# bgmanuel99/Super-Resolution-Images-for-3D-Printing-Defect-Detection

Hardware: AMD Instinct MI355X
Metric: 4x-SR MPix/s on 512x512 LR batch (higher is better)
Workload: dtype bf16

## Files before the change

__graft_entry__.py:

```python
import os
import subprocess
import sys

ROOT = os.path.dirname(os.path.abspath(__file__))
PKG = os.path.join(ROOT, "super-resolution-images-for-3d-printing-defect-detection_amd")
for p in (ROOT, PKG):
    if p not in sys.path:
        sys.path.insert(0, p)


def build():
    jobs = str(min(4, os.cpu_count() or 1))
    subprocess.run(["make", "-C", os.path.join(PKG, "csrc"), "-j", jobs], check=True)
    subprocess.run([sys.executable, os.path.join(ROOT, "tools", "check_prefetch_hazards.py")], check=True)
    subprocess.run([sys.executable, os.path.join(ROOT, "tools", "check_prefetch_hazards.py"), "--source", os.path.join(PKG, "csrc", "attention.hip"),
                    "--match", "attn_bf16_kernel", "--allow-scratch"], check=True)
    import sr355
    from sr355 import _lib
    _lib.load()
    import SRModels.loading_methods
    import oracle


def smoke():
    import numpy as np
    import torch
    assert torch.cuda.is_available(), "smoke() needs a GPU"
    from oracle import models as OM
    from oracle import ops as OO
    from sr355 import Context
    from sr355.synth import make_pairs
    from sr355.weights import bf16_rounded, init_weights
    from SRModels.deep_learning_models.ESRGAN_model import ESRGAN

    ctx = Context.get(0)
    lr, hr = make_pairs(1, 40, 36, 4, seed=7)
    for dtype, tol in (("f32", 1e-4), ("bf16", 2e-2)):
        m = ESRGAN(compute_dtype=dtype)
        m.setup_model(scale_factor=4, growth_channels=32, num_rrdb_blocks=2)
        w = init_weights(m.generator.layer_shapes(), seed=3000)
        if dtype == "bf16":
            w = bf16_rounded(w)
        m.set_weights(w)
        sr, metrics = m.super_resolve_image(lr[0], patch_size_lr=24, stride=12)
        ref = OM.esrgan_super_resolve(lr[0], w, 4, 24, 12, num_rrdb=2, dtype=np.float64)
        err = float(np.abs(sr - ref).max())
        assert sr.shape == (160, 144, 3) and err <= tol, (dtype, err)
        p_gpu = float(ctx.psnr(ctx.to_device(hr), ctx.to_device(sr[None]))[0])
        p_ref = float(OO.psnr(hr, ref[None].astype(np.float32))[0])
        assert abs(p_gpu - p_ref) <= 0.01, (p_gpu, p_ref)
        print(f"smoke[{dtype}]: max|gpu-oracle|={err:.2e}  PSNR(gpu,HR)={p_gpu:.4f} dB  PSNR(oracle,HR)={p_ref:.4f} dB  "
              f"time_sec={metrics['time_sec']:.4f}")
    print("smoke OK")


if __name__ == "__main__":
    build()
    if len(sys.argv) > 1 and sys.argv[1] == "smoke":
        smoke()
```

super-resolution-images-for-3d-printing-defect-detection_amd/csrc/api.hip:

```cpp
#include <math.h>
#include <stdio.h>
#include <stdlib.h>
#include <string.h>

#include <memory>

#include "common.h"

void* sr_ctx::dalloc(size_t bytes) {
    void* p = nullptr;
    if (bytes == 0) bytes = 16;
    if (alloc_cap > 0 && cur_bytes + (int64_t)bytes > alloc_cap) {
        err = "allocation of " + std::to_string(bytes) + " bytes exceeds the debug cap (sr_debug_set_alloc_cap)";
        return nullptr;
    }
    hipError_t e = hipMalloc(&p, bytes);
    if (e != hipSuccess) {
        err = std::string("hipMalloc(") + std::to_string(bytes) + "): " + hipGetErrorString(e);
        return nullptr;
    }
    allocs[p] = bytes;
    cur_bytes += (int64_t)bytes;
    if (cur_bytes > peak_bytes) peak_bytes = cur_bytes;
    return p;
}
void sr_ctx::dfree(void* p) {
    if (!p) return;
    auto it = allocs.find(p);
    if (it != allocs.end()) { cur_bytes -= (int64_t)it->second; allocs.erase(it); }
    (void)hipFree(p);
}
int sr_ctx::ensure_dyn_lds(const void* kernel, int bytes) {
    if (bytes > MAX_LDS_BYTES) return fail(SR_ERR_INVALID, "kernel needs " + std::to_string(bytes) + " bytes of LDS, a CU has " + std::to_string(MAX_LDS_BYTES));
    auto it = lds_attr_done.find(kernel);
    if (it != lds_attr_done.end() && it->second >= bytes) return SR_OK;
    hipError_t e = hipFuncSetAttribute(kernel, hipFuncAttributeMaxDynamicSharedMemorySize, bytes);
    if (e != hipSuccess) return fail(SR_ERR_HIP, std::string("hipFuncSetAttribute: ") + hipGetErrorString(e));
    lds_attr_done[kernel] = bytes;
    return SR_OK;
}
void* sr_ctx::scratch(size_t bytes) {
    if (bytes <= scratch_cap) return scratch_buf;
    if (scratch_buf) { (void)hipDeviceSynchronize(); dfree(scratch_buf); scratch_buf = nullptr; scratch_cap = 0; }
    size_t cap = bytes < (1u << 20) ? (1u << 20) : bytes;
    scratch_buf = dalloc(cap);
    if (scratch_buf) scratch_cap = cap;
    return scratch_buf;
}

int sr_ctx::cu_count() {
    if (num_cus <= 0) {
        hipDeviceProp_t prop;
        num_cus = (hipGetDeviceProperties(&prop, device) == hipSuccess && prop.multiProcessorCount > 0) ? prop.multiProcessorCount : 256;
    }
    return num_cus;
}

void* sr_ctx::arena(Arena& a, size_t bytes, hipStream_t st) {
    if (bytes <= a.cap) return a.p;
    if (a.p) { (void)hipStreamSynchronize(st); dfree(a.p); a.p = nullptr; a.cap = 0; }
    const size_t cap = bytes < (1u << 20) ? (1u << 20) : bytes + bytes / 4;
    a.p = dalloc(cap);
    if (a.p) a.cap = cap;
    return a.p;
}

int sr_ctx::prof_open(const std::string& name, double flops, double bytes, hipStream_t st) {
    if (!prof) return -1;
    int ni = -1;
    for (size_t i = 0; i < prof_names.size(); ++i) if (prof_names[i] == name) { ni = (int)i; break; }
    if (ni < 0) { prof_names.push_back(name); ni = (int)prof_names.size() - 1; }
    hipEvent_t e[2];
    for (int k = 0; k < 2; ++k) {
        if (!ev_pool.empty()) { e[k] = ev_pool.back(); ev_pool.pop_back(); }
        else if (hipEventCreate(&e[k]) != hipSuccess) return -1;
    }
    (void)hipEventRecord(e[0], st);
    prof_recs.push_back(ProfRec{ni, e[0], e[1], flops, bytes});
    return (int)prof_recs.size() - 1;
}
void sr_ctx::prof_close(int rec, hipStream_t st) {
    if (rec >= 0) (void)hipEventRecord(prof_recs[rec].e1, st);
}

namespace {

struct Param {
    std::string name; int which; std::vector<int64_t> shape; std::vector<float> host; bool set = false;
    int64_t count() const { int64_t n = 1; for (auto s : shape) n *= s; return n; }
};
struct Ref { int buf = -1; int coff = 0; };
enum OpKind { OP_CONVERT, OP_CONV, OP_ATTN, OP_POOL, OP_GAP, OP_DENSE, OP_TOBLK, OP_SUBSAMPLE, OP_PREPROC };
struct Op {
    OpKind kind = OP_CONV;
    Ref in, out, skip1, skip2;
    int conv = -1;
    int act = SR_ACT_LINEAR; float alpha = 1.f, beta1 = 0.f, beta2 = 0.f; int clip = 0, d2s = 1;
    int dw = -1, db = -1, In = 0, Out = 0;
    int chain = -1, chain_pos = 0;
    int rgbtail = -1;
    int pack_alt = -1;
    int pw2 = -1;
    int proj = -1;
    int block = -1, block_pos = 0;
};
struct BufSpec { int C = 0; int mul = 1; int shift = 0; bool vec = false; int Cbuf = 0; int blk = 0; int cshift = 0; int cells = 0; int cat = 0; };
struct ConvPart { std::string name; int cout; float scale = 1.f; };
struct ConvSpec { std::vector<ConvPart> parts; int KS = 3, Cin = 0, Cout = 0; ConvWeights w; int rows_head = 0; };
struct ChainSpec { int conv_a = -1, conv_b = -1; int tail = 0; ChainWeights w; };
struct RgbTailSpec { int conv_b = -1; RgbTailWeights w; };
struct BlockSpec { int conv[5] = {-1, -1, -1, -1, -1}; BlockWeights w; };
struct ProjSpec { int conv = -1; ProjWeights w; };
struct Pw2Spec { int conv = -1; int act = 0; Pw2Weights w; };

}

struct sr_model {
    sr_ctx* ctx = nullptr;
    int kind = 0;
    sr_model_cfg cfg{};
    int T = SR_DTYPE_BF16;
    std::vector<Param> params;
    std::vector<ConvSpec> convs;
    std::vector<ChainSpec> chains;
    std::vector<BlockSpec> blocks;
    std::vector<RgbTailSpec> rgbtails;
    std::vector<ProjSpec> projs;
    std::vector<Pw2Spec> pw2s;
    std::vector<BufSpec> bufs;
    std::vector<void*> bufp;
    std::vector<float*> dense_dev;
    std::vector<Op> ops;
    int in_C = 3, out_C = 3, out_mul = 1, out_shift = 0; bool out_vec = false;
    bool finalized = false;
    std::vector<size_t> bufcap;
    std::vector<CellGrid> grid_now;
    std::vector<int> routes;
    struct Tap { float* dst; int64_t cap; };
    std::unordered_map<int, Tap> taps;
    std::vector<std::string> op_names;
    int block_stream = 0;

    int find_param(const std::string& n, int which) const {
        for (size_t i = 0; i < params.size(); ++i) if (params[i].which == which && params[i].name == n) return (int)i;
        return -1;
    }
    void free_bufs() { for (auto& p : bufp) { if (p) ctx->dfree(p); p = nullptr; } bufcap.assign(bufcap.size(), 0); grid_now.assign(grid_now.size(), CellGrid{}); }
    TensorView view(const Ref& r) const { return r.buf >= 0 ? TensorView{bufp[r.buf], bufs[r.buf].Cbuf, r.coff, bufs[r.buf].blk} : TensorView{}; }
};

namespace {

struct Builder {
    sr_model* m;
    int esz() const { return dtype_size(m->T); }
    int E() const { return 16 / esz(); }
    int buf(int C, int mul = 1, int shift = 0) {
        BufSpec b; b.C = C; b.mul = mul; b.shift = shift; b.Cbuf = round_up(C, 32);
        m->bufs.push_back(b); return (int)m->bufs.size() - 1;
    }
    int vecbuf(int C) { BufSpec b; b.C = C; b.vec = true; b.Cbuf = C; m->bufs.push_back(b); return (int)m->bufs.size() - 1; }
    void add_layer_params(const std::string& name, std::vector<int64_t> kshape) {
        Param k; k.name = name; k.which = SR_WEIGHT_KERNEL; k.shape = kshape; m->params.push_back(k);
        Param b; b.name = name; b.which = SR_WEIGHT_BIAS; b.shape = {kshape.back()}; m->params.push_back(b);
    }
    int conv_spec(std::vector<ConvPart> parts, int KS, int Cin) {
        ConvSpec c; c.parts = parts; c.KS = KS; c.Cin = Cin; c.Cout = 0;
        for (auto& p : parts) { c.Cout += p.cout; add_layer_params(p.name, {KS, KS, Cin, p.cout}); }
        m->convs.push_back(c); return (int)m->convs.size() - 1;
    }
    Op& conv(const std::string& name, int KS, int Cin, int Cout, Ref in, Ref out, int act = SR_ACT_LINEAR) {
        Op o; o.kind = OP_CONV; o.conv = conv_spec({{name, Cout}}, KS, Cin); o.in = in; o.out = out; o.act = act;
        m->ops.push_back(o); return m->ops.back();
    }
    Op& conv_again(int spec, Ref in, Ref out, int act = SR_ACT_LINEAR) {
        Op o; o.kind = OP_CONV; o.conv = spec; o.in = in; o.out = out; o.act = act;
        m->ops.push_back(o); return m->ops.back();
    }
    void self_attention(const std::string& name, int x, int y, int qkv, int ao) {
        const float kscale = m->T == SR_DTYPE_BF16 ? 1.4426950408889634f : 1.f;
        Op p; p.kind = OP_CONV; p.conv = conv_spec({{name + "_f", 8, kscale}, {name + "_g", 8}, {name + "_h", 32}}, 1, 64);
        p.in = {x, 0}; p.out = {qkv, 0};
        if (m->T == SR_DTYPE_BF16 && !m->ops.empty() && m->ops.back().kind == OP_CONV && m->ops.back().out.buf == x && m->ops.back().out.coff == 0) {
            ProjSpec ps; ps.conv = p.conv;
            m->projs.push_back(ps);
            m->ops.back().proj = (int)m->projs.size() - 1;
        }
        m->ops.push_back(p);
        Op a; a.kind = OP_ATTN; a.in = {qkv, 0}; a.out = {ao, 0}; m->ops.push_back(a);
        Op& v = conv(name + "_v", 1, 32, 64, {ao, 0}, {y, 0});
        v.skip1 = {x, 0}; v.beta1 = 1.f;
    }
};

int build_srcnn(sr_model* m) {
    Builder b{m};
    const int C = m->cfg.channels;
    m->in_C = C; m->out_C = C; m->out_mul = 1;
    const int x0 = b.buf(b.E()), c1 = b.buf(96), c2 = b.buf(32);
    m->bufs[x0].Cbuf = b.E();
    Op cv; cv.kind = OP_CONVERT; cv.out = {x0, 0}; m->ops.push_back(cv);
    b.conv("conv2d", 9, C, 96, {x0, 0}, {c1, 0}, SR_ACT_RELU);
    b.conv("conv2d_1", 1, 96, 32, {c1, 0}, {c2, 0}, SR_ACT_RELU);
    if (m->T == SR_DTYPE_F32 && C == 3) {
        Pw2Spec ps; ps.conv = m->ops.back().conv; ps.act = SR_ACT_RELU;
        m->pw2s.push_back(ps);
        m->ops[m->ops.size() - 2].pw2 = (int)m->pw2s.size() - 1;
    }
    b.conv("conv2d_2", 5, 32, C, {c2, 0}, {-2, 0});
    return SR_OK;
}

int build_edsr(sr_model* m) {
    Builder b{m};
    const sr_model_cfg& c = m->cfg;
    const int C = c.channels, F = c.num_filters, s = c.scale_factor;
    if (s != 2 && s != 3 && s != 4) return m->ctx->fail(SR_ERR_INVALID, "Scale factor " + std::to_string(s) + " not supported. Use 2, 3, or 4.");
    m->in_C = C; m->out_C = C; m->out_mul = s;
    int li = 0;
    auto lname = [&]() { std::string n = li == 0 ? "conv2d" : "conv2d_" + std::to_string(li); ++li; return n; };
    const int x0 = b.buf(b.E());
    m->bufs[x0].Cbuf = b.E();
    const int head = b.buf(F), tmp = b.buf(F), ra = b.buf(F), rb = b.buf(F);
    Op cv; cv.kind = OP_CONVERT; cv.out = {x0, 0}; m->ops.push_back(cv);
    b.conv(lname(), 3, C, F, {x0, 0}, {head, 0});
    int cur = head;
    for (int i = 0; i < c.num_blocks; ++i) {
        const int nxt = (cur == ra) ? rb : ra;
        b.conv(lname(), 3, F, F, {cur, 0}, {tmp, 0}, SR_ACT_RELU);
        Op& o = b.conv(lname(), 3, F, F, {tmp, 0}, {nxt, 0});
        o.alpha = c.res_scaling; o.skip1 = {cur, 0}; o.beta1 = 1.f;
        cur = nxt;
    }
    const int body = (cur == ra) ? rb : ra;
    { Op& o = b.conv(lname(), 3, F, F, {cur, 0}, {body, 0}); o.skip1 = {head, 0}; o.beta1 = 1.f; }
    int up = body, mul = 1;
    const int nup = s == 4 ? 2 : 1, r = s == 4 ? 2 : s;
    for (int i = 0; i < nup; ++i) {
        mul *= r;
        const int ub = b.buf(F, mul);
        Op& o = b.conv(lname(), 3, F, F * r * r, {up, 0}, {ub, 0}); o.d2s = r;
        up = ub;
    }
    { Op& o = b.conv(lname(), 3, F, C, {up, 0}, {-2, 0}); o.clip = 1; }
    return SR_OK;
}

int build_esrgan(sr_model* m) {
    Builder b{m};
    const sr_model_cfg& c = m->cfg;
    const int C = c.channels, G = c.growth_channels, s = c.scale_factor;
    if (s < 1 || (s & (s - 1)) != 0) return m->ctx->fail(SR_ERR_INVALID, "ESRGAN scale_factor must be a power of two");
    if (G <= 0 || c.num_blocks < 0) return m->ctx->fail(SR_ERR_INVALID, "ESRGAN growth_channels/num_rrdb_blocks invalid");
    m->in_C = C; m->out_C = C; m->out_mul = s;
    const int CC = 64 + 4 * G;
    const int x0 = b.buf(b.E());
    const bool head_rows = m->T == SR_DTYPE_BF16;
    m->bufs[x0].Cbuf = head_rows ? 32 : b.E();
    const int trunk = b.buf(64);
    int cat[3] = {b.buf(CC), b.buf(CC), b.buf(CC)};
    if (m->T == SR_DTYPE_BF16 && G % 8 == 0)
        for (int i = 0; i < 3; ++i) m->bufs[cat[i]].blk = 1;
    for (int i = 0; i < 3; ++i) m->bufs[cat[i]].cat = 1;
    Op cv; cv.kind = OP_CONVERT; cv.out = {x0, 0}; m->ops.push_back(cv);
    b.conv("initial_conv", 3, C, 64, {x0, 0}, {trunk, 0});
    if (head_rows) m->convs.back().rows_head = 1;
    if (m->bufs[cat[0]].blk) {
        Op t; t.kind = OP_TOBLK; t.in = {trunk, 0}; t.out = {cat[0], 0}; m->ops.push_back(t);
    } else {
        b.conv_again((int)m->convs.size() - 1, {x0, 0}, {cat[0], 0});
    }
    int X = 0, Y = 1, Z = 2;
    for (int r = 0; r < c.num_blocks; ++r) {
        const int src[3] = {X, Y, Z}, dst[3] = {Y, Z, Y};
        for (int d = 0; d < 3; ++d) {
            const std::string dn = "rrdb_" + std::to_string(r) + "_dense" + std::to_string(d + 1);
            const int I = cat[src[d]], O = cat[dst[d]];
            const size_t first_op = m->ops.size();
            for (int k = 1; k <= 4; ++k)
                b.conv(dn + "_conv" + std::to_string(k), 3, 64 + (k - 1) * G, G, {I, 0}, {I, 64 + (k - 1) * G}, SR_ACT_RELU);
            Op& o = b.conv(dn + "_conv5", 3, CC, 64, {I, 0}, {O, 0});
            if (d < 2) { o.alpha = 0.2f; o.skip1 = {I, 0}; o.beta1 = 1.f; }
            else { o.alpha = 0.04f; o.skip1 = {cat[X], 0}; o.beta1 = 1.f; o.skip2 = {I, 0}; o.beta2 = 0.2f; }
            if (m->bufs[I].blk && G == 32) {
                auto link = [&](size_t opa, int tail) {
                    ChainSpec cs; cs.conv_a = m->ops[opa].conv; cs.conv_b = m->ops[opa + 1].conv; cs.tail = tail;
                    m->chains.push_back(cs);
                    m->ops[opa].chain = m->ops[opa + 1].chain = (int)m->chains.size() - 1;
                    m->ops[opa].chain_pos = 0; m->ops[opa + 1].chain_pos = 1;
                };
                link(first_op + 1, 0);
                link(first_op + 3, 1);
            }
            if (m->bufs[I].blk && G == 8) {
                BlockSpec bs;
                for (int k = 0; k < 5; ++k) {
                    bs.conv[k] = m->ops[first_op + k].conv;
                    m->ops[first_op + k].block = (int)m->blocks.size(); m->ops[first_op + k].block_pos = k;
                }
                m->blocks.push_back(bs);
            }
        }
        const int nX = Y, nY = Z, nZ = X; X = nX; Y = nY; Z = nZ;
    }
    const int t2 = b.buf(64);
    { Op& o = b.conv("trunk_conv", 3, 64, 64, {cat[X], 0}, {t2, 0}); o.skip1 = {trunk, 0}; o.beta1 = 1.f; o.pack_alt = cat[Y]; }
    int cur = t2;
    if (c.use_attention) {
        const int qkv = b.buf(64), ao = b.buf(32), t3 = b.buf(64);
        b.self_attention("self_attention_trunk", cur, t3, qkv, ao);
        cur = t3;
    }
    int mul = 1, nup = 0;
    for (int t = s; t > 1; t >>= 1) ++nup;
    for (int i = 0; i < nup; ++i) {
        mul *= 2;
        const int u = b.buf(64, mul);
        Op& o = b.conv("upsample_" + std::to_string(i) + "_conv", 3, 64, 256, {cur, 0}, {u, 0}, SR_ACT_LRELU);
        o.d2s = 2;
        cur = u;
        if (i == 0 && c.use_attention) {
            const int qkv = b.buf(64, mul), ao = b.buf(32, mul), ua = b.buf(64, mul);
            b.self_attention("self_attention_upsample_0", cur, ua, qkv, ao);
            cur = ua;
        }
    }
    const int f1 = b.buf(64, mul);
    b.conv("final_conv1", 3, 64, 64, {cur, 0}, {f1, 0}, SR_ACT_RELU);
    b.conv("final_conv2", 3, 64, C, {f1, 0}, {-2, 0}, SR_ACT_TANH);
    if (m->T == SR_DTYPE_BF16 && C <= 3) {
        RgbTailSpec rt; rt.conv_b = m->ops.back().conv;
        m->rgbtails.push_back(rt);
        m->ops[m->ops.size() - 2].rgbtail = (int)m->rgbtails.size() - 1;
    }
    return SR_OK;
}

int build_vgg16(sr_model* m) {
    Builder b{m};
    const int nc = m->cfg.num_classes;
    if (nc <= 0) return m->ctx->fail(SR_ERR_INVALID, "num_classes must be positive");
    m->in_C = 3; m->out_C = nc; m->out_vec = true;
    static const int cfg[5][2] = {{2, 64}, {2, 128}, {3, 256}, {3, 512}, {3, 512}};
    const int x0 = b.buf(b.E());
    const bool head_rows = m->T == SR_DTYPE_BF16;
    m->bufs[x0].Cbuf = head_rows ? 32 : b.E();
    Op cv; cv.kind = OP_CONVERT; cv.out = {x0, 0}; m->ops.push_back(cv);
    int cur = x0, cin = 3;
    for (int blk = 0; blk < 5; ++blk) {
        for (int k = 0; k < cfg[blk][0]; ++k) {
            const int o = b.buf(cfg[blk][1], 1, blk);
            b.conv("block" + std::to_string(blk + 1) + "_conv" + std::to_string(k + 1), 3, cin, cfg[blk][1], {cur, 0}, {o, 0}, SR_ACT_RELU);
            if (blk == 0 && k == 0 && head_rows) m->convs.back().rows_head = 1;
            if (blk == 4 && m->T == SR_DTYPE_BF16) m->bufs[o].cells = 1;
            cur = o; cin = cfg[blk][1];
        }
        const int pb = b.buf(cin, 1, blk + 1);
        if (blk == 3 && m->T == SR_DTYPE_BF16) m->bufs[pb].cells = 1;
        Op p; p.kind = OP_POOL; p.in = {cur, 0}; p.out = {pb, 0}; m->ops.push_back(p);
        cur = pb;
    }
    const int g = b.vecbuf(512), d1 = b.vecbuf(256);
    { Op o; o.kind = OP_GAP; o.in = {cur, 0}; o.out = {g, 0}; m->ops.push_back(o); }
    b.add_layer_params("dense", {512, 256});
    { Op o; o.kind = OP_DENSE; o.in = {g, 0}; o.out = {d1, 0}; o.In = 512; o.Out = 256; o.act = SR_ACT_RELU;
      o.dw = m->find_param("dense", SR_WEIGHT_KERNEL); o.db = m->find_param("dense", SR_WEIGHT_BIAS); m->ops.push_back(o); }
    b.add_layer_params("predictions", {256, nc});
    { Op o; o.kind = OP_DENSE; o.in = {d1, 0}; o.out = {-2, 0}; o.In = 256; o.Out = nc; o.act = 100;
      o.dw = m->find_param("predictions", SR_WEIGHT_KERNEL); o.db = m->find_param("predictions", SR_WEIGHT_BIAS); m->ops.push_back(o); }
    return SR_OK;
}

int build_discriminator(sr_model* m) {
    Builder b{m};
    m->in_C = 3; m->out_C = 1; m->out_vec = true;
    const int x0 = b.buf(b.E());
    m->bufs[x0].Cbuf = b.E();
    Op cv; cv.kind = OP_CONVERT; cv.out = {x0, 0}; m->ops.push_back(cv);
    static const int filt[6] = {64, 64, 64, 128, 128, 256}, strd[6] = {1, 2, 1, 2, 1, 2};
    int cur = x0, cin = 3, halv = 0;
    for (int i = 0; i < 6; ++i) {
        const int o = b.buf(filt[i]);
        m->bufs[o].cshift = halv;
        b.conv("disc_conv" + std::to_string(i + 1), 3, cin, filt[i], {cur, 0}, {o, 0}, SR_ACT_LRELU);
        cur = o; cin = filt[i];
        if (strd[i] == 2) {
            ++halv;
            const int s2 = b.buf(filt[i]);
            m->bufs[s2].cshift = halv;
            Op sp; sp.kind = OP_SUBSAMPLE; sp.in = {cur, 0}; sp.out = {s2, 0}; m->ops.push_back(sp);
            cur = s2;
        }
    }
    const int g = b.vecbuf(256), d1 = b.vecbuf(256);
    { Op o; o.kind = OP_GAP; o.in = {cur, 0}; o.out = {g, 0}; m->ops.push_back(o); }
    b.add_layer_params("disc_dense1", {256, 256});
    { Op o; o.kind = OP_DENSE; o.in = {g, 0}; o.out = {d1, 0}; o.In = 256; o.Out = 256; o.act = SR_ACT_LRELU;
      o.dw = m->find_param("disc_dense1", SR_WEIGHT_KERNEL); o.db = m->find_param("disc_dense1", SR_WEIGHT_BIAS); m->ops.push_back(o); }
    b.add_layer_params("disc_output", {256, 1});
    { Op o; o.kind = OP_DENSE; o.in = {d1, 0}; o.out = {-2, 0}; o.In = 256; o.Out = 1; o.act = 101;
      o.dw = m->find_param("disc_output", SR_WEIGHT_KERNEL); o.db = m->find_param("disc_output", SR_WEIGHT_BIAS); m->ops.push_back(o); }
    return SR_OK;
}

int build_vgg19_features(sr_model* m) {
    Builder b{m};
    m->in_C = 3; m->out_C = 512; m->out_mul = 1; m->out_shift = 4;
    static const int cfg[5][2] = {{2, 64}, {2, 128}, {4, 256}, {4, 512}, {4, 512}};
    const int x0 = b.buf(b.E());
    m->bufs[x0].Cbuf = b.E();
    Op pp; pp.kind = OP_PREPROC; pp.out = {x0, 0}; m->ops.push_back(pp);
    int cur = x0, cin = 3;
    for (int blk = 0; blk < 5; ++blk) {
        for (int k = 0; k < cfg[blk][0]; ++k) {
            const bool last = blk == 4 && k == cfg[blk][0] - 1;
            const int o = last ? -2 : b.buf(cfg[blk][1], 1, blk);
            b.conv("block" + std::to_string(blk + 1) + "_conv" + std::to_string(k + 1), 3, cin, cfg[blk][1], {cur, 0}, {o, 0}, SR_ACT_RELU);
            cur = o; cin = cfg[blk][1];
        }
        if (blk == 4) break;
        const int pb = b.buf(cin, 1, blk + 1);
        Op p; p.kind = OP_POOL; p.in = {cur, 0}; p.out = {pb, 0}; m->ops.push_back(p);
        cur = pb;
    }
    return SR_OK;
}

inline void buf_hw(const BufSpec& b, int H, int W, int* h, int* w) {
    *h = (H * b.mul) >> b.shift; *w = (W * b.mul) >> b.shift;
    for (int i = 0; i < b.cshift; ++i) { *h = (*h + 1) / 2; *w = (*w + 1) / 2; }
}

CellGrid cell_grid_for(int B, int h, int w, int Cbuf) {
    CellGrid g;
    if (h < 1 || w < 1 || w + 1 > 16) return g;
    const int gx = 16 / (w + 1);
    const double plain = (double)h * w / ((double)((h + 11) / 12 * 12) * ((w + 15) / 16 * 16));
    const double packed = (double)h / (h + 1) * gx * w / 16.0;
    if (packed < 1.3 * plain) return g;
    const int64_t Hv = (int64_t)((B + gx - 1) / gx) * (h + 1), Wv = (int64_t)gx * (w + 1);
    if (Hv * Wv * Cbuf >= ((int64_t)1 << 31)) return g;
    g.gx = gx; g.ch = h + 1; g.cw = w + 1; g.Hv = (int)Hv; g.Wv = (int)Wv;
    return g;
}

CellGrid cat_grid_for(int B, int H, int W, int Cmax) {
    CellGrid g;
    if (B < 4 || H < 2 || W < 2) return g;
    const double plain = (double)H * W / ((double)((H + 15) / 16 * 16) * ((W + 15) / 16 * 16));
    const int gx = B < 16 ? B : 16;
    const int64_t Hv = (int64_t)((B + gx - 1) / gx) * (H + 1), Wv = (int64_t)gx * (W + 1);
    const double packed = (double)B * H * W / ((double)((Hv + 15) / 16 * 16) * ((Wv + 15) / 16 * 16));
    if (packed >= 1.15 * plain && Hv * Wv * Cmax < ((int64_t)1 << 31)) { g.gx = gx; g.ch = H + 1; g.cw = W + 1; g.Hv = (int)Hv; g.Wv = (int)Wv; }
    return g;
}

struct Layout {
    bool pack2 = false;
    CellGrid cat;
    bool use_cells = false;
    int B_ws = 0;
};

enum BlockKernel { BLOCK_NONE, BLOCK_RESIDENT, BLOCK_STREAM };
BlockKernel block_kernel(const sr_model* m, int H, int W) {
    if (!(m->kind == SR_MODEL_ESRGAN_G && m->T == SR_DTYPE_BF16 && !m->blocks.empty() && (m->ctx->chain_mask & SR_FUSE_TWO_UP) == SR_FUSE_TWO_UP)) return BLOCK_NONE;
    const bool ring = m->block_stream && H >= 1 && sr_dense_block_stream_lds_bytes(m->cfg.growth_channels, W) > 0;
    if (m->block_stream == 2 && ring) return BLOCK_STREAM;
    if (sr_dense_block_lds_bytes(m->cfg.growth_channels, H, W) > 0) return BLOCK_RESIDENT;
    return ring ? BLOCK_STREAM : BLOCK_NONE;
}
bool block_here(const sr_model* m, int H, int W) { return block_kernel(m, H, W) != BLOCK_NONE; }

Layout choose_layout(const sr_model* m, int B, int H, int W) {
    const int mask = m->ctx->chain_mask;
    Layout L;
    L.use_cells = m->taps.empty() && (mask & SR_FUSE_CELLS) != 0;
    L.pack2 = m->kind == SR_MODEL_ESRGAN_G && m->T == SR_DTYPE_BF16 && W == 24 && (mask & SR_FUSE_TWO_UP) == SR_FUSE_TWO_UP && !m->chains.empty() && B >= 2;
    for (const auto& tp : m->taps) {
        const Op& to = m->ops[tp.first];
        if (to.kind == OP_CONV && to.chain >= 0 && m->chains[to.chain].tail && to.chain_pos == 0) L.pack2 = false;
    }
    bool cat_blk = false; int Cmax = 0;
    for (const BufSpec& bs : m->bufs) if (bs.cat) { cat_blk = cat_blk || bs.blk; Cmax = std::max(Cmax, bs.Cbuf); }
    const bool fused_here = !m->chains.empty() && W == 48 && (mask & (SR_FUSE_DENSE_TAIL | SR_FUSE_DENSE_MID));
    if (m->kind == SR_MODEL_ESRGAN_G && m->T == SR_DTYPE_BF16 && cat_blk && !L.pack2 && !fused_here && !block_here(m, H, W) && m->taps.empty()) L.cat = cat_grid_for(B, H, W, Cmax);
    L.B_ws = L.pack2 ? (B + 1) & ~1 : L.cat.gx ? (int)std::max<int64_t>(B, ((int64_t)L.cat.Hv * L.cat.Wv + (int64_t)H * W - 1) / ((int64_t)H * W)) : B;
    return L;
}

int ensure_workspace(sr_model* m, const Layout& L, int H, int W, hipStream_t st) {
    const int B = L.B_ws;
    if (m->bufp.size() != m->bufs.size()) { m->bufp.assign(m->bufs.size(), nullptr); m->bufcap.assign(m->bufs.size(), 0); m->grid_now.assign(m->bufs.size(), CellGrid{}); }
    for (size_t i = 0; i < m->bufs.size(); ++i) {
        const BufSpec& b = m->bufs[i];
        size_t bytes;
        CellGrid want;
        if (b.vec) bytes = (size_t)B * b.C * sizeof(float);
        else {
            int h, w; buf_hw(b, H, W, &h, &w);
            bytes = (size_t)B * h * w * b.Cbuf * dtype_size(m->T) + 4096;
            if (b.cat) want = L.cat;
            else if (b.cells && L.use_cells) want = cell_grid_for(B, h, w, b.Cbuf);
            if (want.gx) bytes = std::max(bytes, (size_t)want.Hv * want.Wv * b.Cbuf * dtype_size(m->T) + 4096);
        }
        if (bytes <= m->bufcap[i]) {
            const CellGrid& have = m->grid_now[i];
            if (want.gx && !(have.gx == want.gx && have.ch == want.ch && have.cw == want.cw && have.Wv == want.Wv)) SR_HIP(m->ctx, hipMemsetAsync(m->bufp[i], 0, m->bufcap[i], st));
            m->grid_now[i] = want;
            continue;
        }
        m->grid_now[i] = want;
        if (m->bufp[i]) { SR_HIP(m->ctx, hipDeviceSynchronize()); m->ctx->dfree(m->bufp[i]); m->bufp[i] = nullptr; m->bufcap[i] = 0; }
        m->bufp[i] = m->ctx->dalloc(bytes);
        if (!m->bufp[i]) {
            const std::string why = m->ctx->err;
            (void)hipDeviceSynchronize();
            m->free_bufs();
            return m->ctx->fail(SR_ERR_OOM, "workspace for [" + std::to_string(B) + "," + std::to_string(H) + "," + std::to_string(W) + "]: " + why +
                                                " (all workspaces of this model were released)");
        }
        SR_HIP(m->ctx, hipMemsetAsync(m->bufp[i], 0, bytes, st));
        m->bufcap[i] = bytes;
    }
    return SR_OK;
}

enum Route { RT_CHAIN = OP_PREPROC + 1, RT_CHAIN_SECOND, RT_BLOCK, RT_BLOCK_REST, RT_CONV1_STREAM, RT_RGB_TAIL, RT_PW2, RT_IN_EPILOGUE, RT_BLOCK_STREAM };

bool tapped(const sr_model* m, size_t oi) { return !m->taps.empty() && m->taps.count((int)oi) != 0; }
bool bare_epilogue(const Op& op) { return op.skip1.buf < 0 && op.skip2.buf < 0 && op.d2s == 1 && !op.clip; }

bool chain_fits(const sr_model* m, size_t oi, int w, bool pack2) {
    const Op& op = m->ops[oi];
    if (op.chain < 0 || op.chain_pos != 0) return false;
    const ChainSpec& ch = m->chains[op.chain];
    return !(ch.tail && tapped(m, oi)) && (m->ctx->chain_mask & (ch.tail ? SR_FUSE_DENSE_TAIL : SR_FUSE_DENSE_MID)) && chain_supported(ch.w, m->view(op.in), pack2 ? 48 : w);
}
bool conv1_stream_fits(const sr_model* m, const Op& op, int w, bool pack2) {
    return (m->ctx->chain_mask & SR_FUSE_CONV1_STREAM) && op.chain < 0 && op.act == SR_ACT_RELU && op.alpha == 1.f && bare_epilogue(op) && op.out.buf == op.in.buf &&
           op.in.coff == 0 && op.out.coff == 64 && conv1_stream_supported(m->convs[op.conv].w, m->view(op.in), pack2 ? 48 : w);
}
bool rgb_tail_fits(const sr_model* m, const Op& op, size_t oi, int B, int h, int w) {
    const ConvWeights& cw = m->convs[op.conv].w;
    return op.rgbtail >= 0 && (m->ctx->chain_mask & SR_FUSE_RGB_TAIL) && !tapped(m, oi) && cw.rows && cw.NT == 4 && cw.Cout == 64 && bare_epilogue(op) &&
           op.act != SR_ACT_TANH && op.out.buf >= 0 && (int64_t)m->bufcap[op.out.buf] >= rgbtail_partial_bytes(B, h, w);
}
bool pw2_fits(const sr_model* m, const Op& op, size_t oi) {
    const ConvWeights& cw = m->convs[op.conv].w;
    return op.pw2 >= 0 && (m->ctx->chain_mask & SR_FUSE_SRCNN_1X1) && !tapped(m, oi) && cw.thin && !cw.few && cw.dtype == SR_DTYPE_F32 && bare_epilogue(op);
}
bool pool_fits(const sr_model* m, const Op& op, size_t oi, int h, int w) {
    if (oi + 1 >= m->ops.size() || op.out.buf < 0) return false;
    const Op& pl = m->ops[oi + 1];
    const ConvWeights& cw = m->convs[op.conv].w;
    return (m->ctx->chain_mask & SR_FUSE_POOL) && m->T == SR_DTYPE_BF16 && pl.kind == OP_POOL && pl.in.buf == op.out.buf && pl.out.buf >= 0 && cw.rows && cw.NT == 4 &&
           cw.CoutP == cw.Cout && bare_epilogue(op) && op.act != SR_ACT_TANH && !tapped(m, oi) && !m->grid_now[op.in.buf].gx && !m->grid_now[op.out.buf].gx &&
           h >= 2 && w >= 2 && m->bufs[pl.out.buf].Cbuf % 8 == 0 && m->bufs[pl.out.buf].Cbuf >= cw.Cout;
}
bool proj_fits(const sr_model* m, const Op& op) {
    const ConvWeights& cw = m->convs[op.conv].w;
    return op.proj >= 0 && (m->ctx->chain_mask & SR_FUSE_ATTN_PROJ) && cw.rows && cw.NT == 4 && cw.Cout / (op.d2s * op.d2s) == 64 && cw.CoutP == cw.Cout &&
           op.out.buf >= 0 && !m->bufs[op.out.buf].blk && op.skip2.buf < 0 && !op.clip && op.act != SR_ACT_TANH && m->bufs[op.out.buf].Cbuf % 4 == 0;
}

void plan_routes(sr_model* m, const Layout& L, int B, int H, int W) {
    std::vector<int>& rt = m->routes;
    rt.resize(m->ops.size());
    for (size_t oi = 0; oi < m->ops.size(); ++oi) rt[oi] = m->ops[oi].kind;
    for (size_t oi = 0; oi < m->ops.size(); ++oi) {
        const Op& op = m->ops[oi];
        if (rt[oi] != OP_CONV) continue;
        int h, w;
        buf_hw(m->bufs[op.in.buf], H, W, &h, &w);
        if (op.block >= 0 && op.block_pos == 0 && block_here(m, h, w)) {
            rt[oi] = block_kernel(m, h, w) == BLOCK_STREAM ? RT_BLOCK_STREAM : RT_BLOCK;
            for (int k = 1; k < 5; ++k) rt[oi + k] = RT_BLOCK_REST;
        }
        else if (chain_fits(m, oi, w, L.pack2)) { rt[oi] = RT_CHAIN; rt[oi + 1] = RT_CHAIN_SECOND; }
        else if (conv1_stream_fits(m, op, w, L.pack2)) rt[oi] = RT_CONV1_STREAM;
        else if (rgb_tail_fits(m, op, oi, B, h, w)) { rt[oi] = RT_RGB_TAIL; rt[oi + 1] = RT_IN_EPILOGUE; }
        else if (pw2_fits(m, op, oi)) { rt[oi] = RT_PW2; rt[oi + 1] = RT_IN_EPILOGUE; }
        else if (pool_fits(m, op, oi, h, w) || proj_fits(m, op)) rt[oi + 1] = RT_IN_EPILOGUE;
    }
}

}

extern "C" {

int sr_init(int device_id, sr_ctx** out) {
    if (!out) return SR_ERR_INVALID;
    *out = nullptr;
    int n = 0;
    if (hipGetDeviceCount(&n) != hipSuccess || device_id < 0 || device_id >= n) return SR_ERR_HIP;
    if (hipSetDevice(device_id) != hipSuccess) return SR_ERR_HIP;
    sr_ctx* c = new sr_ctx();
    c->device = device_id;
    if (hipEventCreate(&c->ev0) != hipSuccess || hipEventCreate(&c->ev1) != hipSuccess) { delete c; return SR_ERR_HIP; }
    c->zero_page = c->dalloc(sr_ctx::ZERO_PAGE_BYTES);
    if (!c->zero_page) { sr_destroy(c); return SR_ERR_OOM; }
    if (hipMemset(c->zero_page, 0, sr_ctx::ZERO_PAGE_BYTES) != hipSuccess) { sr_destroy(c); return SR_ERR_HIP; }
    *out = c;
    return SR_OK;
}

void sr_destroy(sr_ctx* ctx) {
    DeviceGuard dg_(ctx);
    if (!ctx) return;
    (void)hipDeviceSynchronize();
    lpips_release(ctx);
    std::vector<void*> ps;
    for (auto& kv : ctx->allocs) ps.push_back(kv.first);
    for (void* p : ps) ctx->dfree(p);
    if (ctx->ev0) (void)hipEventDestroy(ctx->ev0);
    if (ctx->ev1) (void)hipEventDestroy(ctx->ev1);
    for (auto& r : ctx->prof_recs) { (void)hipEventDestroy(r.e0); (void)hipEventDestroy(r.e1); }
    for (auto& e : ctx->ev_pool) (void)hipEventDestroy(e);
    delete ctx;
}

const char* sr_last_error(sr_ctx* ctx) { return ctx ? ctx->err.c_str() : "null ctx"; }

int sr_mem_info(sr_ctx* ctx, int64_t* current_bytes, int64_t* peak_bytes) {
    if (!ctx) return SR_ERR_INVALID;
    if (current_bytes) *current_bytes = ctx->cur_bytes;
    if (peak_bytes) *peak_bytes = ctx->peak_bytes;
    return SR_OK;
}

int sr_last_forward_ms(sr_ctx* ctx, float* ms) {
    DeviceGuard dg_(ctx);
    if (!ctx || !ms) return SR_ERR_INVALID;
    if (!ctx->timed) return ctx->fail(SR_ERR_STATE, "no forward has run on this ctx");
    SR_HIP(ctx, hipEventSynchronize(ctx->ev1));
    SR_HIP(ctx, hipEventElapsedTime(ms, ctx->ev0, ctx->ev1));
    return SR_OK;
}

int64_t sr_debug_stamp_bytes_needed(int which, int64_t workgroups) {
    if (which == 0) return workgroups < 0 ? -1 : workgroups * 16 * (int64_t)sizeof(unsigned long long);
    if (which == 1) return (int64_t)64 * 4 * 64 * 4 * (int64_t)sizeof(unsigned long long);
    return -1;
}

int sr_debug_set_stamp_buffer(sr_ctx* ctx, void* device_u64_buffer, int64_t capacity_bytes) {
    if (!ctx) return SR_ERR_INVALID;
    if (device_u64_buffer && capacity_bytes < sr_debug_stamp_bytes_needed(0, 1))
        return ctx->fail(SR_ERR_INVALID, "sr_debug_set_stamp_buffer: the buffer does not hold one workgroup's stamps");
    ctx->stamp_buf = static_cast<unsigned long long*>(device_u64_buffer);
    ctx->stamp_cap = device_u64_buffer ? capacity_bytes : 0;
    return SR_OK;
}

int sr_measure_clock(sr_ctx* ctx, float* mhz, void* stream) {
    if (!ctx || !mhz) return SR_ERR_INVALID;
    DeviceGuard dg_(ctx);
    return clock_probe_launch(ctx, mhz, static_cast<hipStream_t>(stream));
}

int sr_debug_set_chain_stamp_buffer(sr_ctx* ctx, void* device_u64_buffer, int64_t capacity_bytes) {
    if (!ctx) return SR_ERR_INVALID;
    if (device_u64_buffer && capacity_bytes < sr_debug_stamp_bytes_needed(1, 0))
        return ctx->fail(SR_ERR_INVALID, "sr_debug_set_chain_stamp_buffer: the buffer is smaller than the stamped kernels write (sr_debug_stamp_bytes_needed(1, 0))");
    ctx->chain_stamp_buf = static_cast<unsigned long long*>(device_u64_buffer);
    const char* skip = getenv("SR355_CHAIN_STAMP_SKIP");
    ctx->chain_stamp_skip = skip ? atoi(skip) : -1;
    return SR_OK;
}

int sr_debug_set_fused(sr_ctx* ctx, int mask, int max_workgroups) {
    if (!ctx) return SR_ERR_INVALID;
    ctx->chain_mask = mask;
    ctx->chain_max_wgs = max_workgroups > 0 ? max_workgroups : 0;
    return SR_OK;
}

int sr_debug_set_block_stream_bands(sr_ctx* ctx, int n) {
    if (!ctx) return SR_ERR_INVALID;
    ctx->block_stream_bands = n > 0 ? n : 0;
    return SR_OK;
}

int sr_model_set_dense_block_stream(sr_model* m, int mode) {
    if (!m) return SR_ERR_INVALID;
    if (mode < 0 || mode > 2) return m->ctx->fail(SR_ERR_INVALID, "sr_model_set_dense_block_stream: mode is 0, 1 or 2");
    if (!(m->kind == SR_MODEL_ESRGAN_G && m->T == SR_DTYPE_BF16 && m->cfg.growth_channels == 8 && !m->blocks.empty()))
        return m->ctx->fail(SR_ERR_INVALID, "sr_model_set_dense_block_stream: the streamed dense-block kernel serves bf16 ESRGAN generators of 8 growth channels only");
    m->block_stream = mode;
    return SR_OK;
}

int sr_debug_set_alloc_cap(sr_ctx* ctx, int64_t bytes) {
    if (!ctx) return SR_ERR_INVALID;
    ctx->alloc_cap = bytes > 0 ? bytes : 0;
    return SR_OK;
}

int sr_debug_conv_routes(sr_ctx* ctx, int enable, char* text, int64_t cap) {
    if (!ctx) return SR_ERR_INVALID;
    if (text && cap <= (int64_t)ctx->route_text.size()) return ctx->fail(SR_ERR_CAPACITY, "sr_debug_conv_routes: the text buffer is too small");
    if (text) memcpy(text, ctx->route_text.c_str(), ctx->route_text.size() + 1);
    ctx->route_text.clear();
    ctx->route_log = enable != 0;
    return SR_OK;
}

int sr_profile_begin(sr_ctx* ctx) {
    if (!ctx) return SR_ERR_INVALID;
    for (auto& r : ctx->prof_recs) { ctx->ev_pool.push_back(r.e0); ctx->ev_pool.push_back(r.e1); }
    ctx->prof_recs.clear();
    ctx->prof = true;
    return SR_OK;
}

int sr_profile_end(sr_ctx* ctx, char* json, int64_t cap) {
    DeviceGuard dg_(ctx);
    if (!ctx || !json || cap <= 0) return SR_ERR_INVALID;
    ctx->prof = false;
    SR_HIP(ctx, hipDeviceSynchronize());
    struct Agg { int64_t n = 0; double ms = 0, flops = 0, bytes = 0; };
    std::vector<Agg> agg(ctx->prof_names.size());
    for (auto& r : ctx->prof_recs) {
        float ms = 0.f;
        if (hipEventElapsedTime(&ms, r.e0, r.e1) != hipSuccess) continue;
        Agg& a = agg[r.name];
        a.n += 1; a.ms += ms; a.flops += r.flops; a.bytes += r.bytes;
    }
    std::string s = "[";
    bool first = true;
    for (size_t i = 0; i < agg.size(); ++i) {
        if (!agg[i].n) continue;
        char buf[512];
        snprintf(buf, sizeof buf, "%s{\"kernel\": \"%s\", \"launches\": %lld, \"total_ms\": %.6f, \"flops\": %.6e, \"bytes\": %.6e}",
                 first ? "" : ", ", ctx->prof_names[i].c_str(), (long long)agg[i].n, agg[i].ms, agg[i].flops, agg[i].bytes);
        s += buf;
        first = false;
    }
    s += "]";
    for (auto& r : ctx->prof_recs) { ctx->ev_pool.push_back(r.e0); ctx->ev_pool.push_back(r.e1); }
    ctx->prof_recs.clear();
    if ((int64_t)s.size() + 1 > cap) return ctx->fail(SR_ERR_CAPACITY, "profile buffer too small");
    memcpy(json, s.c_str(), s.size() + 1);
    return SR_OK;
}

int sr_model_create(sr_ctx* ctx, int kind, const sr_model_cfg* cfg, sr_model** out) {
    if (!ctx || !cfg || !out) return SR_ERR_INVALID;
    *out = nullptr;
    if (cfg->compute_dtype != SR_DTYPE_F32 && cfg->compute_dtype != SR_DTYPE_BF16)
        return ctx->fail(SR_ERR_INVALID, "compute_dtype must be SR_DTYPE_F32 or SR_DTYPE_BF16");
    std::unique_ptr<sr_model> m(new sr_model());
    m->ctx = ctx; m->kind = kind; m->cfg = *cfg; m->T = cfg->compute_dtype;
    if (m->cfg.channels <= 0) m->cfg.channels = 3;
    if (m->cfg.channels > 16 / dtype_size(m->T))
        return ctx->fail(SR_ERR_INVALID, "channels must fit one 16-byte slice (<= 4 for f32, <= 8 for bf16)");
    int rc;
    switch (kind) {
        case SR_MODEL_SRCNN: rc = build_srcnn(m.get()); break;
        case SR_MODEL_EDSR: rc = build_edsr(m.get()); break;
        case SR_MODEL_ESRGAN_G: rc = build_esrgan(m.get()); break;
        case SR_MODEL_VGG16: rc = build_vgg16(m.get()); break;
        case SR_MODEL_ESRGAN_D: rc = build_discriminator(m.get()); break;
        case SR_MODEL_VGG19_FEATURES: rc = build_vgg19_features(m.get()); break;
        default: return ctx->fail(SR_ERR_INVALID, "unknown model kind");
    }
    if (rc) return rc;
    m->dense_dev.assign(m->params.size(), nullptr);
    *out = m.release();
    return SR_OK;
}

void sr_model_destroy(sr_model* m) {
    DeviceGuard dg_(m ? m->ctx : nullptr);
    if (!m) return;
    (void)hipDeviceSynchronize();
    m->free_bufs();
    for (auto& c : m->convs) conv_free_weights(m->ctx, &c.w);
    for (auto& ch : m->chains) chain_free_weights(m->ctx, &ch.w);
    for (auto& bs : m->blocks) block_free_weights(m->ctx, &bs.w);
    for (auto& rt : m->rgbtails) rgbtail_free_weights(m->ctx, &rt.w);
    for (auto& pj : m->projs) proj_free_weights(m->ctx, &pj.w);
    for (auto& pw : m->pw2s) pw2_free_weights(m->ctx, &pw.w);
    for (auto& p : m->dense_dev) if (p) m->ctx->dfree(p);
    delete m;
}

int sr_model_release_workspace(sr_model* m) {
    if (!m) return SR_ERR_INVALID;
    DeviceGuard dg_(m->ctx);
    SR_HIP(m->ctx, hipDeviceSynchronize());
    m->free_bufs();
    return SR_OK;
}

static void op_out_view(const sr_model* m, const Op& op, int* C, int* mul, int* shift, int* cshift = nullptr) {
    *C = 0; *mul = 1; *shift = 0;
    if (cshift) *cshift = 0;
    if (op.out.buf < 0) return;
    const BufSpec& b = m->bufs[op.out.buf];
    if (b.vec) return;
    *mul = b.mul; *shift = b.shift;
    if (cshift) *cshift = b.cshift;
    if (op.kind == OP_CONV) { const ConvSpec& cs = m->convs[op.conv]; *C = cs.Cout / (op.d2s * op.d2s); }
    else if (op.kind == OP_ATTN) *C = 32;
    else if (op.kind == OP_TOBLK) *C = 64;
    else *C = b.C;
}

int sr_model_num_ops(sr_model* m) { return m ? (int)m->ops.size() : SR_ERR_INVALID; }

int sr_model_op_info(sr_model* m, int index, const char** name, int* channels, int* mul, int* shift, int* ceil_halvings) {
    if (!m || index < 0 || index >= (int)m->ops.size()) return SR_ERR_INVALID;
    if (m->op_names.size() != m->ops.size()) {
        m->op_names.clear();
        static const char* kinds[] = {"convert", "conv", "attention", "maxpool", "gap", "dense", "to_blocked", "stride2_pick", "vgg_preprocess"};
        for (const Op& op : m->ops)
            m->op_names.push_back(op.kind == OP_CONV ? m->convs[op.conv].parts[0].name : std::string(kinds[op.kind]));
    }
    int C, mu, sh, cs;
    op_out_view(m, m->ops[index], &C, &mu, &sh, &cs);
    if (name) *name = m->op_names[index].c_str();
    if (channels) *channels = C;
    if (mul) *mul = mu;
    if (shift) *shift = sh;
    if (ceil_halvings) *ceil_halvings = cs;
    return SR_OK;
}

int sr_model_set_tap(sr_model* m, int op_index, float* device_dst, int64_t capacity) {
    if (!m || op_index < 0 || op_index >= (int)m->ops.size()) return SR_ERR_INVALID;
    if (!device_dst) { m->taps.erase(op_index); return SR_OK; }
    int C, mu, sh;
    op_out_view(m, m->ops[op_index], &C, &mu, &sh);
    if (C <= 0) return m->ctx->fail(SR_ERR_INVALID, "this op has no activation-buffer output to tap");
    m->taps[op_index] = sr_model::Tap{device_dst, capacity};
    return SR_OK;
}

int sr_model_num_params(sr_model* m) { return m ? (int)m->params.size() : SR_ERR_INVALID; }

int sr_model_param_info(sr_model* m, int index, const char** name, int* which, int64_t shape[4], int* ndim) {
    if (!m || index < 0 || index >= (int)m->params.size()) return SR_ERR_INVALID;
    const Param& p = m->params[index];
    if (name) *name = p.name.c_str();
    if (which) *which = p.which;
    if (ndim) *ndim = (int)p.shape.size();
    if (shape) for (size_t i = 0; i < 4; ++i) shape[i] = i < p.shape.size() ? p.shape[i] : 1;
    return SR_OK;
}

int sr_model_set_weight(sr_model* m, const char* name, int which, const float* host, const int64_t* shape, int ndim) {
    if (!m || !name || !host || !shape) return SR_ERR_INVALID;
    const int i = m->find_param(name, which);
    if (i < 0) return m->ctx->fail(SR_ERR_NAME, std::string("no parameter '") + name + "' (which=" + std::to_string(which) + ")");
    Param& p = m->params[i];
    bool ok = ndim == (int)p.shape.size();
    for (int d = 0; ok && d < ndim; ++d) ok = shape[d] == p.shape[d];
    if (!ok) return m->ctx->fail(SR_ERR_INVALID, std::string("shape mismatch for '") + name + "'");
    p.host.assign(host, host + p.count());
    p.set = true;
    m->finalized = false;
    return SR_OK;
}

int sr_model_finalize(sr_model* m) {
    DeviceGuard dg_(m ? m->ctx : nullptr);
    if (!m) return SR_ERR_INVALID;
    sr_ctx* ctx = m->ctx;
    for (auto& p : m->params)
        if (!p.set) return ctx->fail(SR_ERR_STATE, "parameter '" + p.name + (p.which ? "' bias" : "' kernel") + " was never set");
    auto gather = [&](const ConvSpec& c, std::vector<float>& k, std::vector<float>& bias) {
        const int taps = c.KS * c.KS;
        k.assign((size_t)taps * c.Cin * c.Cout, 0.f); bias.assign(c.Cout, 0.f);
        int co0 = 0;
        for (auto& part : c.parts) {
            const Param& pk = m->params[m->find_param(part.name, SR_WEIGHT_KERNEL)];
            const Param& pb = m->params[m->find_param(part.name, SR_WEIGHT_BIAS)];
            for (int t = 0; t < taps; ++t)
                for (int ci = 0; ci < c.Cin; ++ci)
                    for (int co = 0; co < part.cout; ++co)
                        k[((size_t)t * c.Cin + ci) * c.Cout + co0 + co] = part.scale * pk.host[((size_t)t * c.Cin + ci) * part.cout + co];
            for (int co = 0; co < part.cout; ++co) bias[co0 + co] = part.scale * pb.host[co];
            co0 += part.cout;
        }
    };
    for (auto& c : m->convs) {
        conv_free_weights(ctx, &c.w);
        std::vector<float> k, bias;
        gather(c, k, bias);
        int rc = conv_pack_weights(ctx, k.data(), bias.data(), c.KS, c.Cin, c.Cout, m->T, &c.w, c.rows_head);
        if (rc) return rc;
    }
    for (auto& ch : m->chains) {
        chain_free_weights(ctx, &ch.w);
        const ConvSpec& a = m->convs[ch.conv_a], &bq = m->convs[ch.conv_b];
        std::vector<float> ka, ba, kb, bb;
        gather(a, ka, ba);
        gather(bq, kb, bb);
        int rc = chain_pack_weights(ctx, ka.data(), ba.data(), kb.data(), bb.data(), a.Cin / 32, a.Cout / 16, bq.Cout / 16, &ch.w);
        if (rc) return rc;
    }
    for (auto& bs : m->blocks) {
        block_free_weights(ctx, &bs.w);
        std::vector<float> k[5], bias[5];
        const float* kp[5]; const float* bp[5];
        for (int i = 0; i < 5; ++i) { gather(m->convs[bs.conv[i]], k[i], bias[i]); kp[i] = k[i].data(); bp[i] = bias[i].data(); }
        int rc = block_pack_weights(ctx, kp, bp, &bs.w);
        if (rc) return rc;
    }
    for (auto& rt : m->rgbtails) {
        rgbtail_free_weights(ctx, &rt.w);
        const ConvSpec& c2 = m->convs[rt.conv_b];
        std::vector<float> k, bias;
        gather(c2, k, bias);
        int rc = rgbtail_pack_weights(ctx, k.data(), bias.data(), c2.Cout, &rt.w);
        if (rc) return rc;
    }
    for (auto& pj : m->projs) {
        proj_free_weights(ctx, &pj.w);
        const ConvSpec& c1 = m->convs[pj.conv];
        std::vector<float> k, bias;
        gather(c1, k, bias);
        int rc = proj_pack_weights(ctx, k.data(), bias.data(), c1.Cout, &pj.w);
        if (rc) return rc;
    }
    for (auto& pw : m->pw2s) {
        pw2_free_weights(ctx, &pw.w);
        const ConvSpec& c1 = m->convs[pw.conv];
        std::vector<float> k, bias;
        gather(c1, k, bias);
        int rc = pw2_pack_weights(ctx, k.data(), bias.data(), c1.Cin, c1.Cout, pw.act, &pw.w);
        if (rc) return rc;
    }
    for (auto& op : m->ops) {
        if (op.kind != OP_DENSE) continue;
        for (int pi : {op.dw, op.db}) {
            if (m->dense_dev[pi]) ctx->dfree(m->dense_dev[pi]);
            const Param& p = m->params[pi];
            m->dense_dev[pi] = static_cast<float*>(ctx->dalloc(sizeof(float) * p.count()));
            if (!m->dense_dev[pi]) return SR_ERR_OOM;
            SR_HIP(ctx, hipMemcpy(m->dense_dev[pi], p.host.data(), sizeof(float) * p.count(), hipMemcpyHostToDevice));
        }
    }
    m->finalized = true;
    return SR_OK;
}

int sr_model_output_shape(sr_model* m, int B, int H, int W, int C, int64_t out_shape[4]) {
    if (!m || !out_shape) return SR_ERR_INVALID;
    (void)C;
    if (m->out_vec) { out_shape[0] = B; out_shape[1] = m->out_C; out_shape[2] = 1; out_shape[3] = 1; }
    else { out_shape[0] = B; out_shape[1] = ((int64_t)H * m->out_mul) >> m->out_shift; out_shape[2] = ((int64_t)W * m->out_mul) >> m->out_shift; out_shape[3] = m->out_C; }
    return SR_OK;
}

int sr_forward(sr_model* m, const void* x, int io_dtype, int B, int H, int W, int C, void* y, int64_t y_capacity, void* stream) {
    DeviceGuard dg_(m ? m->ctx : nullptr);
    if (!m) return SR_ERR_INVALID;
    sr_ctx* ctx = m->ctx;
    hipStream_t st = static_cast<hipStream_t>(stream);
    if (!m->finalized) return ctx->fail(SR_ERR_STATE, "sr_model_finalize has not been called");
    if (!x || !y) return ctx->fail(SR_ERR_INVALID, "null tensor");
    if (io_dtype != SR_DTYPE_F32 && io_dtype != SR_DTYPE_BF16) return ctx->fail(SR_ERR_INVALID, "io dtype must be f32 or bf16");
    if (io_dtype == SR_DTYPE_BF16 && m->T == SR_DTYPE_F32) return ctx->fail(SR_ERR_INVALID, "an fp32 model takes fp32 tensors");
    if (C != m->in_C) return ctx->fail(SR_ERR_INVALID, "channel count does not match the model");
    if (B == 0) return SR_OK;
    if (B < 0 || H <= 0 || W <= 0) return ctx->fail(SR_ERR_INVALID, "bad tensor shape");
    int64_t os[4];
    sr_model_output_shape(m, B, H, W, C, os);
    if (y_capacity < os[0] * os[1] * os[2] * os[3]) return ctx->fail(SR_ERR_CAPACITY, "output buffer too small");
    if (m->kind == SR_MODEL_VGG16 && (H < 32 || W < 32)) return ctx->fail(SR_ERR_INVALID, "VGG16 needs H,W >= 32");
    if (m->kind == SR_MODEL_VGG19_FEATURES && (H < 16 || W < 16)) return ctx->fail(SR_ERR_INVALID, "VGG19 features need H,W >= 16");
    const Layout L = choose_layout(m, B, H, W);
    int rc = ensure_workspace(m, L, H, W, st);
    if (rc) return rc;
    plan_routes(m, L, B, H, W);
    SR_HIP(ctx, hipEventRecord(ctx->ev0, st));
    const int T = m->T;
    for (size_t oi = 0; oi < m->ops.size(); ++oi) {
        const Op& op = m->ops[oi];
        const int route = m->routes[oi];
        const Op* nx = oi + 1 < m->ops.size() && m->routes[oi + 1] == RT_IN_EPILOGUE ? &m->ops[oi + 1] : nullptr;
        int h = H, w = W;
        if (op.in.buf >= 0) buf_hw(m->bufs[op.in.buf], H, W, &h, &w);
        const TensorView vi = m->view(op.in), vo = m->view(op.out);
        void* const po = op.out.buf >= 0 ? m->bufp[op.out.buf] : nullptr;
        switch (route) {
            case RT_CHAIN_SECOND: case RT_BLOCK_REST: case RT_IN_EPILOGUE:
                break;
            case RT_BLOCK: case RT_BLOCK_STREAM: {
                const Op& o5 = m->ops[oi + 4];
                const bool x1 = o5.skip1.buf == op.in.buf && o5.skip1.coff == 0;
                const Ref& other = x1 ? o5.skip2 : o5.skip1;
                bool grow = false;
                for (int k = 0; k < 4; ++k) grow = grow || tapped(m, oi + k);
                rc = (route == RT_BLOCK ? block_launch : block_stream_launch)(ctx, m->blocks[op.block].w, vi, B, h, w, m->view(o5.out), other.buf >= 0 ? m->view(other) : TensorView{},
                                                                              o5.alpha, o5.beta1, o5.beta2, x1 ? 1 : 2, grow ? 1 : 0, st);
                break;
            }
            case RT_CHAIN: {
                const ChainSpec& ch = m->chains[op.chain];
                const Op& ob = m->ops[oi + 1];
                TensorView outv{}, so{};
                float bx = 0.f, bo = 0.f;
                if (ch.tail) {
                    outv = m->view(ob.out);
                    for (int k2 = 0; k2 < 2; ++k2) {
                        const Ref& r = k2 ? ob.skip2 : ob.skip1;
                        const float be = k2 ? ob.beta2 : ob.beta1;
                        if (r.buf < 0) continue;
                        if (r.buf == op.in.buf && r.coff == 0) bx = be; else { so = m->view(r); bo = be; }
                    }
                }
                rc = chain_launch(ctx, ch.w, vi, L.pack2 ? (B + 1) / 2 : B, h, L.pack2 ? 48 : w, outv, so, ob.alpha, bx, bo, st, L.pack2);
                break;
            }
            case RT_CONV1_STREAM:
                rc = conv1_stream_launch(ctx, m->convs[op.conv].w, vi, L.pack2 ? (B + 1) / 2 : B, h, L.pack2 ? 48 : w, st, L.pack2);
                break;
            case RT_RGB_TAIL: case RT_PW2: case OP_CONV: {
                const ConvSpec& cs = m->convs[op.conv];
                int in = op.in.buf;
                TensorView xin = vi;
                if (op.pack_alt >= 0 && (L.pack2 || m->grid_now[in].gx)) {
                    void* d = m->bufp[op.pack_alt];
                    const int64_t dC = m->bufs[op.pack_alt].Cbuf;
                    const CellGrid& g = m->grid_now[in];
                    rc = g.gx ? cell_unpack_launch(ctx, vi.p, vi.cs, vi.coff, B, h, w, 64, d, dC, 0, g, st) : unpack_pairs_launch(ctx, vi.p, vi.cs, vi.coff, B, h, w, 64, d, dC, 0, st);
                    if (rc) return rc;
                    in = op.pack_alt;
                    m->grid_now[in] = CellGrid{};
                    xin = m->view({in, 0});
                } else if (L.pack2 && vi.blk) {
                    return ctx->fail(SR_ERR_STATE, "two-up packed dense blocks: a conv outside the fused kernels would read a packed buffer");
                }
                const CellGrid g = m->grid_now[in];
                bool same = g.gx == 0 || op.d2s == 1;
                for (const Ref& r : {op.out, op.skip1, op.skip2})
                    if (r.buf != -1 && !((r.buf >= 0 ? m->grid_now[r.buf] : CellGrid{}) == g)) same = false;
                if (!same) return ctx->fail(SR_ERR_STATE, "packed small-image layout: producer and consumer disagree");
                const int cB = g.gx ? 1 : B;
                if (g.gx) { h = g.Hv; w = g.Wv; }
                ConvEpilogue ep;
                ep.act = op.act; ep.alpha = op.alpha; ep.clip01 = op.clip; ep.d2s_r = op.d2s; ep.cell_h = g.ch; ep.cell_w = g.cw;
                if (op.skip1.buf >= 0) { ep.skip1 = m->view(op.skip1); ep.beta1 = op.beta1; }
                if (op.skip2.buf >= 0) { ep.skip2 = m->view(op.skip2); ep.beta2 = op.beta2; }
                if (route == RT_RGB_TAIL) {
                    const RgbTailWeights& rt = m->rgbtails[op.rgbtail].w;
                    ep.f2 = &rt; ep.f2_part = static_cast<float*>(po);
                    rc = conv_launch(ctx, cs.w, xin, cB, h, w, TensorView{}, ep, st);
                    if (!rc) rc = rgbtail_finish_launch(ctx, rt, ep.f2_part, cB, h, w, nx->act, nx->alpha, nx->clip, y, m->out_C, 0, io_dtype == SR_DTYPE_F32, st);
                    break;
                }
                if (route == RT_PW2) ep.pw2 = &m->pw2s[op.pw2].w;
                else if (nx && nx->kind == OP_POOL) { ep.pool_out = m->view(nx->out); ep.pool_grid = m->grid_now[nx->out.buf]; }
                else if (nx) { ep.pj = &m->projs[op.proj].w; ep.pj_out = m->view(nx->out); }
                if (op.out.buf == -2) {
                    ep.out_f32 = io_dtype == SR_DTYPE_F32;
                    rc = conv_launch(ctx, cs.w, xin, B, h, w, y, m->out_C, 0, ep, st);
                } else {
                    rc = conv_launch(ctx, cs.w, xin, cB, h, w, route == RT_PW2 ? m->view(nx->out) : vo, ep, st);
                }
                break;
            }
            case OP_CONVERT:
                rc = convert_pad_launch(ctx, x, io_dtype, (int64_t)B * H * W, C, po, T, vo.cs, 1.f, 0.f, st);
                break;
            case OP_PREPROC:
                rc = vgg_preproc_launch(ctx, x, io_dtype, (int64_t)B * H * W, po, T, vo.cs, st);
                break;
            case OP_ATTN:
                rc = attention_launch(ctx, T, vi.p, vi.cs,  8,  0,  16, B, h * w, po, vo.cs, 0, st);
                break;
            case OP_SUBSAMPLE:
                rc = subsample2_launch(ctx, T, vi.p, B, h, w, m->bufs[op.in.buf].C, vi.cs, po, vo.cs, st);
                break;
            case OP_TOBLK: {
                const CellGrid& g = m->grid_now[op.out.buf];
                rc = g.gx ? cell_pack_launch(ctx, vi.p, vi.cs, vi.coff, B, h, w, 64, po, vo.cs, vo.coff, g, st)
                   : L.pack2 ? pack_pairs_launch(ctx, vi.p, vi.cs, vi.coff, B, h, w, 64, po, vo.cs, vo.coff, st)
                             : nhwc_to_blocked_launch(ctx, vi.p, vi.cs, vi.coff, B, h, w, 64, po, vo.cs, vo.coff, st);
                break;
            }
            case OP_POOL:
                rc = maxpool2_launch(ctx, T, vi.p, B, h, w, m->bufs[op.in.buf].C, vi.cs, po, vo.cs, st, m->grid_now[op.in.buf], m->grid_now[op.out.buf]);
                break;
            case OP_GAP:
                rc = gap_launch(ctx, T, vi.p, B, h * w, m->bufs[op.in.buf].C, vi.cs, static_cast<float*>(po), st);
                break;
            case OP_DENSE: {
                const bool f32 = op.out.buf != -2 || io_dtype == SR_DTYPE_F32;
                float* yf = static_cast<float*>(op.out.buf == -2 ? y : po);
                rc = dense_launch(ctx, static_cast<const float*>(vi.p), m->dense_dev[op.dw], m->dense_dev[op.db], B, op.In, op.Out, op.act, f32 ? yf : nullptr,
                                  f32 ? 0 : io_dtype, f32 ? nullptr : y, st);
                break;
            }
        }
        if (rc) return rc;
        if (tapped(m, oi)) {
            int C_, mu, sh, th, tw;
            op_out_view(m, op, &C_, &mu, &sh);
            buf_hw(m->bufs[op.out.buf], H, W, &th, &tw);
            const sr_model::Tap& tp = m->taps.at((int)oi);
            if (tp.cap < (int64_t)B * th * tw * C_) return ctx->fail(SR_ERR_CAPACITY, "tap buffer too small");
            rc = tap_copy_launch(ctx, vo.p, T, vo.blk, vo.cs, vo.coff, B, th, tw, C_, tp.dst, st, L.pack2 && vo.blk);
            if (rc) return rc;
        }
    }
    SR_HIP(ctx, hipEventRecord(ctx->ev1, st));
    ctx->timed = true;
    return SR_OK;
}

static ConvEpilogue single_op_epilogue(int act, float alpha, int clip01, int d2s_r, TensorView skip1, float beta1, TensorView skip2, float beta2) {
    ConvEpilogue ep;
    ep.act = act; ep.alpha = alpha; ep.clip01 = clip01; ep.d2s_r = d2s_r < 1 ? 1 : d2s_r;
    ep.allow_splitk = 1;
    if (skip1.p) { ep.skip1 = skip1; ep.beta1 = beta1; }
    if (skip2.p) { ep.skip2 = skip2; ep.beta2 = beta2; }
    return ep;
}

static int padded_cin(const ConvWeights& cw) { return cw.thin ? cw.CinP : round_up(cw.CinP, 32); }

int sr_conv2d(sr_ctx* ctx, const void* x, int dtype, int B, int H, int W, int Cin, const float* w_hwio, const float* bias, int KH, int KW,
              int Cout, int act, float alpha, const void* skip1, float beta1, const void* skip2, float beta2, int clip01, int d2s_r,
              void* y, void* stream) {
    DeviceGuard dg_(ctx);
    if (!ctx) return SR_ERR_INVALID;
    hipStream_t st = static_cast<hipStream_t>(stream);
    if (!x || !w_hwio || !y) return ctx->fail(SR_ERR_INVALID, "null tensor");
    if (KH != KW) return ctx->fail(SR_ERR_INVALID, "square kernels only");
    if (dtype != SR_DTYPE_F32 && dtype != SR_DTYPE_BF16) return ctx->fail(SR_ERR_INVALID, "dtype must be f32 or bf16");
    if (B <= 0 || H <= 0 || W <= 0 || Cin <= 0 || Cout <= 0) return ctx->fail(SR_ERR_INVALID, "bad tensor shape");
    ConvWeights cw;
    int rc = conv_pack_weights(ctx, w_hwio, bias, KH, Cin, Cout, dtype, &cw);
    if (rc) return rc;
    const int esz = dtype_size(dtype);
    const int Cp = padded_cin(cw);
    void* xp = ctx->dalloc((size_t)B * H * W * Cp * esz + 4096);
    if (!xp) { conv_free_weights(ctx, &cw); return SR_ERR_OOM; }
    rc = convert_pad_launch(ctx, x, dtype, (int64_t)B * H * W, Cin, xp, dtype, Cp, 1.f, 0.f, st);
    if (!rc) {
        auto skip_view = [&](const void* s) { return (s == x && Cout == Cin) ? TensorView{xp, Cp, 0} : TensorView{s, Cout, 0}; };
        const ConvEpilogue ep = single_op_epilogue(act, alpha, clip01, d2s_r, skip_view(skip1), beta1, skip_view(skip2), beta2);
        const int r = ep.d2s_r;
        rc = conv_launch(ctx, cw, TensorView{xp, Cp, 0}, B, H, W, y, Cout / (r * r), 0, ep, st);
    }
    hipError_t e = hipStreamSynchronize(st);
    ctx->dfree(xp);
    conv_free_weights(ctx, &cw);
    if (!rc && e != hipSuccess) return ctx->fail(SR_ERR_HIP, std::string("conv2d: ") + hipGetErrorString(e));
    return rc;
}

int sr_conv2d_dev(sr_ctx* ctx, const void* x, int B, int H, int W, int Cin, const float* d_w, const float* d_bias, int K, int Cout, int rot,
                  int act, float alpha, const void* skip1, float beta1, const void* skip2, float beta2, int clip01, int d2s_r, void* y,
                  void* stream) {
    DeviceGuard dg_(ctx);
    if (!ctx) return SR_ERR_INVALID;
    hipStream_t st = static_cast<hipStream_t>(stream);
    if (!x || !d_w || !y) return ctx->fail(SR_ERR_INVALID, "null tensor");
    if (B <= 0 || H <= 0 || W <= 0 || Cin <= 0 || Cout <= 0) return ctx->fail(SR_ERR_INVALID, "bad tensor shape");
    ConvWeights cw;
    int rc = conv_pack_weights_dev(ctx, d_w, d_bias, K, Cin, Cout, rot, &cw, st);
    if (rc) return rc;
    const int Cp = padded_cin(cw);
    const void* xp = x;
    if (Cp != Cin || ((uintptr_t)x % 16) != 0) {
        void* xa = ctx->arena(ctx->dev_x, (size_t)B * H * W * Cp * 4 + 4096, st);
        if (!xa) return SR_ERR_OOM;
        rc = convert_pad_launch(ctx, x, SR_DTYPE_F32, (int64_t)B * H * W, Cin, xa, SR_DTYPE_F32, Cp, 1.f, 0.f, st);
        if (rc) return rc;
        xp = xa;
    }
    const ConvEpilogue ep = single_op_epilogue(act, alpha, clip01, d2s_r, TensorView{skip1, Cout, 0}, beta1, TensorView{skip2, Cout, 0}, beta2);
    const int r = ep.d2s_r;
    return conv_launch(ctx, cw, TensorView{xp, Cp, 0}, B, H, W, y, Cout / (r * r), 0, ep, st);
}

int sr_conv2d_dev_views(sr_ctx* ctx, const sr_view* x, int B, int H, int W, int Cin, const float* d_w, const float* d_bias, int K, int Cout, int rot, int act, float alpha,
                        const sr_view* skip1, float beta1, const sr_view* y, void* stream) {
    DeviceGuard dg_(ctx);
    if (!ctx) return SR_ERR_INVALID;
    hipStream_t st = static_cast<hipStream_t>(stream);
    if (!x || !x->p || !d_w || !y || !y->p) return ctx->fail(SR_ERR_INVALID, "null tensor");
    if (B <= 0 || H <= 0 || W <= 0 || Cin <= 0 || Cout <= 0) return ctx->fail(SR_ERR_INVALID, "bad tensor shape");
    for (const sr_view* v : {x, y, skip1})
        if (v && v->p && (v->coff < 0 || v->cs <= 0 || v->coff >= v->cs)) return ctx->fail(SR_ERR_INVALID, "bad view");
    if (x->cs - x->coff < Cin || y->cs - y->coff < Cout || (skip1 && skip1->p && skip1->cs - skip1->coff < Cout)) return ctx->fail(SR_ERR_INVALID, "a view is narrower than its channel count");
    ConvWeights cw;
    int rc = conv_pack_weights_dev(ctx, d_w, d_bias, K, Cin, Cout, rot, &cw, st);
    if (rc) return rc;
    if (cw.thin || cw.CinP != Cin) return ctx->fail(SR_ERR_INVALID, "conv views: the input channel count must be a whole number of the kernel's channel chunks (16 fp32 channels)");
    const ConvEpilogue ep = single_op_epilogue(act, alpha, 0, 1, skip1 ? TensorView{skip1->p, skip1->cs, skip1->coff} : TensorView{}, beta1, TensorView{}, 0.f);
    return conv_launch(ctx, cw, TensorView{x->p, x->cs, x->coff}, B, H, W, TensorView{y->p, y->cs, y->coff}, ep, st);
}

int sr_conv_prepack(sr_ctx* ctx, const sr_pack_desc* uses, int n, void* stream) {
    DeviceGuard dg_(ctx);
    if (!ctx) return SR_ERR_INVALID;
    if (n < 0 || (n > 0 && !uses)) { ctx->pack32.cache.clear(); return ctx->fail(SR_ERR_INVALID, "conv prepack: bad list"); }
    return conv_prepack_dev(ctx, uses, n, static_cast<hipStream_t>(stream));
}

int sr_conv2d_dev_bf16(sr_ctx* ctx, const void* x, int B, int H, int W, int Cin, const float* d_w, const float* d_bias, int K, int Cout, int rot,
                       int act, float alpha, const void* skip1, float beta1, const void* skip2, float beta2, int clip01, int d2s_r, void* y,
                       void* stream) {
    DeviceGuard dg_(ctx);
    if (!ctx) return SR_ERR_INVALID;
    hipStream_t st = static_cast<hipStream_t>(stream);
    if (!x || !d_w || !y) return ctx->fail(SR_ERR_INVALID, "null tensor");
    if (B <= 0 || H <= 0 || W <= 0 || Cin <= 0 || Cout <= 0) return ctx->fail(SR_ERR_INVALID, "bad tensor shape");
    ConvWeights cw;
    int rc = conv_pack_weights_dev_bf16(ctx, d_w, d_bias, K, Cin, Cout, rot, &cw, st);
    if (rc) return rc;
    const int Cp = padded_cin(cw);
    const void* xp = x;
    if (Cp != Cin || ((uintptr_t)x % 16) != 0) {
        void* xa = ctx->arena(ctx->dev_x, (size_t)B * H * W * Cp * 2 + 4096, st);
        if (!xa) return SR_ERR_OOM;
        rc = convert_pad_launch(ctx, x, SR_DTYPE_BF16, (int64_t)B * H * W, Cin, xa, SR_DTYPE_BF16, Cp, 1.f, 0.f, st);
        if (rc) return rc;
        xp = xa;
    }
    auto skip_view = [&](const void* s) { return (s == x && Cout == Cin) ? TensorView{xp, Cp, 0} : TensorView{s, Cout, 0}; };
    const ConvEpilogue ep = single_op_epilogue(act, alpha, clip01, d2s_r, skip_view(skip1), beta1, skip_view(skip2), beta2);
    const int r = ep.d2s_r;
    return conv_launch(ctx, cw, TensorView{xp, Cp, 0}, B, H, W, y, Cout / (r * r), 0, ep, st);
}

int sr_conv_prepack_bf16(sr_ctx* ctx, const sr_pack_desc* uses, int n, void* stream) {
    DeviceGuard dg_(ctx);
    if (!ctx) return SR_ERR_INVALID;
    if (n < 0 || (n > 0 && !uses)) { ctx->pack16.cache.clear(); return ctx->fail(SR_ERR_INVALID, "conv prepack: bad list"); }
    return conv_prepack_dev_bf16(ctx, uses, n, static_cast<hipStream_t>(stream));
}

int sr_conv2d_wgrad_bf16(sr_ctx* ctx, const void* x, int64_t x_cs, const void* dy, int64_t dy_cs, int B, int H, int W, int Cin, int Cout, int K, float scale, float* dw_hwio,
                         float* db, void* stream) {
    DeviceGuard dg_(ctx);
    if (!ctx) return SR_ERR_INVALID;
    if (!x || !dy || !dw_hwio) return ctx->fail(SR_ERR_INVALID, "null tensor");
    if (K != 3) return ctx->fail(SR_ERR_INVALID, "wgrad_bf16: 3x3 layers only");
    return wgrad_bf16_launch(ctx, static_cast<const bf16_t*>(x), x_cs, static_cast<const bf16_t*>(dy), dy_cs, B, H, W, Cin, Cout, scale, dw_hwio, db, static_cast<hipStream_t>(stream));
}

int sr_conv2d_dev_views_bf16(sr_ctx* ctx, const sr_view* x, int B, int H, int W, int Cin, const float* d_w, const float* d_bias, int K, int Cout, int rot, int act, float alpha,
                             const sr_view* skip1, float beta1, const sr_view* skip2, float beta2, const sr_view* y, void* stream) {
    DeviceGuard dg_(ctx);
    if (!ctx) return SR_ERR_INVALID;
    hipStream_t st = static_cast<hipStream_t>(stream);
    if (!x || !x->p || !d_w || !y || !y->p) return ctx->fail(SR_ERR_INVALID, "null tensor");
    if (B <= 0 || H <= 0 || W <= 0 || Cin <= 0 || Cout <= 0) return ctx->fail(SR_ERR_INVALID, "bad tensor shape");
    for (const sr_view* v : {x, y, skip1, skip2})
        if (v && v->p && (v->coff < 0 || v->cs <= 0 || v->coff >= v->cs || v->cs % 8 != 0 || v->coff % 8 != 0 || ((uintptr_t)v->p % 16) != 0))
            return ctx->fail(SR_ERR_INVALID, "conv views bf16: a view's channel stride and first channel must be multiples of 8 (16 bytes), its buffer 16-byte aligned");
    if (x->cs - x->coff < Cin || y->cs - y->coff < Cout || (skip1 && skip1->p && skip1->cs - skip1->coff < Cout) || (skip2 && skip2->p && skip2->cs - skip2->coff < Cout))
        return ctx->fail(SR_ERR_INVALID, "a view is narrower than its channel count");
    if (Cin % 32 != 0) return ctx->fail(SR_ERR_INVALID, "conv views bf16: the input channel count must be a whole number of the kernel's 32-channel chunks");
    ConvWeights cw;
    int rc = conv_pack_weights_dev_bf16(ctx, d_w, d_bias, K, Cin, Cout, rot, &cw, st);
    if (rc) return rc;
    if (cw.thin || cw.CinP != Cin) return ctx->fail(SR_ERR_INVALID, "conv views bf16: the input channel count must be a whole number of the kernel's 32-channel chunks");
    auto tv = [](const sr_view* v) { return (v && v->p) ? TensorView{v->p, v->cs, v->coff} : TensorView{}; };
    const ConvEpilogue ep = single_op_epilogue(act, alpha, 0, 1, tv(skip1), beta1, tv(skip2), beta2);
    return conv_launch(ctx, cw, tv(x), B, H, W, tv(y), ep, st);
}

int sr_conv2d_wgrad_group_bf16(sr_ctx* ctx, const sr_wgrad_job* jobs, int n, int B, int H, int W, void* stream) {
    DeviceGuard dg_(ctx);
    if (!ctx) return SR_ERR_INVALID;
    return wgrad_group_bf16_launch(ctx, jobs, n, B, H, W, static_cast<hipStream_t>(stream));
}

int sr_eltwise_views_bf16(sr_ctx* ctx, int op, const sr_view* a, const sr_view* b, float alpha, float beta, const sr_view* out, int64_t npix, int C, void* stream) {
    DeviceGuard dg_(ctx);
    if (!ctx) return SR_ERR_INVALID;
    if (!a || !a->p || !out || !out->p) return ctx->fail(SR_ERR_INVALID, "null tensor");
    for (const sr_view* v : {a, b, out})
        if (v && v->p && (v->coff < 0 || v->cs - v->coff < C)) return ctx->fail(SR_ERR_INVALID, "a view is narrower than its channel count");
    const bf16_t* bp = (b && b->p) ? static_cast<const bf16_t*>(b->p) + b->coff : nullptr;
    return eltwise_views_bf16_launch(ctx, op, static_cast<const bf16_t*>(a->p) + a->coff, a->cs, bp, bp ? b->cs : 0, alpha, beta,
                                     static_cast<bf16_t*>(const_cast<void*>(out->p)) + out->coff, out->cs, npix, C, static_cast<hipStream_t>(stream));
}

int sr_relu_bwd_bf16(sr_ctx* ctx, const void* dy, const void* y, void* out, int64_t n, void* stream) {
    DeviceGuard dg_(ctx);
    if (!ctx) return SR_ERR_INVALID;
    if (!dy || !y || !out) return ctx->fail(SR_ERR_INVALID, "null tensor");
    return relu_bwd_bf16_launch(ctx, static_cast<const bf16_t*>(dy), static_cast<const bf16_t*>(y), static_cast<bf16_t*>(out), n, static_cast<hipStream_t>(stream));
}

int sr_space_to_depth_bf16(sr_ctx* ctx, const void* x, int B, int H, int W, int C, int r, void* y, void* stream) {
    DeviceGuard dg_(ctx);
    if (!ctx) return SR_ERR_INVALID;
    if (!x || !y) return ctx->fail(SR_ERR_INVALID, "null tensor");
    return space_to_depth_bf16_launch(ctx, static_cast<const bf16_t*>(x), B, H, W, C, r, static_cast<bf16_t*>(y), static_cast<hipStream_t>(stream));
}

int sr_mse_clip_grad_bf16(sr_ctx* ctx, const void* pre, const float* t, int64_t n, float* loss1, void* dpre, float* y, void* stream) {
    DeviceGuard dg_(ctx);
    if (!ctx) return SR_ERR_INVALID;
    if (!pre || !t || !loss1 || !dpre) return ctx->fail(SR_ERR_INVALID, "null tensor");
    return mse_clip_grad_bf16_launch(ctx, static_cast<const bf16_t*>(pre), t, n, loss1, static_cast<bf16_t*>(dpre), y, static_cast<hipStream_t>(stream));
}

int sr_conv2d_wgrad_views(sr_ctx* ctx, const sr_view* x, const sr_view* dy, int B, int H, int W, int Cin, int Cout, int K, float* dw_hwio, float* db, void* stream) {
    DeviceGuard dg_(ctx);
    if (!ctx) return SR_ERR_INVALID;
    if (!x || !x->p || !dy || !dy->p || !dw_hwio) return ctx->fail(SR_ERR_INVALID, "null tensor");
    if (x->coff < 0 || dy->coff < 0 || x->cs - x->coff < Cin || dy->cs - dy->coff < Cout) return ctx->fail(SR_ERR_INVALID, "a view is narrower than its channel count");
    return wgrad_launch_views(ctx, static_cast<const float*>(x->p) + x->coff, x->cs, static_cast<const float*>(dy->p) + dy->coff, dy->cs, B, H, W, Cin, Cout, K, dw_hwio, db,
                              static_cast<hipStream_t>(stream));
}

int sr_eltwise_views(sr_ctx* ctx, int op, const sr_view* a, const sr_view* b, float alpha, float beta, const sr_view* out, int64_t npix, int C, void* stream) {
    DeviceGuard dg_(ctx);
    if (!ctx) return SR_ERR_INVALID;
    if (!a || !a->p || !out || !out->p) return ctx->fail(SR_ERR_INVALID, "null tensor");
    for (const sr_view* v : {a, b, out})
        if (v && v->p && (v->coff < 0 || v->cs - v->coff < C)) return ctx->fail(SR_ERR_INVALID, "a view is narrower than its channel count");
    const float* bp = (b && b->p) ? static_cast<const float*>(b->p) + b->coff : nullptr;
    return eltwise_views_launch(ctx, op, static_cast<const float*>(a->p) + a->coff, a->cs, bp, bp ? b->cs : 0, alpha, beta,
                                static_cast<float*>(const_cast<void*>(out->p)) + out->coff, out->cs, npix, C, static_cast<hipStream_t>(stream));
}

int sr_self_attention(sr_ctx* ctx, const void* x, int dtype, int B, int H, int W, int C, const float* wf, const float* bf, const float* wg,
                      const float* bg, const float* wh, const float* bh, const float* wv, const float* bv, void* y, void* stream) {
    DeviceGuard dg_(ctx);
    if (!ctx) return SR_ERR_INVALID;
    hipStream_t st = static_cast<hipStream_t>(stream);
    if (C != 64) return ctx->fail(SR_ERR_INVALID, "SelfAttention kernel is built for channels=64 (d_qk=8, d_v=32)");
    if (dtype != SR_DTYPE_F32 && dtype != SR_DTYPE_BF16) return ctx->fail(SR_ERR_INVALID, "dtype must be f32 or bf16");
    if (B <= 0 || H <= 0 || W <= 0) return ctx->fail(SR_ERR_INVALID, "bad tensor shape");
    const float kscale = dtype == SR_DTYPE_BF16 ? 1.4426950408889634f : 1.f;
    std::vector<float> wp((size_t)64 * 48), bp(48);
    for (int ci = 0; ci < 64; ++ci) {
        for (int co = 0; co < 8; ++co) { wp[(size_t)ci * 48 + co] = kscale * wf[ci * 8 + co]; wp[(size_t)ci * 48 + 8 + co] = wg[ci * 8 + co]; }
        for (int co = 0; co < 32; ++co) wp[(size_t)ci * 48 + 16 + co] = wh[ci * 32 + co];
    }
    for (int co = 0; co < 8; ++co) { bp[co] = bf ? kscale * bf[co] : 0.f; bp[8 + co] = bg ? bg[co] : 0.f; }
    for (int co = 0; co < 32; ++co) bp[16 + co] = bh ? bh[co] : 0.f;
    ConvWeights cp, cv;
    int rc = conv_pack_weights(ctx, wp.data(), bp.data(), 1, 64, 48, dtype, &cp);
    if (rc) return rc;
    rc = conv_pack_weights(ctx, wv, bv, 1, 32, 64, dtype, &cv);
    if (rc) { conv_free_weights(ctx, &cp); return rc; }
    const int esz = dtype_size(dtype);
    const int64_t npix = (int64_t)B * H * W;
    void* qkv = ctx->dalloc((size_t)npix * 64 * esz + 4096);
    void* ao = ctx->dalloc((size_t)npix * 32 * esz + 4096);
    if (!qkv || !ao) rc = SR_ERR_OOM;
    if (!rc) rc = (hipMemsetAsync(qkv, 0, (size_t)npix * 64 * esz, st) == hipSuccess) ? SR_OK : ctx->fail(SR_ERR_HIP, "memset");
    ConvEpilogue e0;
    if (!rc) rc = conv_launch(ctx, cp, TensorView{x, 64, 0}, B, H, W, qkv, 64, 0, e0, st);
    if (!rc) rc = attention_launch(ctx, dtype, qkv, 64, 8, 0, 16, B, H * W, ao, 32, 0, st);
    ConvEpilogue e1;
    e1.skip1 = {x, 64, 0}; e1.beta1 = 1.f;
    if (!rc) rc = conv_launch(ctx, cv, TensorView{ao, 32, 0}, B, H, W, y, 64, 0, e1, st);
    hipError_t e = hipStreamSynchronize(st);
    ctx->dfree(qkv); ctx->dfree(ao);
    conv_free_weights(ctx, &cp); conv_free_weights(ctx, &cv);
    if (!rc && e != hipSuccess) return ctx->fail(SR_ERR_HIP, std::string("self_attention: ") + hipGetErrorString(e));
    return rc;
}

int sr_bicubic(sr_ctx* ctx, const void* x, int dtype, int B, int H, int W, int C, int outH, int outW, void* y, void* stream) {
    DeviceGuard dg_(ctx);
    if (!ctx) return SR_ERR_INVALID;
    if (!x || !y) return ctx->fail(SR_ERR_INVALID, "null tensor");
    return bicubic_launch(ctx, x, dtype, B, H, W, C, outH, outW, y, dtype, C, static_cast<hipStream_t>(stream));
}

int sr_resize(sr_ctx* ctx, const void* x, int dtype, int B, int H, int W, int C, int outH, int outW, int interpolation, void* y, void* stream) {
    DeviceGuard dg_(ctx);
    if (!ctx) return SR_ERR_INVALID;
    if (!x || !y) return ctx->fail(SR_ERR_INVALID, "null tensor");
    return resize_launch(ctx, x, dtype, B, H, W, C, outH, outW, interpolation, y, static_cast<hipStream_t>(stream));
}

int sr_psnr(sr_ctx* ctx, const void* a, const void* b, int B, int H, int W, int C, float max_val, float* out_B, void* stream) {
    DeviceGuard dg_(ctx);
    if (!ctx) return SR_ERR_INVALID;
    if (!a || !b || !out_B) return ctx->fail(SR_ERR_INVALID, "null tensor");
    return psnr_launch(ctx, static_cast<const float*>(a), static_cast<const float*>(b), B, (int64_t)H * W * C, max_val, out_B,
                       static_cast<hipStream_t>(stream));
}

int sr_ssim(sr_ctx* ctx, const void* a, const void* b, int B, int H, int W, int C, float max_val, float* out_B, void* stream) {
    DeviceGuard dg_(ctx);
    if (!ctx) return SR_ERR_INVALID;
    if (!a || !b || !out_B) return ctx->fail(SR_ERR_INVALID, "null tensor");
    return ssim_launch(ctx, static_cast<const float*>(a), static_cast<const float*>(b), B, H, W, C, max_val, out_B,
                       static_cast<hipStream_t>(stream));
}

int sr_mse(sr_ctx* ctx, const void* a, const void* b, int64_t n, float* out1, void* stream) {
    DeviceGuard dg_(ctx);
    if (!ctx) return SR_ERR_INVALID;
    if (!a || !b || !out1) return ctx->fail(SR_ERR_INVALID, "null tensor");
    return mse_launch(ctx, static_cast<const float*>(a), static_cast<const float*>(b), n, out1, static_cast<hipStream_t>(stream));
}

int sr_conv2d_wgrad(sr_ctx* ctx, const void* x, const void* dy, int B, int H, int W, int Cin, int Cout, int K, float* dw_hwio, float* db, void* stream) {
    DeviceGuard dg_(ctx);
    if (!ctx) return SR_ERR_INVALID;
    if (!x || !dy || !dw_hwio) return ctx->fail(SR_ERR_INVALID, "null tensor");
    return wgrad_launch(ctx, static_cast<const float*>(x), static_cast<const float*>(dy), B, H, W, Cin, Cout, K, dw_hwio, db, static_cast<hipStream_t>(stream));
}

int sr_conv2d_wgrad_maps(sr_ctx* ctx, const void* x, const void* dy, int B, int H, int W, int Cin, int Cout, float* dw_hwio, float* db, void* stream) {
    DeviceGuard dg_(ctx);
    if (!ctx) return SR_ERR_INVALID;
    if (!x || !dy || !dw_hwio) return ctx->fail(SR_ERR_INVALID, "null tensor");
    return wgrad_maps_launch(ctx, static_cast<const float*>(x), static_cast<const float*>(dy), B, H, W, Cin, Cout, dw_hwio, db, static_cast<hipStream_t>(stream));
}

int sr_eltwise(sr_ctx* ctx, int op, const void* a, const void* b, float alpha, float beta, void* out, int64_t n, void* stream) {
    DeviceGuard dg_(ctx);
    if (!ctx) return SR_ERR_INVALID;
    if (!a || !out) return ctx->fail(SR_ERR_INVALID, "null tensor");
    return eltwise_launch(ctx, op, static_cast<const float*>(a), static_cast<const float*>(b), alpha, beta, static_cast<float*>(out), n, static_cast<hipStream_t>(stream));
}

int sr_adam(sr_ctx* ctx, void* w, const void* g, void* m, void* v, int64_t n, float lr_t, float beta1, float one_minus_beta1, float beta2,
            float one_minus_beta2, float epsilon, float grad_scale, void* stream) {
    DeviceGuard dg_(ctx);
    if (!ctx) return SR_ERR_INVALID;
    if (!w || !g || !m || !v) return ctx->fail(SR_ERR_INVALID, "null tensor");
    return adam_launch(ctx, static_cast<float*>(w), static_cast<const float*>(g), static_cast<float*>(m), static_cast<float*>(v), n, lr_t, beta1,
                       one_minus_beta1, beta2, one_minus_beta2, epsilon, grad_scale, static_cast<hipStream_t>(stream));
}

int sr_space_to_depth(sr_ctx* ctx, const void* x, int B, int H, int W, int C, int r, void* y, void* stream) {
    DeviceGuard dg_(ctx);
    if (!ctx) return SR_ERR_INVALID;
    if (!x || !y) return ctx->fail(SR_ERR_INVALID, "null tensor");
    return space_to_depth_launch(ctx, static_cast<const float*>(x), B, H, W, C, r, static_cast<float*>(y), static_cast<hipStream_t>(stream));
}

int sr_spatial_op(sr_ctx* ctx, int op, const void* x, int B, int H, int W, int C, void* y, void* stream) {
    DeviceGuard dg_(ctx);
    if (!ctx) return SR_ERR_INVALID;
    if (!x || !y) return ctx->fail(SR_ERR_INVALID, "null tensor");
    if (B <= 0 || H <= 0 || W <= 0 || C <= 0) return ctx->fail(SR_ERR_INVALID, "bad tensor shape");
    hipStream_t st = static_cast<hipStream_t>(stream);
    switch (op) {
        case SR_SP_MAXPOOL2: return maxpool2_launch(ctx, SR_DTYPE_F32, x, B, H, W, C, C, y, C, st);
        case SR_SP_GAP: return gap_launch(ctx, SR_DTYPE_F32, x, B, H * W, C, C, static_cast<float*>(y), st);
        case SR_SP_PICK2: return subsample2_launch(ctx, SR_DTYPE_F32, x, B, H, W, C, C, y, C, st);
        case SR_SP_VGG_PREPROCESS:
            if (C != 3) return ctx->fail(SR_ERR_INVALID, "VGG preprocessing takes RGB");
            return vgg_preproc_launch(ctx, x, SR_DTYPE_F32, (int64_t)B * H * W, y, SR_DTYPE_F32, 3, st);
    }
    return ctx->fail(SR_ERR_INVALID, "unknown spatial op");
}

#define SR_F(p) static_cast<const float*>(p)
#define SR_FM(p) static_cast<float*>(p)
int sr_matmul(sr_ctx* ctx, const void* A, const void* B, void* C, int batch, int M, int N, int K, int transA, int transB, float alpha, void* stream) {
    DeviceGuard dg_(ctx);
    if (!ctx) return SR_ERR_INVALID;
    if (!A || !B || !C) return ctx->fail(SR_ERR_INVALID, "null tensor");
    return matmul_launch(ctx, SR_F(A), SR_F(B), SR_FM(C), batch, M, N, K, transA, transB, alpha, static_cast<hipStream_t>(stream));
}
int sr_softmax_rows(sr_ctx* ctx, void* s, int64_t rows, int cols, void* stream) {
    DeviceGuard dg_(ctx);
    if (!ctx) return SR_ERR_INVALID;
    if (!s) return ctx->fail(SR_ERR_INVALID, "null tensor");
    return softmax_rows_launch(ctx, SR_FM(s), rows, cols, static_cast<hipStream_t>(stream));
}
int sr_softmax_bwd(sr_ctx* ctx, const void* p, const void* dp, void* ds, int64_t rows, int cols, void* stream) {
    DeviceGuard dg_(ctx);
    if (!ctx) return SR_ERR_INVALID;
    if (!p || !dp || !ds) return ctx->fail(SR_ERR_INVALID, "null tensor");
    return softmax_bwd_launch(ctx, SR_F(p), SR_F(dp), SR_FM(ds), rows, cols, static_cast<hipStream_t>(stream));
}
int sr_attention_fwd_lse(sr_ctx* ctx, const void* q, const void* k, const void* v, int64_t q_rs, int64_t k_rs, int64_t v_rs, int B, int N, void* o,
                         void* lse, void* stream) {
    DeviceGuard dg_(ctx);
    if (!ctx) return SR_ERR_INVALID;
    if (!q || !k || !v || !o || !lse) return ctx->fail(SR_ERR_INVALID, "null tensor");
    return attention_fwd_lse_launch(ctx, SR_F(q), SR_F(k), SR_F(v), q_rs, k_rs, v_rs, B, N, SR_FM(o), SR_FM(lse), static_cast<hipStream_t>(stream));
}
int sr_attention_bwd(sr_ctx* ctx, const void* q, const void* k, const void* v, const void* o, const void* dO, const void* lse, int64_t q_rs,
                     int64_t k_rs, int64_t v_rs, int B, int N, void* dq, void* dk, void* dv, void* stream) {
    DeviceGuard dg_(ctx);
    if (!ctx) return SR_ERR_INVALID;
    if (!q || !k || !v || !o || !dO || !lse || !dq || !dk || !dv) return ctx->fail(SR_ERR_INVALID, "null tensor");
    return attention_bwd_launch(ctx, SR_F(q), SR_F(k), SR_F(v), SR_F(o), SR_F(dO), SR_F(lse), q_rs, k_rs, v_rs, B, N, SR_FM(dq), SR_FM(dk), SR_FM(dv),
                                static_cast<hipStream_t>(stream));
}
int sr_maxpool2_bwd(sr_ctx* ctx, const void* x, const void* dy, int B, int H, int W, int C, void* dx, void* stream) {
    DeviceGuard dg_(ctx);
    if (!ctx) return SR_ERR_INVALID;
    if (!x || !dy || !dx) return ctx->fail(SR_ERR_INVALID, "null tensor");
    return maxpool2_bwd_launch(ctx, SR_F(x), SR_F(dy), B, H, W, C, SR_FM(dx), static_cast<hipStream_t>(stream));
}
int sr_zero_insert2(sr_ctx* ctx, const void* dy, int B, int H, int W, int C, void* out, void* stream) {
    DeviceGuard dg_(ctx);
    if (!ctx) return SR_ERR_INVALID;
    if (!dy || !out) return ctx->fail(SR_ERR_INVALID, "null tensor");
    return zero_insert2_launch(ctx, SR_F(dy), B, H, W, C, SR_FM(out), static_cast<hipStream_t>(stream));
}
int sr_spectral_l1_bwd(sr_ctx* ctx, const void* a, const void* b, int B, int H, int W, int C, float scale, void* da, void* stream) {
    DeviceGuard dg_(ctx);
    if (!ctx) return SR_ERR_INVALID;
    if (!a || !b || !da) return ctx->fail(SR_ERR_INVALID, "null tensor");
    return spectral_l1_bwd_launch(ctx, SR_F(a), SR_F(b), B, H, W, C, scale, SR_FM(da), static_cast<hipStream_t>(stream));
}

int sr_l1(sr_ctx* ctx, const void* a, const void* b, int64_t n, float* out1, void* stream) {
    DeviceGuard dg_(ctx);
    if (!ctx) return SR_ERR_INVALID;
    if (!a || !b || !out1) return ctx->fail(SR_ERR_INVALID, "null tensor");
    return l1_launch(ctx, static_cast<const float*>(a), static_cast<const float*>(b), n, out1, static_cast<hipStream_t>(stream));
}

int sr_spectral_l1(sr_ctx* ctx, const void* a, const void* b, int B, int H, int W, int C, float* out1, void* stream) {
    DeviceGuard dg_(ctx);
    if (!ctx) return SR_ERR_INVALID;
    if (!a || !b || !out1) return ctx->fail(SR_ERR_INVALID, "null tensor");
    return spectral_l1_launch(ctx, static_cast<const float*>(a), static_cast<const float*>(b), B, H, W, C, out1, static_cast<hipStream_t>(stream));
}

int sr_extract_patches(sr_ctx* ctx, const float* img, int H, int W, int C, int patch, int stride, float mul, float add, int out_dtype,
                       void* out, int64_t out_capacity, int* n_patches, void* stream) {
    DeviceGuard dg_(ctx);
    if (!ctx) return SR_ERR_INVALID;
    if (H <= 0 || W <= 0 || C <= 0 || patch <= 0 || stride <= 0) return ctx->fail(SR_ERR_INVALID, "bad shape/patch/stride");
    const int ph = pad_amount(H, patch, stride), pw = pad_amount(W, patch, stride);
    if (ph >= H || pw >= W) return ctx->fail(SR_ERR_INVALID, "reflect padding needs pad < image size");
    const int Hp = H + ph, Wp = W + pw;
    const int ny = Hp >= patch ? (Hp - patch) / stride + 1 : 0, nx = Wp >= patch ? (Wp - patch) / stride + 1 : 0;
    if (n_patches) *n_patches = ny * nx;
    if (!out) return SR_OK;
    if (!img) return ctx->fail(SR_ERR_INVALID, "null image");
    if (out_dtype != SR_DTYPE_F32 && out_dtype != SR_DTYPE_BF16) return ctx->fail(SR_ERR_INVALID, "out dtype must be f32 or bf16");
    if (out_capacity < (int64_t)ny * nx * patch * patch * C) return ctx->fail(SR_ERR_CAPACITY, "patch buffer too small");
    return extract_patches_launch(ctx, img, H, W, C, patch, stride, mul, add, out_dtype, out, ny, nx, static_cast<hipStream_t>(stream));
}

int sr_overlap_add(sr_ctx* ctx, const void* patches, int in_dtype, int H, int W, int C, int patch, int stride, int scale, float mul,
                   float add, float* out, void* stream) {
    DeviceGuard dg_(ctx);
    if (!ctx) return SR_ERR_INVALID;
    if (!patches || !out) return ctx->fail(SR_ERR_INVALID, "null tensor");
    if (H <= 0 || W <= 0 || C <= 0 || patch <= 0 || stride <= 0 || scale <= 0) return ctx->fail(SR_ERR_INVALID, "bad shape/patch/stride");
    if (in_dtype != SR_DTYPE_F32 && in_dtype != SR_DTYPE_BF16) return ctx->fail(SR_ERR_INVALID, "patch dtype must be f32 or bf16");
    const int Hp = H + pad_amount(H, patch, stride), Wp = W + pad_amount(W, patch, stride);
    const int ny = (Hp - patch) / stride + 1, nx = (Wp - patch) / stride + 1;
    return overlap_add_launch(ctx, patches, in_dtype, H, W, C, patch, stride, scale, mul, add, ny, nx, out, static_cast<hipStream_t>(stream));
}

}
```

super-resolution-images-for-3d-printing-defect-detection_amd/csrc/attention.hip:

```cpp
#include "attn_f32.h"
#include "common.h"

#include <cstdlib>

namespace {

struct AttnParams {
    const char* qkv; int64_t cs; int qoff, koff, voff;
    char* o; int64_t o_cs; int o_coff;
    int N;
    const float* knorm;
};

__global__ void __launch_bounds__(256, 2) attn_f32_kernel(AttnParams p) {
    __shared__ __attribute__((aligned(16))) char vt[32 * ATTN_VT_PITCH];
    const int b = blockIdx.y;
    const float* base = reinterpret_cast<const float*>(p.qkv) + (int64_t)b * p.N * p.cs;
    const AttnF32Args a{base + p.qoff, base + p.koff, base + p.voff, p.cs, p.cs, p.cs,
                        reinterpret_cast<float*>(p.o) + (int64_t)b * p.N * p.o_cs + p.o_coff, p.o_cs, nullptr, p.N};
    attn_f32_body<false>(a, blockIdx.x * 128, vt);
}

constexpr int KT2 = 128;
constexpr int PITCH2 = KT2 * 2 + 8;

__global__ void __launch_bounds__(64) attn_knorm_kernel(const bf16_t* qkv, int64_t cs, int koff, int N, int ngroups, float* out) {
    const int g = blockIdx.x % ngroups, b = blockIdx.x / ngroups, lane = threadIdx.x;
    const bf16_t* base = qkv + (int64_t)b * N * cs + koff;
    float m = 0.f;
#pragma unroll
    for (int t = 0; t < 2; ++t) {
        const int key = g * 128 + t * 64 + lane;
        if (key < N) {
            const bf16x8 k = *reinterpret_cast<const bf16x8*>(base + (int64_t)key * cs);
            float n2 = 0.f;
#pragma unroll
            for (int e = 0; e < 8; ++e) n2 += (float)k[e] * (float)k[e];
            m = fmaxf(m, n2);
        }
    }
#pragma unroll
    for (int o = 32; o > 0; o >>= 1) m = fmaxf(m, __shfl_xor(m, o));
    if (lane == 0) out[(int64_t)b * ngroups + g] = sqrtf(m);
}

template <int QB>
__global__ void __launch_bounds__(256, 3) attn_bf16_kernel(AttnParams p) {
    __shared__ __attribute__((aligned(16))) char vt[32 * PITCH2];
    const int tid = threadIdx.x, lane = tid & 63, wave = tid >> 6, r = lane & 31, h = lane >> 5;
    const int N = p.N;
    constexpr int QW = 64 * QB * 2;
    const int nqt = (N + QW - 1) / QW;
    const int b = blockIdx.x / nqt, qt = blockIdx.x - b * nqt;
    const bf16_t* base = reinterpret_cast<const bf16_t*>(p.qkv) + (int64_t)b * N * p.cs;
    const int cs = (int)p.cs;
    int qi[QB];
    bf16x8 qb[QB];
#pragma unroll
    for (int j = 0; j < QB; ++j) {
        qi[j] = qt * QW + wave * (32 * QB) + j * 32 + r;
        const int qc = qi[j] < N ? qi[j] : N - 1;
        bf16x8 z = {};
        qb[j] = z;
        if (h == 0) qb[j] = *reinterpret_cast<const bf16x8*>(base + (int64_t)qc * cs + p.qoff);
    }
    float qn2 = 0.f;
#pragma unroll
    for (int j = 0; j < QB; ++j) {
        float n2 = 0.f;
#pragma unroll
        for (int e = 0; e < 8; ++e) n2 += (float)qb[j][e] * (float)qb[j][e];
        qn2 = fmaxf(qn2, n2);
    }
#pragma unroll
    for (int o = 32; o > 0; o >>= 1) qn2 = fmaxf(qn2, __shfl_xor(qn2, o));
    const float qmaxv = sqrtf(qn2) * 1.0009765625f;
    const int* knorm_bits = reinterpret_cast<const int*>(p.knorm) + (int64_t)b * ((N + KT2 - 1) / KT2);
    f32x16 oacc[QB];
    bf16x8 sel = {};
    {
        const int m = lane & 15, kg = lane >> 4;
        const bf16_t one = (bf16_t)1.f;
        if ((m == 0 && (kg & 1) == 0) || (m == 1 && (kg & 1) == 1)) sel = bf16x8{one, one, one, one, one, one, one, one};
    }
    f32x4 lacc[QB];
    float m_run[QB];
#pragma unroll
    for (int j = 0; j < QB; ++j) {
        m_run[j] = 0.f; lacc[j] = f32x4{0.f, 0.f, 0.f, 0.f};
#pragma unroll
        for (int e = 0; e < 16; ++e) oacc[j][e] = 0.f;
    }

    const int kp = tid >> 2, oct = tid & 3;
    bf16x8 kneg = {};
    kneg[0] = (bf16_t)-1.f; kneg[1] = (bf16_t)-1.f; kneg[2] = (bf16_t)-1.f;
    auto load_k = [&](int kb) {
        int l;
        asm volatile("v_mbcnt_lo_u32_b32 %0, -1, 0\n\tv_mbcnt_hi_u32_b32 %0, -1, %0" : "=v"(l));
        bf16x8 kf = kneg;
        const int key = kb + (l & 31);
        if (l < 32) kf = *reinterpret_cast<const bf16x8*>(base + (int64_t)(key < N ? key : N - 1) * cs + p.koff);
        return kf;
    };
    bf16x8 knext = load_k(0);
    f32x16 zero16;
#pragma unroll
    for (int e = 0; e < 16; ++e) zero16[e] = 0.f;
    struct { } false_c; struct { int x; } true_c{0};
    auto hmax = [](float v) {
        const unsigned u = __builtin_bit_cast(unsigned, v);
        const auto sw = __builtin_amdgcn_permlane32_swap(u, u, false, false);
        return fmaxf(__builtin_bit_cast(float, (unsigned)sw[0]), __builtin_bit_cast(float, (unsigned)sw[1]));
    };
    auto tile = [&](const bf16x8 kf, const int sub, const int kb, auto ragged_tag, const bool first) {
        constexpr bool RAGGED = sizeof(ragged_tag) > 1;
        f32x16 s[QB];
        float mx[QB];
#pragma unroll
        for (int j = 0; j < QB; ++j) {
            s[j] = __builtin_amdgcn_mfma_f32_32x32x16_bf16(kf, qb[j], zero16, 0, 0, 0);
            if constexpr (RAGGED) {
#pragma unroll
                for (int i = 0; i < 16; ++i)
                    if (kb + (i & 3) + 8 * (i >> 2) + 4 * h >= N) s[j][i] = -INFINITY;
            }
            float m = fmaxf(fmaxf(s[j][0], s[j][1]), s[j][2]);
#pragma unroll
            for (int i = 3; i + 1 < 16; i += 2) m = fmaxf(fmaxf(m, s[j][i]), s[j][i + 1]);
            m = fmaxf(m, s[j][15]);
            mx[j] = hmax(m);
        }
        bool grew = first;
#pragma unroll
        for (int j = 0; j < QB; ++j) grew = grew || mx[j] > 0.f;
        if (__any(grew)) {
#pragma unroll
            for (int j = 0; j < QB; ++j) {
                const float delta = first ? mx[j] : fmaxf(mx[j], 0.f);
                const float alpha = first ? 1.f : __builtin_amdgcn_exp2f(-delta);
                lacc[j][0] *= alpha;
                lacc[j][1] *= __shfl(alpha, (lane + 16) & 63);
#pragma unroll
                for (int e = 0; e < 16; ++e) oacc[j][e] *= alpha;
#pragma unroll
                for (int i = 0; i < 16; ++i) s[j][i] -= delta;
                m_run[j] += delta;
                if (h == 1) {
                    const bf16_t m1 = (bf16_t)m_run[j];
                    const float r1 = m_run[j] - (float)m1;
                    const bf16_t m2 = (bf16_t)r1;
                    qb[j][0] = m1; qb[j][1] = m2; qb[j][2] = (bf16_t)(r1 - (float)m2);
                }
            }
        }
#pragma unroll
        for (int j = 0; j < QB; ++j) {
#pragma unroll
            for (int i = 0; i < 16; ++i) s[j][i] = __builtin_amdgcn_exp2f(s[j][i]);
        }
#pragma unroll
        for (int ks = 0; ks < 2; ++ks) {
            const char* vrow = vt + r * PITCH2 + (sub * 32 + 16 * ks + 4 * h) * 2;
            const bf16x4 va = *reinterpret_cast<const bf16x4*>(vrow);
            const bf16x4 vb = *reinterpret_cast<const bf16x4*>(vrow + 16);
            const bf16x8 vf = {va[0], va[1], va[2], va[3], vb[0], vb[1], vb[2], vb[3]};
#pragma unroll
            for (int j = 0; j < QB; ++j) {
                bf16x8 pf;
#pragma unroll
                for (int e = 0; e < 8; ++e) pf[e] = (bf16_t)s[j][8 * ks + e];
                oacc[j] = __builtin_amdgcn_mfma_f32_32x32x16_bf16(vf, pf, oacc[j], 0, 0, 0);
                lacc[j] = __builtin_amdgcn_mfma_f32_16x16x32_bf16(sel, pf, lacc[j], 0, 0, 0);
            }
        }
    };

    constexpr float GROW_OK = 40.f;
    auto tile_fast = [&](const bf16x8 kf, const int sub, const bool guard) -> bool {
        f32x16 s[QB];
#pragma unroll
        for (int j = 0; j < QB; ++j) s[j] = __builtin_amdgcn_mfma_f32_32x32x16_bf16(kf, qb[j], zero16, 0, 0, 0);
        if (guard) {
            bool risky = false;
#pragma unroll
            for (int j = 0; j < QB; ++j) {
                float m = fmaxf(fmaxf(s[j][0], s[j][1]), s[j][2]);
#pragma unroll
                for (int i = 3; i + 1 < 16; i += 2) m = fmaxf(fmaxf(m, s[j][i]), s[j][i + 1]);
                m = fmaxf(m, s[j][15]);
                risky = risky || m > GROW_OK;
            }
            if (__any(risky)) return false;
        }
#pragma unroll
        for (int j = 0; j < QB; ++j) {
#pragma unroll
            for (int i = 0; i < 16; ++i) s[j][i] = __builtin_amdgcn_exp2f(s[j][i]);
        }
#pragma unroll
        for (int ks = 0; ks < 2; ++ks) {
            const char* vrow = vt + r * PITCH2 + (sub * 32 + 16 * ks + 4 * h) * 2;
            const bf16x4 va = *reinterpret_cast<const bf16x4*>(vrow);
            const bf16x4 vb = *reinterpret_cast<const bf16x4*>(vrow + 16);
            const bf16x8 vf = {va[0], va[1], va[2], va[3], vb[0], vb[1], vb[2], vb[3]};
#pragma unroll
            for (int j = 0; j < QB; ++j) {
                bf16x8 pf;
#pragma unroll
                for (int e = 0; e < 8; ++e) pf[e] = (bf16_t)s[j][8 * ks + e];
                oacc[j] = __builtin_amdgcn_mfma_f32_32x32x16_bf16(vf, pf, oacc[j], 0, 0, 0);
                lacc[j] = __builtin_amdgcn_mfma_f32_16x16x32_bf16(sel, pf, lacc[j], 0, 0, 0);
            }
        }
        return true;
    };
    auto thresh_of_wave = [&]() -> int {
        float m = m_run[0];
#pragma unroll
        for (int j = 1; j < QB; ++j) m = fminf(m, m_run[j]);
#pragma unroll
        for (int o = 32; o > 0; o >>= 1) m = fminf(m, __shfl_xor(m, o));
        const float lim = GROW_OK + m;
        const float th = !(lim >= 0.f) ? -1.f : (qmaxv > 0.f ? lim / qmaxv * 0.9990234375f : INFINITY);
        return __builtin_amdgcn_readfirstlane(__builtin_bit_cast(int, th));
    };
    int thresh_bits = __builtin_amdgcn_readfirstlane(__builtin_bit_cast(int, -1.f));
    auto stage_v = [&](const int k0, auto whole_tag) {
        constexpr bool WHOLE = sizeof(whole_tag) > 1;
        __syncthreads();
#pragma unroll
        for (int part = 0; part < KT2 / 128; ++part) {
            const int ka = k0 + part * 128 + 2 * kp, kbb = ka + 1;
            if (!WHOLE && ka - 2 * kp >= N) break;
            const bf16x8 va = *reinterpret_cast<const bf16x8*>(base + (int64_t)(WHOLE || ka < N ? ka : N - 1) * cs + p.voff + oct * 8);
            const bf16x8 vb = *reinterpret_cast<const bf16x8*>(base + (int64_t)(WHOLE || kbb < N ? kbb : N - 1) * cs + p.voff + oct * 8);
#pragma unroll
            for (int e = 0; e < 8; ++e) {
                typedef bf16_t bf16x2 __attribute__((ext_vector_type(2)));
                bf16x2 pr = {va[e], vb[e]};
                *reinterpret_cast<bf16x2*>(vt + (oct * 8 + e) * PITCH2 + (part * 64 + kp) * 4) = pr;
            }
        }
        __syncthreads();
    };
    auto slow_tiles = [&](const int k0, const int sub0, bf16x8 kf) {
        for (int sub = sub0; sub < KT2 / 32; ++sub) {
            const int kb = k0 + sub * 32;
            if (kb >= N) break;
            if (sub != sub0) { kf = knext; knext = load_k(kb + 32); }
            if (kb + 32 <= N) tile(kf, sub, kb, false_c, kb == 0);
            else tile(kf, sub, kb, true_c, kb == 0);
        }
    };

    const unsigned kvoff = (unsigned)r * (unsigned)cs * 2u;
    auto fetch_k = [&](bf16x8& use, bf16x8& next, const char* tile_base) {
        asm volatile("s_waitcnt vmcnt(0)\n\ts_mov_b32 exec_hi, 0\n\tglobal_load_dwordx4 %1, %2, %3\n\ts_mov_b32 exec_hi, -1"
                     : "+v"(use), "+v"(next) : "v"(kvoff), "s"(tile_base) : "memory");
    };
    const int nfast = N % KT2 == 0 ? N / KT2 : (N - 32) / KT2;
    auto fast_run = [&](const int g) -> int {
        if (g >= nfast) return 0;
        int l;
        asm volatile("v_mbcnt_lo_u32_b32 %0, -1, 0\n\tv_mbcnt_hi_u32_b32 %0, -1, %0" : "=v"(l));
        const int gi = g + l;
        const bool ok = gi < nfast && knorm_bits[gi < nfast ? gi : nfast - 1] <= thresh_bits;
        const unsigned long long fails = ~__ballot(ok);
        return fails ? __builtin_ctzll(fails) : 64;
    };
    const char* const kimg = reinterpret_cast<const char*>(base + p.koff);
    const int64_t tile_bytes = (int64_t)32 * cs * 2;

    for (int k0 = 0; k0 < N;) {
        {
            stage_v(k0, false_c);
            int sub = 0;
            bf16x8 kf = knext;
            const bool full = k0 != 0 && k0 + KT2 <= N;
            if (full) {
                const bool guard = !(knorm_bits[k0 / KT2] <= thresh_bits);
#pragma unroll
                for (; sub < KT2 / 32; ++sub) {
                    kf = knext;
                    knext = load_k(k0 + sub * 32 + 32);
                    if (!tile_fast(kf, sub, guard)) break;
                }
            } else {
                knext = load_k(k0 + 32);
            }
            if (sub < KT2 / 32) {
                slow_tiles(k0, sub, kf);
                thresh_bits = thresh_of_wave();
            }
            k0 += KT2;
        }
        int run = fast_run(k0 / KT2);
        if (run > 0) {
            bf16x8 ka = knext, kb = kneg;
            const char* kt = kimg + (int64_t)(k0 + 32) * cs * 2;
            do {
                stage_v(k0, true_c);
                fetch_k(ka, kb, kt); kt += tile_bytes;
                tile_fast(ka, 0, false);
                fetch_k(kb, ka, kt); kt += tile_bytes;
                tile_fast(kb, 1, false);
                fetch_k(ka, kb, kt); kt += tile_bytes;
                tile_fast(ka, 2, false);
                fetch_k(kb, ka, k0 + KT2 + 32 <= N ? kt : kt - tile_bytes); kt += tile_bytes;
                tile_fast(kb, 3, false);
                k0 += KT2;
            } while (--run);
            asm volatile("s_waitcnt vmcnt(0)" : "+v"(ka));
            knext = ka;
        }
    }
#pragma unroll
    for (int j = 0; j < QB; ++j) {
        const float l0 = __shfl(lacc[j][0], r & 15), l1 = __shfl(lacc[j][1], r & 15);
        const float inv = 1.f / ((r >> 4) ? l1 : l0);
        if (qi[j] < N) {
            bf16_t* op = reinterpret_cast<bf16_t*>(p.o) + ((int64_t)b * N + qi[j]) * p.o_cs + p.o_coff;
#pragma unroll
            for (int g = 0; g < 4; ++g) {
                bf16x4 t = {(bf16_t)(oacc[j][4 * g] * inv), (bf16_t)(oacc[j][4 * g + 1] * inv), (bf16_t)(oacc[j][4 * g + 2] * inv),
                            (bf16_t)(oacc[j][4 * g + 3] * inv)};
                *reinterpret_cast<bf16x4*>(op + 8 * g + 4 * h) = t;
            }
        }
    }
}

}

int attention_launch(sr_ctx* ctx, int dtype, const void* qkv, int64_t cs, int qoff, int koff, int voff, int B, int N,
                     void* o, int64_t o_cs, int o_coff, hipStream_t st) {
    if (B <= 0 || N <= 0) return ctx->fail(SR_ERR_INVALID, "attention: empty tensor");
    const int esz = dtype_size(dtype);
    if ((cs * esz) % 16 || (qoff * esz) % 16 || (koff * esz) % 16 || (voff * esz) % 16 || (o_cs * esz) % 16 || (o_coff * esz) % 16)
        return ctx->fail(SR_ERR_INVALID, "attention: views must be 16-byte aligned");
    AttnParams p{static_cast<const char*>(qkv), cs, qoff, koff, voff, static_cast<char*>(o), o_cs, o_coff, N, nullptr};
    dim3 grid((unsigned)((N + 127) / 128), (unsigned)B);
    if (dtype != SR_DTYPE_BF16 && dtype != SR_DTYPE_F32) return ctx->fail(SR_ERR_INVALID, "attention: dtype must be f32 or bf16");
    const int rec = ctx->prof_open(dtype == SR_DTYPE_BF16 ? "attn<bf16>" : "attn<f32>", 2.0 * B * (double)N * N * 40.0,
                                   (double)B * N * 80.0 * esz, st);
    if (dtype == SR_DTYPE_BF16) {
        constexpr int QBr = 2;
        const int64_t nwg = (int64_t)B * ((N + 128 * QBr - 1) / (128 * QBr));
        const int ngroups = (N + KT2 - 1) / KT2;
        if (nwg >= (1ll << 31) || (int64_t)B * ngroups >= (1ll << 31)) { ctx->prof_close(rec, st); return ctx->fail(SR_ERR_INVALID, "attention: too many workgroups for one launch"); }
        float* kn = static_cast<float*>(ctx->arena(ctx->attn_kn, sizeof(float) * (size_t)B * ngroups, st));
        if (!kn) { ctx->prof_close(rec, st); return SR_ERR_OOM; }
        p.knorm = kn;
        hipLaunchKernelGGL(attn_knorm_kernel, dim3((unsigned)((int64_t)B * ngroups)), dim3(64), 0, st, reinterpret_cast<const bf16_t*>(qkv) + 0, cs, koff, N, ngroups, kn);
        hipLaunchKernelGGL(attn_bf16_kernel<QBr>, dim3((unsigned)nwg), dim3(256), 0, st, p);
    }
    else hipLaunchKernelGGL(attn_f32_kernel, grid, dim3(256), 0, st, p);
    ctx->prof_close(rec, st);
    SR_HIP(ctx, hipGetLastError());
    return SR_OK;
}
```

super-resolution-images-for-3d-printing-defect-detection_amd/csrc/common.h:

```cpp
#pragma once
#include <hip/hip_runtime.h>
#include <stdint.h>
#include <string.h>
#include <algorithm>
#include <string>
#include <unordered_map>
#include <unordered_set>
#include <vector>

#include "../../include/sr355.h"

typedef __bf16 bf16_t;
typedef __bf16 bf16x8 __attribute__((ext_vector_type(8)));
typedef __bf16 bf16x4 __attribute__((ext_vector_type(4)));
typedef float f32x4 __attribute__((ext_vector_type(4)));
typedef float f32x16 __attribute__((ext_vector_type(16)));

struct sr_ctx {
    int device = 0;
    std::string err;
    int64_t cur_bytes = 0, peak_bytes = 0;
    std::unordered_map<void*, size_t> allocs;
    hipEvent_t ev0 = nullptr, ev1 = nullptr;
    bool timed = false;

    void* scratch_buf = nullptr;
    size_t scratch_cap = 0;
    unsigned long long* stamp_buf = nullptr;
    int64_t stamp_cap = 0;
    int chain_stamp_skip = -1;
    unsigned long long* chain_stamp_buf = nullptr;

    struct ProfRec { int name; hipEvent_t e0, e1; double flops, bytes; };
    bool prof = false;
    std::vector<std::string> prof_names;
    std::vector<ProfRec> prof_recs;
    std::vector<hipEvent_t> ev_pool;
    int prof_open(const std::string& name, double flops, double bytes, hipStream_t st);
    void prof_close(int rec, hipStream_t st);

    static constexpr int MAX_LDS_BYTES = 160 * 1024;
    std::unordered_map<const void*, int> lds_attr_done;
    int ensure_dyn_lds(const void* kernel, int bytes);
    void* tab_buf = nullptr; size_t tab_cap = 0;
    struct Arena { void* p = nullptr; size_t cap = 0; };
    Arena attn_kn;
    Arena attn_d;
    Arena small_w;
    Arena dev_w, dev_b, dev_x;
    Arena cls_tab, cls_work, cls_fft;
    std::unordered_map<int64_t, double*> dft_ops;
    Arena met_work, met_fft;
    Arena eda_work, eda_dct;
    Arena deg_work;
    Arena crop_work;
    Arena sn_work, sn_tab, dhead_work;
    std::vector<char> sn_tab_host;
    void* sn_tab_dev = nullptr;
    struct LpipsState* lpips = nullptr;
    Arena lpips_work;
    int* deg_status = nullptr;
    void* arena(Arena& a, size_t bytes, hipStream_t st);
    struct PackKey {
        const void* w; const void* b; int K, Cin, Cout, rot;
        bool operator==(const PackKey& o) const { return w == o.w && b == o.b && K == o.K && Cin == o.Cin && Cout == o.Cout && rot == o.rot; }
    };
    struct PackKeyHash {
        size_t operator()(const PackKey& k) const {
            return std::hash<const void*>()(k.w) ^ (std::hash<const void*>()(k.b) * 31u) ^ ((size_t)k.rot << 1) ^ ((size_t)k.Cin << 20) ^ ((size_t)k.Cout << 36) ^ ((size_t)k.K << 52);
        }
    };
    struct PackSet {
        std::unordered_map<PackKey, std::pair<void*, float*>, PackKeyHash> cache;
        Arena w, b, tab;
        std::vector<char> tab_host;
        void* tab_dev = nullptr;
    };
    PackSet pack32, pack16;
    static constexpr int ZERO_PAGE_BYTES = 32768;
    void* zero_page = nullptr;
    int num_cus = 0;
    int cu_count();
    int chain_mask = 511;
    int chain_max_wgs = 0;
    int block_stream_bands = 0;
    int64_t alloc_cap = 0;
    bool route_log = false;
    std::string route_text;

    void* dalloc(size_t bytes);
    void dfree(void* p);
    void* scratch(size_t bytes);
    int fail(int code, const std::string& msg) { err = msg; return code; }
};
static_assert(511 == SR_FUSE_ALL && SR_FUSE_ALL == (SR_FUSE_DENSE_TAIL | SR_FUSE_DENSE_MID | SR_FUSE_RGB_TAIL | SR_FUSE_ATTN_PROJ | SR_FUSE_CELLS | SR_FUSE_CONV1_STREAM |
                                             SR_FUSE_POOL | SR_FUSE_CONV_STREAM | SR_FUSE_SRCNN_1X1), "sr_ctx::chain_mask's default is every SR_FUSE_* bit");

struct DeviceGuard {
    int prev = -1; bool switched = false;
    explicit DeviceGuard(const sr_ctx* c) {
        if (c && hipGetDevice(&prev) == hipSuccess && prev != c->device) switched = hipSetDevice(c->device) == hipSuccess;
    }
    ~DeviceGuard() { if (switched) (void)hipSetDevice(prev); }
    DeviceGuard(const DeviceGuard&) = delete;
    DeviceGuard& operator=(const DeviceGuard&) = delete;
};

#define SR_HIP(ctx, call)                                                                        \
    do {                                                                                         \
        hipError_t e_ = (call);                                                                  \
        if (e_ != hipSuccess)                                                                    \
            return (ctx)->fail(SR_ERR_HIP, std::string(#call) + ": " + hipGetErrorString(e_));   \
    } while (0)

void lpips_release(sr_ctx* ctx);

__device__ inline int gray_bgr(int b, int g, int r) { return (1868 * b + 9617 * g + 4899 * r + 8192) >> 14; }

static inline int dtype_size(int dt) { return dt == SR_DTYPE_F32 ? 4 : (dt == SR_DTYPE_BF16 ? 2 : 1); }
static inline int round_up(int a, int b) { return (a + b - 1) / b * b; }
static inline uint16_t f32_to_bf16_host(float f) {
    uint32_t u;
    memcpy(&u, &f, 4);
    if ((u & 0x7fffffffu) > 0x7f800000u) return (uint16_t)((u >> 16) | 0x40);
    u += 0x7fffu + ((u >> 16) & 1u);
    return (uint16_t)(u >> 16);
}

int weights_upload(sr_ctx* ctx, const void* packed, size_t bytes, const float* bias, int n, int npad, void** d_w, float** d_bias);
template <typename P> static inline void weights_free(sr_ctx* ctx, P*& w, float*& bias) {
    if (w) ctx->dfree(w);
    if (bias) ctx->dfree(bias);
    w = nullptr; bias = nullptr;
}

struct ConvWeights {
    void* w = nullptr;
    float* bias = nullptr;
    int dtype = SR_DTYPE_BF16;
    int KS = 3, Cin = 0, Cout = 0;
    int CinP = 0, CoutP = 0;
    int thin = 0;
    int KGPT = 2;
    int NT = 1;
    int rows = 0;
    int few = 0;
    int pw = 0;
    int nchunks = 1;
    size_t bytes = 0;
};

struct TensorView {
    const void* p = nullptr;
    int64_t cs = 0;
    int coff = 0;
    int blk = 0;
};

struct RgbTailWeights {
    void* a = nullptr;
    float* bias = nullptr;
    int c2 = 0;
};

struct ProjWeights {
    void* a = nullptr;
    float* bias = nullptr;
    int nblk = 0;
};

struct Pw2Weights {
    float* a = nullptr;
    float* bias = nullptr;
    int cin = 0, cout = 0, act = 0;
};

struct CellGrid {
    int gx = 0, ch = 0, cw = 0, Hv = 0, Wv = 0;
    bool operator==(const CellGrid& o) const { return gx == o.gx && ch == o.ch && cw == o.cw && Hv == o.Hv && Wv == o.Wv; }
};

struct ConvEpilogue {
    TensorView pool_out;
    CellGrid pool_grid;
    int cell_h = 0, cell_w = 0;
    const ProjWeights* pj = nullptr;
    TensorView pj_out;
    const Pw2Weights* pw2 = nullptr;
    const RgbTailWeights* f2 = nullptr;
    float* f2_part = nullptr;
    int act = SR_ACT_LINEAR;
    float alpha = 1.f;
    TensorView skip1, skip2;
    float beta1 = 0.f, beta2 = 0.f;
    int clip01 = 0;
    int d2s_r = 1;
    int out_f32 = 0;
    int allow_splitk = 0;
};

int conv_pack_weights_dev(sr_ctx* ctx, const float* d_hwio, const float* d_bias, int KS, int Cin, int Cout, int rot, ConvWeights* out, hipStream_t st);
int conv_prepack_dev(sr_ctx* ctx, const sr_pack_desc* descs, int n, hipStream_t st);
int conv_pack_weights_dev_bf16(sr_ctx* ctx, const float* d_hwio, const float* d_bias, int KS, int Cin, int Cout, int rot, ConvWeights* out, hipStream_t st);
int conv_prepack_dev_bf16(sr_ctx* ctx, const sr_pack_desc* descs, int n, hipStream_t st);
int conv_pack_weights(sr_ctx* ctx, const float* hwio, const float* bias, int KS, int Cin, int Cout,
                      int dtype, ConvWeights* out, int rows_head = 0);
static inline void conv_free_weights(sr_ctx* ctx, ConvWeights* w) { weights_free(ctx, w->w, w->bias); }
int conv_launch(sr_ctx* ctx, const ConvWeights& w, TensorView x, int B, int H, int W,
                void* y, int64_t y_cs, int y_coff, const ConvEpilogue& ep, hipStream_t st);
int conv_launch(sr_ctx* ctx, const ConvWeights& w, TensorView x, int B, int H, int W, TensorView y, const ConvEpilogue& ep, hipStream_t st);

int proj_pack_weights(sr_ctx* ctx, const float* w_hwio, const float* bias, int cout, ProjWeights* out);
int pw2_pack_weights(sr_ctx* ctx, const float* w_hwio, const float* bias, int cin, int cout, int act, Pw2Weights* out);
static inline void pw2_free_weights(sr_ctx* ctx, Pw2Weights* w) { weights_free(ctx, w->a, w->bias); *w = Pw2Weights{}; }
static inline void proj_free_weights(sr_ctx* ctx, ProjWeights* w) { weights_free(ctx, w->a, w->bias); }
int rgbtail_pack_weights(sr_ctx* ctx, const float* w2_hwio, const float* bias2, int c2, RgbTailWeights* out);
static inline void rgbtail_free_weights(sr_ctx* ctx, RgbTailWeights* w) { weights_free(ctx, w->a, w->bias); }
int64_t rgbtail_partial_bytes(int B, int H, int W);
int rgbtail_finish_launch(sr_ctx* ctx, const RgbTailWeights& w, const float* part, int B, int H, int W, int act, float alpha, int clip01, void* y,
                          int64_t y_cs, int y_coff, int out_f32, hipStream_t st);

struct ChainWeights {
    void* w = nullptr; float* bias = nullptr;
    int ext = 0, nb0 = 0, nb1 = 0;
    size_t bytes = 0;
};
int chain_pack_weights(sr_ctx* ctx, const float* wa_hwio, const float* ba, const float* wb_hwio, const float* bb, int ext, int nb0, int nb1, ChainWeights* out);
static inline void chain_free_weights(sr_ctx* ctx, ChainWeights* w) { weights_free(ctx, w->w, w->bias); }
bool chain_supported(const ChainWeights& w, const TensorView& in, int W);
bool conv1_stream_supported(const ConvWeights& w, const TensorView& in, int W);
int conv1_stream_launch(sr_ctx* ctx, const ConvWeights& w, TensorView in, int B, int H, int W, hipStream_t st, bool seam = false);
int pack_pairs_launch(sr_ctx* ctx, const void* src, int64_t src_cs, int src_coff, int B, int H, int W, int C, void* dst, int64_t dst_C, int dst_coff, hipStream_t st);
int unpack_pairs_launch(sr_ctx* ctx, const void* src, int64_t src_C, int src_coff, int B, int H, int W, int C, void* dst, int64_t dst_C, int dst_coff, hipStream_t st);
int cell_pack_launch(sr_ctx* ctx, const void* src, int64_t src_cs, int src_coff, int B, int H, int W, int C, void* dst, int64_t dst_C, int dst_coff, const CellGrid& g, hipStream_t st);
int cell_unpack_launch(sr_ctx* ctx, const void* src, int64_t src_C, int src_coff, int B, int H, int W, int C, void* dst, int64_t dst_C, int dst_coff, const CellGrid& g, hipStream_t st);
int chain_launch(sr_ctx* ctx, const ChainWeights& w, TensorView in, int B, int H, int W, TensorView out, TensorView skip_o, float alpha, float beta_x,
                 float beta_o, hipStream_t st, bool seam = false);

struct BlockWeights { void* w = nullptr; float* bias = nullptr; size_t bytes = 0; };
int block_pack_weights(sr_ctx* ctx, const float* const k[5], const float* const b[5], BlockWeights* out);
static inline void block_free_weights(sr_ctx* ctx, BlockWeights* w) { weights_free(ctx, w->w, w->bias); }
int block_launch(sr_ctx* ctx, const BlockWeights& w, TensorView in, int B, int H, int W, TensorView out, TensorView skip_o, float alpha, float beta1,
                 float beta2, int x_skip, int store_growth, hipStream_t st);
int block_stream_launch(sr_ctx* ctx, const BlockWeights& w, TensorView in, int B, int H, int W, TensorView out, TensorView skip_o, float alpha, float beta1,
                        float beta2, int x_skip, int store_growth, hipStream_t st);

int attention_launch(sr_ctx* ctx, int dtype, const void* qkv, int64_t cs, int qoff, int koff, int voff,
                     int B, int N, void* o, int64_t o_cs, int o_coff, hipStream_t st);
int attention_fwd_lse_launch(sr_ctx* ctx, const float* q, const float* k, const float* v, int64_t q_rs, int64_t k_rs, int64_t v_rs, int B, int N,
                             float* o, float* lse, hipStream_t st);
int attention_bwd_launch(sr_ctx* ctx, const float* q, const float* k, const float* v, const float* o, const float* dout, const float* lse,
                         int64_t q_rs, int64_t k_rs, int64_t v_rs, int B, int N, float* dq, float* dk, float* dv, hipStream_t st);

int nhwc_to_blocked_launch(sr_ctx* ctx, const void* src, int64_t src_cs, int src_coff, int B, int H, int W, int C, void* dst, int64_t dst_C,
                           int dst_coff, hipStream_t st);
int clock_probe_launch(sr_ctx* ctx, float* mhz_out, hipStream_t st);
int tap_copy_launch(sr_ctx* ctx, const void* src, int dtype, int blk, int64_t cs, int coff, int B, int H, int W, int C, float* dst, hipStream_t st, bool pairs = false);
int convert_pad_launch(sr_ctx* ctx, const void* x, int in_dtype, int64_t npix, int C, void* y, int out_dtype,
                       int Cp, float mul, float add, hipStream_t st);
int maxpool2_launch(sr_ctx* ctx, int dtype, const void* x, int B, int H, int W, int C, int64_t x_cs, void* y,
                    int64_t y_cs, hipStream_t st, CellGrid in_grid = CellGrid{}, CellGrid out_grid = CellGrid{});
int gap_launch(sr_ctx* ctx, int dtype, const void* x, int B, int HW, int C, int64_t x_cs, float* y, hipStream_t st);
int dense_launch(sr_ctx* ctx, const float* x, const float* w, const float* bias, int B, int In, int Out, int act,
                 float* y, int y_dtype, void* y_typed, hipStream_t st);
int bicubic_launch(sr_ctx* ctx, const void* x, int dtype, int B, int H, int W, int C, int outH, int outW,
                   void* y, int out_dtype, int64_t y_cs, hipStream_t st);
int subsample2_launch(sr_ctx* ctx, int dtype, const void* x, int B, int H, int W, int C, int64_t x_cs, void* y, int64_t y_cs, hipStream_t st);
int vgg_preproc_launch(sr_ctx* ctx, const void* x, int in_dtype, int64_t npix, void* y, int out_dtype, int Cp, hipStream_t st);
int l1_launch(sr_ctx* ctx, const float* a, const float* b, int64_t n, float* out, hipStream_t st);
int spectral_l1_launch(sr_ctx* ctx, const float* a, const float* b, int B, int H, int W, int C, float* out, hipStream_t st);
int wgrad_launch(sr_ctx* ctx, const float* x, const float* dy, int B, int H, int W, int Cin, int Cout, int KS, float* dw, float* db, hipStream_t st);
int wgrad_maps_launch(sr_ctx* ctx, const float* x, const float* dy, int B, int H, int W, int Cin, int Cout, float* dw, float* db, hipStream_t st);
int wgrad_launch_views(sr_ctx* ctx, const float* x, int64_t x_cs, const float* dy, int64_t dy_cs, int B, int H, int W, int Cin, int Cout, int KS, float* dw, float* db,
                       hipStream_t st);
int eltwise_views_launch(sr_ctx* ctx, int op, const float* a, int64_t a_cs, const float* b, int64_t b_cs, float alpha, float beta, float* out, int64_t o_cs, int64_t npix, int C,
                         hipStream_t st);
int adam_launch(sr_ctx* ctx, float* w, const float* g, float* m, float* v, int64_t n, float lr_t, float b1, float omb1, float b2, float omb2, float eps,
                float gscale, hipStream_t st);
int eltwise_launch(sr_ctx* ctx, int op, const float* a, const float* b, float alpha, float beta, float* out, int64_t n, hipStream_t st);
int space_to_depth_launch(sr_ctx* ctx, const float* x, int B, int H, int W, int C, int r, float* y, hipStream_t st);
int wgrad_bf16_launch(sr_ctx* ctx, const bf16_t* x, int64_t x_cs, const bf16_t* dy, int64_t dy_cs, int B, int H, int W, int Cin, int Cout, float scale, float* dw, float* db,
                      hipStream_t st);
int wgrad_group_bf16_launch(sr_ctx* ctx, const sr_wgrad_job* jobs, int n, int B, int H, int W, hipStream_t st);
int eltwise_views_bf16_launch(sr_ctx* ctx, int op, const bf16_t* a, int64_t a_cs, const bf16_t* b, int64_t b_cs, float alpha, float beta, bf16_t* out, int64_t o_cs, int64_t npix,
                              int C, hipStream_t st);
int relu_bwd_bf16_launch(sr_ctx* ctx, const bf16_t* dy, const bf16_t* y, bf16_t* out, int64_t n, hipStream_t st);
int space_to_depth_bf16_launch(sr_ctx* ctx, const bf16_t* x, int B, int H, int W, int C, int r, bf16_t* y, hipStream_t st);
int mse_clip_grad_bf16_launch(sr_ctx* ctx, const bf16_t* pre, const float* t, int64_t n, float* loss, bf16_t* dpre, float* y, hipStream_t st);
int matmul_launch(sr_ctx* ctx, const float* A, const float* B, float* C, int batch, int M, int N, int K, int tA, int tB, float alpha, hipStream_t st);
int softmax_rows_launch(sr_ctx* ctx, float* s, int64_t rows, int cols, hipStream_t st);
int softmax_bwd_launch(sr_ctx* ctx, const float* p, const float* dp, float* ds, int64_t rows, int cols, hipStream_t st);
int maxpool2_bwd_launch(sr_ctx* ctx, const float* x, const float* dy, int B, int H, int W, int C, float* dx, hipStream_t st);
int zero_insert2_launch(sr_ctx* ctx, const float* dy, int B, int H, int W, int C, float* out, hipStream_t st);
int spectral_l1_bwd_launch(sr_ctx* ctx, const float* a, const float* b, int B, int H, int W, int C, float scale, float* da, hipStream_t st);
int resize_launch(sr_ctx* ctx, const void* x, int dtype, int B, int H, int W, int C, int outH, int outW, int interp, void* y, hipStream_t st);
int psnr_launch(sr_ctx* ctx, const float* a, const float* b, int B, int64_t n_per_image, float max_val, float* out,
                hipStream_t st);
int ssim_launch(sr_ctx* ctx, const float* a, const float* b, int B, int H, int W, int C, float max_val, float* out,
                hipStream_t st);
int mse_launch(sr_ctx* ctx, const float* a, const float* b, int64_t n, float* out, hipStream_t st);
int extract_patches_launch(sr_ctx* ctx, const float* img, int H, int W, int C, int patch, int stride, float mul,
                           float add, int out_dtype, void* out, int ny, int nx, hipStream_t st);
int overlap_add_launch(sr_ctx* ctx, const void* patches, int in_dtype, int H, int W, int C, int patch, int stride,
                       int scale, float mul, float add, int ny, int nx, float* out, hipStream_t st);

static inline int pad_amount(int n, int patch, int stride) {
    int pad = (n % stride != 0) ? (patch - (n % stride)) % stride : 0;
    int extra = patch - stride;
    return pad > extra ? pad : extra;
}
```

super-resolution-images-for-3d-printing-defect-detection_amd/csrc/conv_stream.hip:

```cpp
#include <stdlib.h>

#include <algorithm>
#include <type_traits>

#include "conv_rows_epi.h"

namespace {

using namespace convk;

__device__ __forceinline__ f32x4 mma16s(bf16x8 a, bf16x8 b, f32x4 c) { return __builtin_amdgcn_mfma_f32_16x16x32_bf16(a, b, c, 0, 0, 0); }

constexpr int S_NCOMP = 8, S_NLOAD = 4, S_R = 3;
constexpr int S_TH = S_NCOMP * S_R, S_TW = 16, S_PH = S_TH + 2, S_PW = S_TW + 2, S_NPIX = S_PH * S_PW;
constexpr int S_BUF = S_NPIX * 64;
constexpr int S_NBUF = 3;
constexpr int S_WB = 2 * 9 * 4 * 1024;
constexpr int S_LDS = S_WB + S_NBUF * S_BUF + 64 * 4;
constexpr int S_PIECES = (S_NPIX + 15) / 16;
static_assert(S_LDS <= 160 * 1024, "LDS budget");

template <int N> __device__ __forceinline__ void wait_vm() {
    static_assert(N >= 0 && N < 64, "vmcnt is a 6-bit counter");
    asm volatile("s_waitcnt vmcnt(%0)" ::"n"(N) : "memory");
}

struct StreamParams {
    ConvParams c;
    const char* zero;
    int nct, tilesX, tilesY;
    int tiles_per_wg;
    int ntiles;
};

__global__ void __launch_bounds__((S_NCOMP + S_NLOAD) * 64, (S_NCOMP + S_NLOAD + 3) / 4) conv64_stream_kernel(StreamParams sp) {
    extern __shared__ __attribute__((aligned(16))) char smem[];
    char* const lw = smem;
    char* const stg = smem + S_WB;
    float* const lbias = reinterpret_cast<float*>(stg + S_NBUF * S_BUF);
    constexpr int NTHR = (S_NCOMP + S_NLOAD) * 64;
    const ConvParams& p = sp.c;
    const int tid = threadIdx.x, lane = tid & 63, px = lane & 15, q = lane >> 4;
    const int wave = __builtin_amdgcn_readfirstlane(tid >> 6);
    const int ct = blockIdx.x % sp.nct, wgs = blockIdx.x / sp.nct;
    const int t0 = wgs * sp.tiles_per_wg, t1 = min(sp.ntiles, t0 + sp.tiles_per_wg);
    if (t0 >= t1) return;
    const int nunits = 2 * (t1 - t0);
    const int H = p.H, W = p.W;

    {
        const char* wsrc = p.w + (int64_t)ct * S_WB;
        for (int u = tid; u < S_WB / 16; u += NTHR) *reinterpret_cast<f32x4*>(lw + u * 16) = *reinterpret_cast<const f32x4*>(wsrc + u * 16);
        if (tid < 64) lbias[tid] = p.bias[ct * 64 + tid];
    }
    auto tile_of = [&](int tt, int& b, int& y0, int& x0) {
        const int tx = tt % sp.tilesX;
        const int r = tt / sp.tilesX;
        const int ty = r % sp.tilesY;
        b = r / sp.tilesY;
        y0 = ty * S_TH; x0 = tx * S_TW;
    };
    if (wave >= S_NCOMP) {
        asm volatile("s_waitcnt vmcnt(0) lgkmcnt(0)" ::: "memory");
        const int lwr = wave - S_NCOMP;
        auto loader = [&](auto LWc) {
            constexpr int LW = decltype(LWc)::value;
            constexpr int NP = (S_PIECES - LW + 3) / 4;
            int rel[NP];
#pragma unroll
            for (int i = 0; i < NP; ++i) {
                const int t = 16 * (LW + 4 * i) + (lane >> 2);
                rel[i] = t < S_NPIX ? ((t / S_PW) << 16) | (t % S_PW) : -1;
            }
            const int slot = lane & 3;
            auto stage_unit = [&](int k) {
                const int c = k & 1;
                int b, y0, x0;
                tile_of(min(t0 + (k >> 1), t1 - 1), b, y0, x0);
                const char* const img = p.in + ((int64_t)b * H * W * p.in_cs + p.in_coff) * 2 + c * 64;
                char* const dst = stg + (k % S_NBUF) * S_BUF;
#pragma unroll
                for (int i = 0; i < NP; ++i) {
                    const int t = 16 * (LW + 4 * i) + (lane >> 2);
                    const int gy = y0 + (rel[i] >> 16) - 1, gx = x0 + (rel[i] & 0xffff) - 1;
                    const bool inside = rel[i] >= 0 && (unsigned)gy < (unsigned)H && (unsigned)gx < (unsigned)W;
                    const int sl = slot ^ ((t & 4) >> 1);
                    const char* src = inside ? img + ((int64_t)gy * W + gx) * (p.in_cs * 2) + sl * 16 : sp.zero + sl * 16;
                    if (rel[i] >= 0)
                        __builtin_amdgcn_global_load_lds((const __attribute__((address_space(1))) void*)src,
                                                         (__attribute__((address_space(3))) void*)(dst + (LW + 4 * i) * 1024), 16, 0, 0);
                }
            };
            stage_unit(0); stage_unit(1);
            for (int k = 0; k < nunits; ++k) {
                if (k == 0) wait_vm<NP>();
                __builtin_amdgcn_s_barrier();
                stage_unit(k + 2);
                wait_vm<NP>();
            }
            asm volatile("s_waitcnt vmcnt(0)" ::: "memory");
        };
        if (lwr == 0) loader(std::integral_constant<int, 0>{});
        else if (lwr == 1) loader(std::integral_constant<int, 1>{});
        else if (lwr == 2) loader(std::integral_constant<int, 2>{});
        else loader(std::integral_constant<int, 3>{});
        return;
    }
    asm volatile("s_waitcnt vmcnt(0) lgkmcnt(0)" ::: "memory");
    const int tbase = wave * S_R * S_PW + px;
    auto xaddr = [&](int yi, int kx) {
        const int tt = tbase + yi * S_PW + kx;
        return tt * 64 + ((q * 16) ^ ((tt & 4) << 3));
    };
    auto tiles = [&](auto KINDc) {
    constexpr int KIND = decltype(KINDc)::value;
    for (int ti = t0; ti < t1; ++ti) {
        f32x4 acc[S_R][4];
#pragma unroll
        for (int r = 0; r < S_R; ++r)
#pragma unroll
            for (int n = 0; n < 4; ++n) acc[r][n] = f32x4{0.f, 0.f, 0.f, 0.f};
#pragma unroll
        for (int c = 0; c < 2; ++c) {
            const int k = 2 * (ti - t0) + c;
            asm volatile("s_waitcnt lgkmcnt(0)" ::: "memory");
            __builtin_amdgcn_s_barrier();
            const char* const lin = stg + (k % S_NBUF) * S_BUF;
            const char* const lwc = lw + c * (9 * 4 * 1024);
            bf16x8 xcur = *reinterpret_cast<const bf16x8*>(lin + xaddr(0, 0));
#pragma unroll
            for (int kx = 0; kx < 3; ++kx) {
                bf16x8 wf[3][4];
#pragma unroll
                for (int ky = 0; ky < 3; ++ky)
#pragma unroll
                    for (int n = 0; n < 4; ++n) wf[ky][n] = *reinterpret_cast<const bf16x8*>(lwc + ((ky * 3 + kx) * 4 + n) * 1024 + lane * 16);
#pragma unroll
                for (int yi = 0; yi < S_R + 2; ++yi) {
                    const bf16x8 xf = xcur;
                    if (yi + 1 < S_R + 2) xcur = *reinterpret_cast<const bf16x8*>(lin + xaddr(yi + 1, kx));
                    else if (kx + 1 < 3) xcur = *reinterpret_cast<const bf16x8*>(lin + xaddr(0, kx + 1));
#pragma unroll
                    for (int ky = 0; ky < 3; ++ky) {
                        const int yo = yi - ky;
                        if (yo >= 0 && yo < S_R) {
#pragma unroll
                            for (int n = 0; n < 4; ++n) acc[yo][n] = mma16s(wf[ky][n], xf, acc[yo][n]);
                        }
                    }
                }
            }
        }
        int b, y0, x0;
        tile_of(ti, b, y0, x0);
        f32x4 biasv[4];
#pragma unroll
        for (int n = 0; n < 4; ++n) biasv[n] = *reinterpret_cast<const f32x4*>(lbias + n * 16 + 4 * q);
        rows_epilogue_as<4, S_R, KIND>(p, acc, biasv, b, y0, x0, ct, wave, px, q);
    }
    };
    switch (rows_epilogue_kind<4>(p)) {
        case 0: tiles(std::integral_constant<int, 0>{}); break;
        case 1: tiles(std::integral_constant<int, 1>{}); break;
        case 2: tiles(std::integral_constant<int, 2>{}); break;
        default: tiles(std::integral_constant<int, 3>{}); break;
    }
}

}

bool conv_stream_supported(const ConvWeights& w, const convk::ConvParams& p) {
    return w.rows && w.dtype == SR_DTYPE_BF16 && w.NT == 4 && w.nchunks == 2 && w.Cin == 64 && w.CoutP == w.Cout && p.in_ps == 32 && p.in_cs >= 64 && p.in_cs % 8 == 0 &&
           p.in_coff % 8 == 0 && p.H % S_TH == 0 && p.W % S_TW == 0 && p.skip_lds == 0 && !p.f2w && !p.pjw && !p.plout && !p.dbg && p.cell_h == 0 && p.cell_w == 0 &&
           p.vec != 0 && (p.Cout & 3) == 0 && p.act != SR_ACT_TANH && (p.r <= 1 || (p.Cd & 15) == 0) && !p.s2;
}

int conv_stream_launch(sr_ctx* ctx, const ConvWeights& w, const convk::ConvParams& p0, hipStream_t st) {
    if (!ctx->zero_page) return ctx->fail(SR_ERR_STATE, "context has no zero page");
    StreamParams sp;
    sp.c = p0;
    sp.zero = static_cast<const char*>(ctx->zero_page);
    sp.nct = w.CoutP / 64;
    sp.tilesX = p0.W / S_TW; sp.tilesY = p0.H / S_TH;
    sp.c.tilesX = sp.tilesX; sp.c.tilesY = sp.tilesY;
    const int64_t ntiles = (int64_t)p0.B * sp.tilesX * sp.tilesY;
    if (ntiles >= (1ll << 30)) return ctx->fail(SR_ERR_INVALID, "conv_stream: too many tiles for one launch");
    sp.ntiles = (int)ntiles;
    const int ncu = ctx->cu_count();
    const int groups = (int)std::max<int64_t>(1, std::min<int64_t>(ntiles, ncu / sp.nct > 0 ? ncu / sp.nct : 1));
    sp.tiles_per_wg = (int)((ntiles + groups - 1) / groups);
    const int ngroups = (int)((ntiles + sp.tiles_per_wg - 1) / sp.tiles_per_wg);
    auto k = conv64_stream_kernel;
    if (int rc = ctx->ensure_dyn_lds(reinterpret_cast<const void*>(k), S_LDS)) return rc;
    hipLaunchKernelGGL(k, dim3(ngroups * sp.nct), dim3((S_NCOMP + S_NLOAD) * 64), S_LDS, st, sp);
    SR_HIP(ctx, hipGetLastError());
    return SR_OK;
}
```

Baseline: 115.5.

## Fuse attention value projection into attention epilogue and remap stream conv blocks per XCD

Adds an attention kernel variant that applies the 1x1 value conv (32->64) plus bias and residual skip directly in its epilogue using MFMA. This removes the separate conv launch and the round trip of the attention output through memory. Separately, the stream conv kernel remaps block indices so that workgroups sharing the same tile group but different output-channel tiles land on the same XCD, which is meant to improve L2 reuse of the input tiles. The stream conv also now respects chain_max_wgs. Environment flags can restore the old behaviour of both changes.

After: 115.8, median of 6. About the same (+0.3%).

```diff
diff --git a/__graft_entry__.py b/__graft_entry__.py
--- a/__graft_entry__.py
+++ b/__graft_entry__.py
@@ -13,8 +13,9 @@
     jobs = str(min(4, os.cpu_count() or 1))
     subprocess.run(["make", "-C", os.path.join(PKG, "csrc"), "-j", jobs], check=True)
     subprocess.run([sys.executable, os.path.join(ROOT, "tools", "check_prefetch_hazards.py")], check=True)
-    subprocess.run([sys.executable, os.path.join(ROOT, "tools", "check_prefetch_hazards.py"), "--source", os.path.join(PKG, "csrc", "attention.hip"),
-                    "--match", "attn_bf16_kernel", "--allow-scratch"], check=True)
+    for kernel in ("attn_bf16_kernel", "attn_bf16v_kernel"):
+        subprocess.run([sys.executable, os.path.join(ROOT, "tools", "check_prefetch_hazards.py"), "--source", os.path.join(PKG, "csrc", "attention.hip"),
+                        "--match", kernel, "--allow-scratch"], check=True)
     import sr355
     from sr355 import _lib
     _lib.load()
diff --git a/super-resolution-images-for-3d-printing-defect-detection_amd/csrc/api.hip b/super-resolution-images-for-3d-printing-defect-detection_amd/csrc/api.hip
--- a/super-resolution-images-for-3d-printing-defect-detection_amd/csrc/api.hip
+++ b/super-resolution-images-for-3d-printing-defect-detection_amd/csrc/api.hip
@@ -102,6 +102,7 @@
     int pack_alt = -1;
     int pw2 = -1;
     int proj = -1;
+    int vconv = -1;
     int block = -1, block_pos = 0;
 };
 struct BufSpec { int C = 0; int mul = 1; int shift = 0; bool vec = false; int Cbuf = 0; int blk = 0; int cshift = 0; int cells = 0; int cat = 0; };
@@ -112,6 +113,7 @@
 struct BlockSpec { int conv[5] = {-1, -1, -1, -1, -1}; BlockWeights w; };
 struct ProjSpec { int conv = -1; ProjWeights w; };
 struct Pw2Spec { int conv = -1; int act = 0; Pw2Weights w; };
+struct VconvSpec { int conv = -1; AttnVconvWeights w; };
 
 }
 
@@ -127,6 +129,7 @@
     std::vector<RgbTailSpec> rgbtails;
     std::vector<ProjSpec> projs;
     std::vector<Pw2Spec> pw2s;
+    std::vector<VconvSpec> vconvs;
     std::vector<BufSpec> bufs;
     std::vector<void*> bufp;
     std::vector<float*> dense_dev;
@@ -188,8 +191,14 @@
         }
         m->ops.push_back(p);
         Op a; a.kind = OP_ATTN; a.in = {qkv, 0}; a.out = {ao, 0}; m->ops.push_back(a);
+        const size_t ai = m->ops.size() - 1;
         Op& v = conv(name + "_v", 1, 32, 64, {ao, 0}, {y, 0});
         v.skip1 = {x, 0}; v.beta1 = 1.f;
+        if (m->T == SR_DTYPE_BF16) {
+            VconvSpec vs; vs.conv = v.conv;
+            m->vconvs.push_back(vs);
+            m->ops[ai].vconv = (int)m->vconvs.size() - 1;
+        }
     }
 };
 
@@ -564,12 +573,25 @@
            op.out.buf >= 0 && !m->bufs[op.out.buf].blk && op.skip2.buf < 0 && !op.clip && op.act != SR_ACT_TANH && m->bufs[op.out.buf].Cbuf % 4 == 0;
 }
 
+bool vconv_fits(const sr_model* m, size_t oi) {
+    const Op& op = m->ops[oi];
+    if (op.kind != OP_ATTN || op.vconv < 0 || m->T != SR_DTYPE_BF16 || !(m->ctx->chain_mask & SR_FUSE_ATTN_PROJ) || m->ctx->attn_vconv_separate || oi + 1 >= m->ops.size() ||
+        tapped(m, oi))
+        return false;
+    const Op& v = m->ops[oi + 1];
+    const ConvSpec& cs = m->convs[m->vconvs[op.vconv].conv];
+    return v.kind == OP_CONV && v.conv == m->vconvs[op.vconv].conv && cs.KS == 1 && cs.Cin == 32 && cs.Cout == 64 && v.in.buf == op.out.buf && v.in.coff == 0 &&
+           v.act == SR_ACT_LINEAR && v.alpha == 1.f && v.skip1.buf >= 0 && v.beta1 == 1.f && v.skip2.buf < 0 && !v.clip && v.d2s == 1 && v.out.buf >= 0 &&
+           !m->bufs[v.out.buf].blk && !m->bufs[v.skip1.buf].blk && !m->grid_now[v.out.buf].gx && !m->grid_now[v.skip1.buf].gx && m->bufs[op.in.buf].Cbuf >= 48;
+}
+
 void plan_routes(sr_model* m, const Layout& L, int B, int H, int W) {
     std::vector<int>& rt = m->routes;
     rt.resize(m->ops.size());
     for (size_t oi = 0; oi < m->ops.size(); ++oi) rt[oi] = m->ops[oi].kind;
     for (size_t oi = 0; oi < m->ops.size(); ++oi) {
         const Op& op = m->ops[oi];
+        if (rt[oi] == OP_ATTN && vconv_fits(m, oi)) rt[oi + 1] = RT_IN_EPILOGUE;
         if (rt[oi] != OP_CONV) continue;
         int h, w;
         buf_hw(m->bufs[op.in.buf], H, W, &h, &w);
@@ -597,6 +619,8 @@
     if (hipSetDevice(device_id) != hipSuccess) return SR_ERR_HIP;
     sr_ctx* c = new sr_ctx();
     c->device = device_id;
+    { const char* e = getenv("SR355_STREAM_MAP_LEGACY"); c->stream_map_legacy = e && atoi(e) != 0; }
+    { const char* e = getenv("SR355_ATTN_VCONV_SEPARATE"); c->attn_vconv_separate = e && atoi(e) != 0; }
     if (hipEventCreate(&c->ev0) != hipSuccess || hipEventCreate(&c->ev1) != hipSuccess) { delete c; return SR_ERR_HIP; }
     c->zero_page = c->dalloc(sr_ctx::ZERO_PAGE_BYTES);
     if (!c->zero_page) { sr_destroy(c); return SR_ERR_OOM; }
@@ -781,6 +805,7 @@
     for (auto& bs : m->blocks) block_free_weights(m->ctx, &bs.w);
     for (auto& rt : m->rgbtails) rgbtail_free_weights(m->ctx, &rt.w);
     for (auto& pj : m->projs) proj_free_weights(m->ctx, &pj.w);
+    for (auto& vc : m->vconvs) attn_vconv_free_weights(m->ctx, &vc.w);
     for (auto& pw : m->pw2s) pw2_free_weights(m->ctx, &pw.w);
     for (auto& p : m->dense_dev) if (p) m->ctx->dfree(p);
     delete m;
@@ -923,6 +948,14 @@
         std::vector<float> k, bias;
         gather(c1, k, bias);
         int rc = proj_pack_weights(ctx, k.data(), bias.data(), c1.Cout, &pj.w);
+        if (rc) return rc;
+    }
+    for (auto& vc : m->vconvs) {
+        attn_vconv_free_weights(ctx, &vc.w);
+        const ConvSpec& c1 = m->convs[vc.conv];
+        std::vector<float> k, bias;
+        gather(c1, k, bias);
+        int rc = attn_vconv_pack_weights(ctx, k.data(), bias.data(), &vc.w);
         if (rc) return rc;
     }
     for (auto& pw : m->pw2s) {
@@ -1071,7 +1104,8 @@
                 rc = vgg_preproc_launch(ctx, x, io_dtype, (int64_t)B * H * W, po, T, vo.cs, st);
                 break;
             case OP_ATTN:
-                rc = attention_launch(ctx, T, vi.p, vi.cs,  8,  0,  16, B, h * w, po, vo.cs, 0, st);
+                if (nx) rc = attention_vconv_launch(ctx, vi.p, vi.cs,  8,  0,  16, B, h * w, m->vconvs[op.vconv].w, m->view(nx->skip1), m->view(nx->out), st);
+                else rc = attention_launch(ctx, T, vi.p, vi.cs,  8,  0,  16, B, h * w, po, vo.cs, 0, st);
                 break;
             case OP_SUBSAMPLE:
                 rc = subsample2_launch(ctx, T, vi.p, B, h, w, m->bufs[op.in.buf].C, vi.cs, po, vo.cs, st);
diff --git a/super-resolution-images-for-3d-printing-defect-detection_amd/csrc/attention.hip b/super-resolution-images-for-3d-printing-defect-detection_amd/csrc/attention.hip
--- a/super-resolution-images-for-3d-printing-defect-detection_amd/csrc/attention.hip
+++ b/super-resolution-images-for-3d-printing-defect-detection_amd/csrc/attention.hip
@@ -10,6 +10,10 @@
     char* o; int64_t o_cs; int o_coff;
     int N;
     const float* knorm;
+    const char* x; int64_t x_cs; int x_coff;
+    char* y; int64_t y_cs; int y_coff;
+    const char* wv;
+    const float* bv;
 };
 
 __global__ void __launch_bounds__(256, 2) attn_f32_kernel(AttnParams p) {
@@ -47,290 +51,41 @@
 template <int QB>
 __global__ void __launch_bounds__(256, 3) attn_bf16_kernel(AttnParams p) {
     __shared__ __attribute__((aligned(16))) char vt[32 * PITCH2];
-    const int tid = threadIdx.x, lane = tid & 63, wave = tid >> 6, r = lane & 31, h = lane >> 5;
-    const int N = p.N;
-    constexpr int QW = 64 * QB * 2;
-    const int nqt = (N + QW - 1) / QW;
-    const int b = blockIdx.x / nqt, qt = blockIdx.x - b * nqt;
-    const bf16_t* base = reinterpret_cast<const bf16_t*>(p.qkv) + (int64_t)b * N * p.cs;
-    const int cs = (int)p.cs;
-    int qi[QB];
-    bf16x8 qb[QB];
-#pragma unroll
-    for (int j = 0; j < QB; ++j) {
-        qi[j] = qt * QW + wave * (32 * QB) + j * 32 + r;
-        const int qc = qi[j] < N ? qi[j] : N - 1;
-        bf16x8 z = {};
-        qb[j] = z;
-        if (h == 0) qb[j] = *reinterpret_cast<const bf16x8*>(base + (int64_t)qc * cs + p.qoff);
-    }
-    float qn2 = 0.f;
-#pragma unroll
-    for (int j = 0; j < QB; ++j) {
-        float n2 = 0.f;
-#pragma unroll
-        for (int e = 0; e < 8; ++e) n2 += (float)qb[j][e] * (float)qb[j][e];
-        qn2 = fmaxf(qn2, n2);
-    }
-#pragma unroll
-    for (int o = 32; o > 0; o >>= 1) qn2 = fmaxf(qn2, __shfl_xor(qn2, o));
-    const float qmaxv = sqrtf(qn2) * 1.0009765625f;
-    const int* knorm_bits = reinterpret_cast<const int*>(p.knorm) + (int64_t)b * ((N + KT2 - 1) / KT2);
-    f32x16 oacc[QB];
-    bf16x8 sel = {};
-    {
-        const int m = lane & 15, kg = lane >> 4;
-        const bf16_t one = (bf16_t)1.f;
-        if ((m == 0 && (kg & 1) == 0) || (m == 1 && (kg & 1) == 1)) sel = bf16x8{one, one, one, one, one, one, one, one};
-    }
-    f32x4 lacc[QB];
-    float m_run[QB];
-#pragma unroll
-    for (int j = 0; j < QB; ++j) {
-        m_run[j] = 0.f; lacc[j] = f32x4{0.f, 0.f, 0.f, 0.f};
-#pragma unroll
-        for (int e = 0; e < 16; ++e) oacc[j][e] = 0.f;
-    }
-
-    const int kp = tid >> 2, oct = tid & 3;
-    bf16x8 kneg = {};
-    kneg[0] = (bf16_t)-1.f; kneg[1] = (bf16_t)-1.f; kneg[2] = (bf16_t)-1.f;
-    auto load_k = [&](int kb) {
-        int l;
-        asm volatile("v_mbcnt_lo_u32_b32 %0, -1, 0\n\tv_mbcnt_hi_u32_b32 %0, -1, %0" : "=v"(l));
-        bf16x8 kf = kneg;
-        const int key = kb + (l & 31);
-        if (l < 32) kf = *reinterpret_cast<const bf16x8*>(base + (int64_t)(key < N ? key : N - 1) * cs + p.koff);
-        return kf;
-    };
-    bf16x8 knext = load_k(0);
-    f32x16 zero16;
-#pragma unroll
-    for (int e = 0; e < 16; ++e) zero16[e] = 0.f;
-    struct { } false_c; struct { int x; } true_c{0};
-    auto hmax = [](float v) {
-        const unsigned u = __builtin_bit_cast(unsigned, v);
-        const auto sw = __builtin_amdgcn_permlane32_swap(u, u, false, false);
-        return fmaxf(__builtin_bit_cast(float, (unsigned)sw[0]), __builtin_bit_cast(float, (unsigned)sw[1]));
-    };
-    auto tile = [&](const bf16x8 kf, const int sub, const int kb, auto ragged_tag, const bool first) {
-        constexpr bool RAGGED = sizeof(ragged_tag) > 1;
-        f32x16 s[QB];
-        float mx[QB];
-#pragma unroll
-        for (int j = 0; j < QB; ++j) {
-            s[j] = __builtin_amdgcn_mfma_f32_32x32x16_bf16(kf, qb[j], zero16, 0, 0, 0);
-            if constexpr (RAGGED) {
-#pragma unroll
-                for (int i = 0; i < 16; ++i)
-                    if (kb + (i & 3) + 8 * (i >> 2) + 4 * h >= N) s[j][i] = -INFINITY;
-            }
-            float m = fmaxf(fmaxf(s[j][0], s[j][1]), s[j][2]);
-#pragma unroll
-            for (int i = 3; i + 1 < 16; i += 2) m = fmaxf(fmaxf(m, s[j][i]), s[j][i + 1]);
-            m = fmaxf(m, s[j][15]);
-            mx[j] = hmax(m);
-        }
-        bool grew = first;
-#pragma unroll
-        for (int j = 0; j < QB; ++j) grew = grew || mx[j] > 0.f;
-        if (__any(grew)) {
-#pragma unroll
-            for (int j = 0; j < QB; ++j) {
-                const float delta = first ? mx[j] : fmaxf(mx[j], 0.f);
-                const float alpha = first ? 1.f : __builtin_amdgcn_exp2f(-delta);
-                lacc[j][0] *= alpha;
-                lacc[j][1] *= __shfl(alpha, (lane + 16) & 63);
-#pragma unroll
-                for (int e = 0; e < 16; ++e) oacc[j][e] *= alpha;
-#pragma unroll
-                for (int i = 0; i < 16; ++i) s[j][i] -= delta;
-                m_run[j] += delta;
-                if (h == 1) {
-                    const bf16_t m1 = (bf16_t)m_run[j];
-                    const float r1 = m_run[j] - (float)m1;
-                    const bf16_t m2 = (bf16_t)r1;
-                    qb[j][0] = m1; qb[j][1] = m2; qb[j][2] = (bf16_t)(r1 - (float)m2);
-                }
-            }
-        }
-#pragma unroll
-        for (int j = 0; j < QB; ++j) {
-#pragma unroll
-            for (int i = 0; i < 16; ++i) s[j][i] = __builtin_amdgcn_exp2f(s[j][i]);
-        }
-#pragma unroll
-        for (int ks = 0; ks < 2; ++ks) {
-            const char* vrow = vt + r * PITCH2 + (sub * 32 + 16 * ks + 4 * h) * 2;
-            const bf16x4 va = *reinterpret_cast<const bf16x4*>(vrow);
-            const bf16x4 vb = *reinterpret_cast<const bf16x4*>(vrow + 16);
-            const bf16x8 vf = {va[0], va[1], va[2], va[3], vb[0], vb[1], vb[2], vb[3]};
-#pragma unroll
-            for (int j = 0; j < QB; ++j) {
-                bf16x8 pf;
-#pragma unroll
-                for (int e = 0; e < 8; ++e) pf[e] = (bf16_t)s[j][8 * ks + e];
-                oacc[j] = __builtin_amdgcn_mfma_f32_32x32x16_bf16(vf, pf, oacc[j], 0, 0, 0);
-                lacc[j] = __builtin_amdgcn_mfma_f32_16x16x32_bf16(sel, pf, lacc[j], 0, 0, 0);
-            }
-        }
-    };
-
-    constexpr float GROW_OK = 40.f;
-    auto tile_fast = [&](const bf16x8 kf, const int sub, const bool guard) -> bool {
-        f32x16 s[QB];
-#pragma unroll
-        for (int j = 0; j < QB; ++j) s[j] = __builtin_amdgcn_mfma_f32_32x32x16_bf16(kf, qb[j], zero16, 0, 0, 0);
-        if (guard) {
-            bool risky = false;
-#pragma unroll
-            for (int j = 0; j < QB; ++j) {
-                float m = fmaxf(fmaxf(s[j][0], s[j][1]), s[j][2]);
-#pragma unroll
-                for (int i = 3; i + 1 < 16; i += 2) m = fmaxf(fmaxf(m, s[j][i]), s[j][i + 1]);
-                m = fmaxf(m, s[j][15]);
-                risky = risky || m > GROW_OK;
-            }
-            if (__any(risky)) return false;
-        }
-#pragma unroll
-        for (int j = 0; j < QB; ++j) {
-#pragma unroll
-            for (int i = 0; i < 16; ++i) s[j][i] = __builtin_amdgcn_exp2f(s[j][i]);
-        }
-#pragma unroll
-        for (int ks = 0; ks < 2; ++ks) {
-            const char* vrow = vt + r * PITCH2 + (sub * 32 + 16 * ks + 4 * h) * 2;
-            const bf16x4 va = *reinterpret_cast<const bf16x4*>(vrow);
-            const bf16x4 vb = *reinterpret_cast<const bf16x4*>(vrow + 16);
-            const bf16x8 vf = {va[0], va[1], va[2], va[3], vb[0], vb[1], vb[2], vb[3]};
-#pragma unroll
-            for (int j = 0; j < QB; ++j) {
-                bf16x8 pf;
-#pragma unroll
-                for (int e = 0; e < 8; ++e) pf[e] = (bf16_t)s[j][8 * ks + e];
-                oacc[j] = __builtin_amdgcn_mfma_f32_32x32x16_bf16(vf, pf, oacc[j], 0, 0, 0);
-                lacc[j] = __builtin_amdgcn_mfma_f32_16x16x32_bf16(sel, pf, lacc[j], 0, 0, 0);
-            }
-        }
-        return true;
-    };
-    auto thresh_of_wave = [&]() -> int {
-        float m = m_run[0];
-#pragma unroll
-        for (int j = 1; j < QB; ++j) m = fminf(m, m_run[j]);
-#pragma unroll
-        for (int o = 32; o > 0; o >>= 1) m = fminf(m, __shfl_xor(m, o));
-        const float lim = GROW_OK + m;
-        const float th = !(lim >= 0.f) ? -1.f : (qmaxv > 0.f ? lim / qmaxv * 0.9990234375f : INFINITY);
-        return __builtin_amdgcn_readfirstlane(__builtin_bit_cast(int, th));
-    };
-    int thresh_bits = __builtin_amdgcn_readfirstlane(__builtin_bit_cast(int, -1.f));
-    auto stage_v = [&](const int k0, auto whole_tag) {
-        constexpr bool WHOLE = sizeof(whole_tag) > 1;
-        __syncthreads();
-#pragma unroll
-        for (int part = 0; part < KT2 / 128; ++part) {
-            const int ka = k0 + part * 128 + 2 * kp, kbb = ka + 1;
-            if (!WHOLE && ka - 2 * kp >= N) break;
-            const bf16x8 va = *reinterpret_cast<const bf16x8*>(base + (int64_t)(WHOLE || ka < N ? ka : N - 1) * cs + p.voff + oct * 8);
-            const bf16x8 vb = *reinterpret_cast<const bf16x8*>(base + (int64_t)(WHOLE || kbb < N ? kbb : N - 1) * cs + p.voff + oct * 8);
-#pragma unroll
-            for (int e = 0; e < 8; ++e) {
-                typedef bf16_t bf16x2 __attribute__((ext_vector_type(2)));
-                bf16x2 pr = {va[e], vb[e]};
-                *reinterpret_cast<bf16x2*>(vt + (oct * 8 + e) * PITCH2 + (part * 64 + kp) * 4) = pr;
-            }
-        }
-        __syncthreads();
-    };
-    auto slow_tiles = [&](const int k0, const int sub0, bf16x8 kf) {
-        for (int sub = sub0; sub < KT2 / 32; ++sub) {
-            const int kb = k0 + sub * 32;
-            if (kb >= N) break;
-            if (sub != sub0) { kf = knext; knext = load_k(kb + 32); }
-            if (kb + 32 <= N) tile(kf, sub, kb, false_c, kb == 0);
-            else tile(kf, sub, kb, true_c, kb == 0);
-        }
-    };
-
-    const unsigned kvoff = (unsigned)r * (unsigned)cs * 2u;
-    auto fetch_k = [&](bf16x8& use, bf16x8& next, const char* tile_base) {
-        asm volatile("s_waitcnt vmcnt(0)\n\ts_mov_b32 exec_hi, 0\n\tglobal_load_dwordx4 %1, %2, %3\n\ts_mov_b32 exec_hi, -1"
-                     : "+v"(use), "+v"(next) : "v"(kvoff), "s"(tile_base) : "memory");
-    };
-    const int nfast = N % KT2 == 0 ? N / KT2 : (N - 32) / KT2;
-    auto fast_run = [&](const int g) -> int {
-        if (g >= nfast) return 0;
-        int l;
-        asm volatile("v_mbcnt_lo_u32_b32 %0, -1, 0\n\tv_mbcnt_hi_u32_b32 %0, -1, %0" : "=v"(l));
-        const int gi = g + l;
-        const bool ok = gi < nfast && knorm_bits[gi < nfast ? gi : nfast - 1] <= thresh_bits;
-        const unsigned long long fails = ~__ballot(ok);
-        return fails ? __builtin_ctzll(fails) : 64;
-    };
-    const char* const kimg = reinterpret_cast<const char*>(base + p.koff);
-    const int64_t tile_bytes = (int64_t)32 * cs * 2;
-
-    for (int k0 = 0; k0 < N;) {
-        {
-            stage_v(k0, false_c);
-            int sub = 0;
-            bf16x8 kf = knext;
-            const bool full = k0 != 0 && k0 + KT2 <= N;
-            if (full) {
-                const bool guard = !(knorm_bits[k0 / KT2] <= thresh_bits);
-#pragma unroll
-                for (; sub < KT2 / 32; ++sub) {
-                    kf = knext;
-                    knext = load_k(k0 + sub * 32 + 32);
-                    if (!tile_fast(kf, sub, guard)) break;
-                }
-            } else {
-                knext = load_k(k0 + 32);
-            }
-            if (sub < KT2 / 32) {
-                slow_tiles(k0, sub, kf);
-                thresh_bits = thresh_of_wave();
-            }
-            k0 += KT2;
-        }
-        int run = fast_run(k0 / KT2);
-        if (run > 0) {
-            bf16x8 ka = knext, kb = kneg;
-            const char* kt = kimg + (int64_t)(k0 + 32) * cs * 2;
-            do {
-                stage_v(k0, true_c);
-                fetch_k(ka, kb, kt); kt += tile_bytes;
-                tile_fast(ka, 0, false);
-                fetch_k(kb, ka, kt); kt += tile_bytes;
-                tile_fast(kb, 1, false);
-                fetch_k(ka, kb, kt); kt += tile_bytes;
-                tile_fast(ka, 2, false);
-                fetch_k(kb, ka, k0 + KT2 + 32 <= N ? kt : kt - tile_bytes); kt += tile_bytes;
-                tile_fast(kb, 3, false);
-                k0 += KT2;
-            } while (--run);
-            asm volatile("s_waitcnt vmcnt(0)" : "+v"(ka));
-            knext = ka;
-        }
-    }
-#pragma unroll
-    for (int j = 0; j < QB; ++j) {
-        const float l0 = __shfl(lacc[j][0], r & 15), l1 = __shfl(lacc[j][1], r & 15);
-        const float inv = 1.f / ((r >> 4) ? l1 : l0);
-        if (qi[j] < N) {
-            bf16_t* op = reinterpret_cast<bf16_t*>(p.o) + ((int64_t)b * N + qi[j]) * p.o_cs + p.o_coff;
-#pragma unroll
-            for (int g = 0; g < 4; ++g) {
-                bf16x4 t = {(bf16_t)(oacc[j][4 * g] * inv), (bf16_t)(oacc[j][4 * g + 1] * inv), (bf16_t)(oacc[j][4 * g + 2] * inv),
-                            (bf16_t)(oacc[j][4 * g + 3] * inv)};
-                *reinterpret_cast<bf16x4*>(op + 8 * g + 4 * h) = t;
-            }
-        }
-    }
+    constexpr bool VCONV = false;
+#include "attn_bf16_body.h"
 }
 
+template <int QB>
+__global__ void __launch_bounds__(256, 3) attn_bf16v_kernel(AttnParams p) {
+    __shared__ __attribute__((aligned(16))) char vt[32 * PITCH2];
+    constexpr bool VCONV = true;
+#include "attn_bf16_body.h"
+}
+
+}
+
+static int attention_launch_impl(sr_ctx* ctx, int dtype, AttnParams p, int B, bool vc, hipStream_t st) {
+    const int N = p.N;
+    const int esz = dtype_size(dtype);
+    dim3 grid((unsigned)((N + 127) / 128), (unsigned)B);
+    const int rec = ctx->prof_open(dtype == SR_DTYPE_BF16 ? "attn<bf16>" : "attn<f32>", 2.0 * B * (double)N * N * 40.0 + (vc ? 2.0 * B * (double)N * 32.0 * 64.0 : 0.0),
+                                   (double)B * N * (vc ? 176.0 : 80.0) * esz, st);
+    if (dtype == SR_DTYPE_BF16) {
+        constexpr int QBr = 2;
+        const int64_t nwg = (int64_t)B * ((N + 128 * QBr - 1) / (128 * QBr));
+        const int ngroups = (N + KT2 - 1) / KT2;
+        if (nwg >= (1ll << 31) || (int64_t)B * ngroups >= (1ll << 31)) { ctx->prof_close(rec, st); return ctx->fail(SR_ERR_INVALID, "attention: too many workgroups for one launch"); }
+        float* kn = static_cast<float*>(ctx->arena(ctx->attn_kn, sizeof(float) * (size_t)B * ngroups, st));
+        if (!kn) { ctx->prof_close(rec, st); return SR_ERR_OOM; }
+        p.knorm = kn;
+        hipLaunchKernelGGL(attn_knorm_kernel, dim3((unsigned)((int64_t)B * ngroups)), dim3(64), 0, st, reinterpret_cast<const bf16_t*>(p.qkv) + 0, p.cs, p.koff, N, ngroups, kn);
+        if (vc) hipLaunchKernelGGL(attn_bf16v_kernel<QBr>, dim3((unsigned)nwg), dim3(256), 0, st, p);
+        else hipLaunchKernelGGL(attn_bf16_kernel<QBr>, dim3((unsigned)nwg), dim3(256), 0, st, p);
+    }
+    else hipLaunchKernelGGL(attn_f32_kernel, grid, dim3(256), 0, st, p);
+    ctx->prof_close(rec, st);
+    SR_HIP(ctx, hipGetLastError());
+    return SR_OK;
 }
 
 int attention_launch(sr_ctx* ctx, int dtype, const void* qkv, int64_t cs, int qoff, int koff, int voff, int B, int N,
@@ -339,24 +94,38 @@
     const int esz = dtype_size(dtype);
     if ((cs * esz) % 16 || (qoff * esz) % 16 || (koff * esz) % 16 || (voff * esz) % 16 || (o_cs * esz) % 16 || (o_coff * esz) % 16)
         return ctx->fail(SR_ERR_INVALID, "attention: views must be 16-byte aligned");
-    AttnParams p{static_cast<const char*>(qkv), cs, qoff, koff, voff, static_cast<char*>(o), o_cs, o_coff, N, nullptr};
-    dim3 grid((unsigned)((N + 127) / 128), (unsigned)B);
     if (dtype != SR_DTYPE_BF16 && dtype != SR_DTYPE_F32) return ctx->fail(SR_ERR_INVALID, "attention: dtype must be f32 or bf16");
-    const int rec = ctx->prof_open(dtype == SR_DTYPE_BF16 ? "attn<bf16>" : "attn<f32>", 2.0 * B * (double)N * N * 40.0,
-                                   (double)B * N * 80.0 * esz, st);
-    if (dtype == SR_DTYPE_BF16) {
-        constexpr int QBr = 2;
-        const int64_t nwg = (int64_t)B * ((N + 128 * QBr - 1) / (128 * QBr));
-        const int ngroups = (N + KT2 - 1) / KT2;
-        if (nwg >= (1ll << 31) || (int64_t)B * ngroups >= (1ll << 31)) { ctx->prof_close(rec, st); return ctx->fail(SR_ERR_INVALID, "attention: too many workgroups for one launch"); }
-        float* kn = static_cast<float*>(ctx->arena(ctx->attn_kn, sizeof(float) * (size_t)B * ngroups, st));
-        if (!kn) { ctx->prof_close(rec, st); return SR_ERR_OOM; }
-        p.knorm = kn;
-        hipLaunchKernelGGL(attn_knorm_kernel, dim3((unsigned)((int64_t)B * ngroups)), dim3(64), 0, st, reinterpret_cast<const bf16_t*>(qkv) + 0, cs, koff, N, ngroups, kn);
-        hipLaunchKernelGGL(attn_bf16_kernel<QBr>, dim3((unsigned)nwg), dim3(256), 0, st, p);
-    }
-    else hipLaunchKernelGGL(attn_f32_kernel, grid, dim3(256), 0, st, p);
-    ctx->prof_close(rec, st);
-    SR_HIP(ctx, hipGetLastError());
+    AttnParams p{};
+    p.qkv = static_cast<const char*>(qkv); p.cs = cs; p.qoff = qoff; p.koff = koff; p.voff = voff;
+    p.o = static_cast<char*>(o); p.o_cs = o_cs; p.o_coff = o_coff; p.N = N;
+    return attention_launch_impl(ctx, dtype, p, B, false, st);
+}
+
+int attn_vconv_pack_weights(sr_ctx* ctx, const float* w_hwio, const float* bias, AttnVconvWeights* out) {
+    std::vector<uint16_t> host(4 * 512, 0);
+    for (int mb = 0; mb < 2; ++mb)
+        for (int kk = 0; kk < 2; ++kk)
+            for (int l = 0; l < 64; ++l)
+                for (int e = 0; e < 8; ++e) {
+                    const int c = 16 * kk + 8 * (e >> 2) + 4 * (l >> 5) + (e & 3);
+                    host[((size_t)(mb * 2 + kk) * 64 + l) * 8 + e] = f32_to_bf16_host(w_hwio[(size_t)c * 64 + 32 * mb + (l & 31)]);
+                }
+    AttnVconvWeights w;
+    if (int rc = weights_upload(ctx, host.data(), host.size() * 2, bias, 64, 64, &w.a, &w.bias)) return rc;
+    *out = w;
     return SR_OK;
 }
+
+int attention_vconv_launch(sr_ctx* ctx, const void* qkv, int64_t cs, int qoff, int koff, int voff, int B, int N, const AttnVconvWeights& w, TensorView x, TensorView y,
+                           hipStream_t st) {
+    if (B <= 0 || N <= 0) return ctx->fail(SR_ERR_INVALID, "attention: empty tensor");
+    if (!w.a || !w.bias || !x.p || !y.p || x.blk || y.blk) return ctx->fail(SR_ERR_INVALID, "attention: the fused output conv needs packed weights and plain NHWC views");
+    if ((cs * 2) % 16 || (qoff * 2) % 16 || (koff * 2) % 16 || (voff * 2) % 16 || (x.cs * 2) % 8 || (x.coff * 2) % 8 || (y.cs * 2) % 8 || (y.coff * 2) % 8)
+        return ctx->fail(SR_ERR_INVALID, "attention: views must be 16-byte aligned (x and y of the fused output conv: 8-byte)");
+    AttnParams p{};
+    p.qkv = static_cast<const char*>(qkv); p.cs = cs; p.qoff = qoff; p.koff = koff; p.voff = voff; p.N = N;
+    p.x = static_cast<const char*>(x.p); p.x_cs = x.cs; p.x_coff = x.coff;
+    p.y = const_cast<char*>(static_cast<const char*>(y.p)); p.y_cs = y.cs; p.y_coff = y.coff;
+    p.wv = static_cast<const char*>(w.a); p.bv = w.bias;
+    return attention_launch_impl(ctx, SR_DTYPE_BF16, p, B, true, st);
+}
diff --git a/super-resolution-images-for-3d-printing-defect-detection_amd/csrc/attn_bf16_body.h b/super-resolution-images-for-3d-printing-defect-detection_amd/csrc/attn_bf16_body.h
--- /dev/null
+++ b/super-resolution-images-for-3d-printing-defect-detection_amd/csrc/attn_bf16_body.h
@@ -0,0 +1,332 @@
+    const int tid = threadIdx.x, lane = tid & 63, wave = tid >> 6, r = lane & 31, h = lane >> 5;
+    const int N = p.N;
+    constexpr int QW = 64 * QB * 2;
+    const int nqt = (N + QW - 1) / QW;
+    const int b = blockIdx.x / nqt, qt = blockIdx.x - b * nqt;
+    const bf16_t* base = reinterpret_cast<const bf16_t*>(p.qkv) + (int64_t)b * N * p.cs;
+    const int cs = (int)p.cs;
+    int qi[QB];
+    bf16x8 qb[QB];
+#pragma unroll
+    for (int j = 0; j < QB; ++j) {
+        qi[j] = qt * QW + wave * (32 * QB) + j * 32 + r;
+        const int qc = qi[j] < N ? qi[j] : N - 1;
+        bf16x8 z = {};
+        qb[j] = z;
+        if (h == 0) qb[j] = *reinterpret_cast<const bf16x8*>(base + (int64_t)qc * cs + p.qoff);
+    }
+    float qn2 = 0.f;
+#pragma unroll
+    for (int j = 0; j < QB; ++j) {
+        float n2 = 0.f;
+#pragma unroll
+        for (int e = 0; e < 8; ++e) n2 += (float)qb[j][e] * (float)qb[j][e];
+        qn2 = fmaxf(qn2, n2);
+    }
+#pragma unroll
+    for (int o = 32; o > 0; o >>= 1) qn2 = fmaxf(qn2, __shfl_xor(qn2, o));
+    const float qmaxv = sqrtf(qn2) * 1.0009765625f;
+    const int* knorm_bits = reinterpret_cast<const int*>(p.knorm) + (int64_t)b * ((N + KT2 - 1) / KT2);
+    f32x16 oacc[QB];
+    bf16x8 sel = {};
+    {
+        const int m = lane & 15, kg = lane >> 4;
+        const bf16_t one = (bf16_t)1.f;
+        if ((m == 0 && (kg & 1) == 0) || (m == 1 && (kg & 1) == 1)) sel = bf16x8{one, one, one, one, one, one, one, one};
+    }
+    f32x4 lacc[QB];
+    float m_run[QB];
+#pragma unroll
+    for (int j = 0; j < QB; ++j) {
+        m_run[j] = 0.f; lacc[j] = f32x4{0.f, 0.f, 0.f, 0.f};
+#pragma unroll
+        for (int e = 0; e < 16; ++e) oacc[j][e] = 0.f;
+    }
+
+    const int kp = tid >> 2, oct = tid & 3;
+    bf16x8 kneg = {};
+    kneg[0] = (bf16_t)-1.f; kneg[1] = (bf16_t)-1.f; kneg[2] = (bf16_t)-1.f;
+    auto load_k = [&](int kb) {
+        int l;
+        asm volatile("v_mbcnt_lo_u32_b32 %0, -1, 0\n\tv_mbcnt_hi_u32_b32 %0, -1, %0" : "=v"(l));
+        bf16x8 kf = kneg;
+        const int key = kb + (l & 31);
+        if (l < 32) kf = *reinterpret_cast<const bf16x8*>(base + (int64_t)(key < N ? key : N - 1) * cs + p.koff);
+        return kf;
+    };
+    bf16x8 knext = load_k(0);
+    f32x16 zero16;
+#pragma unroll
+    for (int e = 0; e < 16; ++e) zero16[e] = 0.f;
+    struct { } false_c; struct { int x; } true_c{0};
+    auto hmax = [](float v) {
+        const unsigned u = __builtin_bit_cast(unsigned, v);
+        const auto sw = __builtin_amdgcn_permlane32_swap(u, u, false, false);
+        return fmaxf(__builtin_bit_cast(float, (unsigned)sw[0]), __builtin_bit_cast(float, (unsigned)sw[1]));
+    };
+    auto tile = [&](const bf16x8 kf, const int sub, const int kb, auto ragged_tag, const bool first) {
+        constexpr bool RAGGED = sizeof(ragged_tag) > 1;
+        f32x16 s[QB];
+        float mx[QB];
+#pragma unroll
+        for (int j = 0; j < QB; ++j) {
+            s[j] = __builtin_amdgcn_mfma_f32_32x32x16_bf16(kf, qb[j], zero16, 0, 0, 0);
+            if constexpr (RAGGED) {
+#pragma unroll
+                for (int i = 0; i < 16; ++i)
+                    if (kb + (i & 3) + 8 * (i >> 2) + 4 * h >= N) s[j][i] = -INFINITY;
+            }
+            float m = fmaxf(fmaxf(s[j][0], s[j][1]), s[j][2]);
+#pragma unroll
+            for (int i = 3; i + 1 < 16; i += 2) m = fmaxf(fmaxf(m, s[j][i]), s[j][i + 1]);
+            m = fmaxf(m, s[j][15]);
+            mx[j] = hmax(m);
+        }
+        bool grew = first;
+#pragma unroll
+        for (int j = 0; j < QB; ++j) grew = grew || mx[j] > 0.f;
+        if (__any(grew)) {
+#pragma unroll
+            for (int j = 0; j < QB; ++j) {
+                const float delta = first ? mx[j] : fmaxf(mx[j], 0.f);
+                const float alpha = first ? 1.f : __builtin_amdgcn_exp2f(-delta);
+                lacc[j][0] *= alpha;
+                lacc[j][1] *= __shfl(alpha, (lane + 16) & 63);
+#pragma unroll
+                for (int e = 0; e < 16; ++e) oacc[j][e] *= alpha;
+#pragma unroll
+                for (int i = 0; i < 16; ++i) s[j][i] -= delta;
+                m_run[j] += delta;
+                if (h == 1) {
+                    const bf16_t m1 = (bf16_t)m_run[j];
+                    const float r1 = m_run[j] - (float)m1;
+                    const bf16_t m2 = (bf16_t)r1;
+                    qb[j][0] = m1; qb[j][1] = m2; qb[j][2] = (bf16_t)(r1 - (float)m2);
+                }
+            }
+        }
+#pragma unroll
+        for (int j = 0; j < QB; ++j) {
+#pragma unroll
+            for (int i = 0; i < 16; ++i) s[j][i] = __builtin_amdgcn_exp2f(s[j][i]);
+        }
+#pragma unroll
+        for (int ks = 0; ks < 2; ++ks) {
+            const char* vrow = vt + r * PITCH2 + (sub * 32 + 16 * ks + 4 * h) * 2;
+            const bf16x4 va = *reinterpret_cast<const bf16x4*>(vrow);
+            const bf16x4 vb = *reinterpret_cast<const bf16x4*>(vrow + 16);
+            const bf16x8 vf = {va[0], va[1], va[2], va[3], vb[0], vb[1], vb[2], vb[3]};
+#pragma unroll
+            for (int j = 0; j < QB; ++j) {
+                bf16x8 pf;
+#pragma unroll
+                for (int e = 0; e < 8; ++e) pf[e] = (bf16_t)s[j][8 * ks + e];
+                oacc[j] = __builtin_amdgcn_mfma_f32_32x32x16_bf16(vf, pf, oacc[j], 0, 0, 0);
+                lacc[j] = __builtin_amdgcn_mfma_f32_16x16x32_bf16(sel, pf, lacc[j], 0, 0, 0);
+            }
+        }
+    };
+
+    constexpr float GROW_OK = 40.f;
+    auto tile_fast = [&](const bf16x8 kf, const int sub, const bool guard) -> bool {
+        f32x16 s[QB];
+#pragma unroll
+        for (int j = 0; j < QB; ++j) s[j] = __builtin_amdgcn_mfma_f32_32x32x16_bf16(kf, qb[j], zero16, 0, 0, 0);
+        if (guard) {
+            bool risky = false;
+#pragma unroll
+            for (int j = 0; j < QB; ++j) {
+                float m = fmaxf(fmaxf(s[j][0], s[j][1]), s[j][2]);
+#pragma unroll
+                for (int i = 3; i + 1 < 16; i += 2) m = fmaxf(fmaxf(m, s[j][i]), s[j][i + 1]);
+                m = fmaxf(m, s[j][15]);
+                risky = risky || m > GROW_OK;
+            }
+            if (__any(risky)) return false;
+        }
+#pragma unroll
+        for (int j = 0; j < QB; ++j) {
+#pragma unroll
+            for (int i = 0; i < 16; ++i) s[j][i] = __builtin_amdgcn_exp2f(s[j][i]);
+        }
+#pragma unroll
+        for (int ks = 0; ks < 2; ++ks) {
+            const char* vrow = vt + r * PITCH2 + (sub * 32 + 16 * ks + 4 * h) * 2;
+            const bf16x4 va = *reinterpret_cast<const bf16x4*>(vrow);
+            const bf16x4 vb = *reinterpret_cast<const bf16x4*>(vrow + 16);
+            const bf16x8 vf = {va[0], va[1], va[2], va[3], vb[0], vb[1], vb[2], vb[3]};
+#pragma unroll
+            for (int j = 0; j < QB; ++j) {
+                bf16x8 pf;
+#pragma unroll
+                for (int e = 0; e < 8; ++e) pf[e] = (bf16_t)s[j][8 * ks + e];
+                oacc[j] = __builtin_amdgcn_mfma_f32_32x32x16_bf16(vf, pf, oacc[j], 0, 0, 0);
+                lacc[j] = __builtin_amdgcn_mfma_f32_16x16x32_bf16(sel, pf, lacc[j], 0, 0, 0);
+            }
+        }
+        return true;
+    };
+    auto thresh_of_wave = [&]() -> int {
+        float m = m_run[0];
+#pragma unroll
+        for (int j = 1; j < QB; ++j) m = fminf(m, m_run[j]);
+#pragma unroll
+        for (int o = 32; o > 0; o >>= 1) m = fminf(m, __shfl_xor(m, o));
+        const float lim = GROW_OK + m;
+        const float th = !(lim >= 0.f) ? -1.f : (qmaxv > 0.f ? lim / qmaxv * 0.9990234375f : INFINITY);
+        return __builtin_amdgcn_readfirstlane(__builtin_bit_cast(int, th));
+    };
+    int thresh_bits = __builtin_amdgcn_readfirstlane(__builtin_bit_cast(int, -1.f));
+    auto stage_v = [&](const int k0, auto whole_tag) {
+        constexpr bool WHOLE = sizeof(whole_tag) > 1;
+        __syncthreads();
+#pragma unroll
+        for (int part = 0; part < KT2 / 128; ++part) {
+            const int ka = k0 + part * 128 + 2 * kp, kbb = ka + 1;
+            if (!WHOLE && ka - 2 * kp >= N) break;
+            const bf16x8 va = *reinterpret_cast<const bf16x8*>(base + (int64_t)(WHOLE || ka < N ? ka : N - 1) * cs + p.voff + oct * 8);
+            const bf16x8 vb = *reinterpret_cast<const bf16x8*>(base + (int64_t)(WHOLE || kbb < N ? kbb : N - 1) * cs + p.voff + oct * 8);
+#pragma unroll
+            for (int e = 0; e < 8; ++e) {
+                typedef bf16_t bf16x2 __attribute__((ext_vector_type(2)));
+                bf16x2 pr = {va[e], vb[e]};
+                *reinterpret_cast<bf16x2*>(vt + (oct * 8 + e) * PITCH2 + (part * 64 + kp) * 4) = pr;
+            }
+        }
+        __syncthreads();
+    };
+    auto slow_tiles = [&](const int k0, const int sub0, bf16x8 kf) {
+        for (int sub = sub0; sub < KT2 / 32; ++sub) {
+            const int kb = k0 + sub * 32;
+            if (kb >= N) break;
+            if (sub != sub0) { kf = knext; knext = load_k(kb + 32); }
+            if (kb + 32 <= N) tile(kf, sub, kb, false_c, kb == 0);
+            else tile(kf, sub, kb, true_c, kb == 0);
+        }
+    };
+
+    const unsigned kvoff = (unsigned)r * (unsigned)cs * 2u;
+    auto fetch_k = [&](bf16x8& use, bf16x8& next, const char* tile_base) {
+        asm volatile("s_waitcnt vmcnt(0)\n\ts_mov_b32 exec_hi, 0\n\tglobal_load_dwordx4 %1, %2, %3\n\ts_mov_b32 exec_hi, -1"
+                     : "+v"(use), "+v"(next) : "v"(kvoff), "s"(tile_base) : "memory");
+    };
+    const int nfast = N % KT2 == 0 ? N / KT2 : (N - 32) / KT2;
+    auto fast_run = [&](const int g) -> int {
+        if (g >= nfast) return 0;
+        int l;
+        asm volatile("v_mbcnt_lo_u32_b32 %0, -1, 0\n\tv_mbcnt_hi_u32_b32 %0, -1, %0" : "=v"(l));
+        const int gi = g + l;
+        const bool ok = gi < nfast && knorm_bits[gi < nfast ? gi : nfast - 1] <= thresh_bits;
+        const unsigned long long fails = ~__ballot(ok);
+        return fails ? __builtin_ctzll(fails) : 64;
+    };
+    const char* const kimg = reinterpret_cast<const char*>(base + p.koff);
+    const int64_t tile_bytes = (int64_t)32 * cs * 2;
+
+    for (int k0 = 0; k0 < N;) {
+        {
+            stage_v(k0, false_c);
+            int sub = 0;
+            bf16x8 kf = knext;
+            const bool full = k0 != 0 && k0 + KT2 <= N;
+            if (full) {
+                const bool guard = !(knorm_bits[k0 / KT2] <= thresh_bits);
+#pragma unroll
+                for (; sub < KT2 / 32; ++sub) {
+                    kf = knext;
+                    knext = load_k(k0 + sub * 32 + 32);
+                    if (!tile_fast(kf, sub, guard)) break;
+                }
+            } else {
+                knext = load_k(k0 + 32);
+            }
+            if (sub < KT2 / 32) {
+                slow_tiles(k0, sub, kf);
+                thresh_bits = thresh_of_wave();
+            }
+            k0 += KT2;
+        }
+        int run = fast_run(k0 / KT2);
+        if (run > 0) {
+            bf16x8 ka = knext, kb = kneg;
+            const char* kt = kimg + (int64_t)(k0 + 32) * cs * 2;
+            do {
+                stage_v(k0, true_c);
+                fetch_k(ka, kb, kt); kt += tile_bytes;
+                tile_fast(ka, 0, false);
+                fetch_k(kb, ka, kt); kt += tile_bytes;
+                tile_fast(kb, 1, false);
+                fetch_k(ka, kb, kt); kt += tile_bytes;
+                tile_fast(ka, 2, false);
+                fetch_k(kb, ka, k0 + KT2 + 32 <= N ? kt : kt - tile_bytes); kt += tile_bytes;
+                tile_fast(kb, 3, false);
+                k0 += KT2;
+            } while (--run);
+            asm volatile("s_waitcnt vmcnt(0)" : "+v"(ka));
+            knext = ka;
+        }
+    }
+    if constexpr (VCONV) {
+        int l;
+        asm volatile("v_mbcnt_lo_u32_b32 %0, -1, 0\n\tv_mbcnt_hi_u32_b32 %0, -1, %0" : "=v"(l));
+        const int hl = l >> 5;
+        const bf16x8* const wfr = reinterpret_cast<const bf16x8*>(p.wv) + l;
+        bf16x8 wf[4];
+#pragma unroll
+        for (int f = 0; f < 4; ++f) wf[f] = wfr[f * 64];
+        f32x4 bias[8];
+        bf16x4 xv[QB][8], yv[4];
+#pragma unroll
+        for (int n = 0; n < 8; ++n) bias[n] = *reinterpret_cast<const f32x4*>(p.bv + 32 * (n >> 2) + 8 * (n & 3) + 4 * hl);
+#pragma unroll
+        for (int j = 0; j < QB; ++j) {
+            const bf16_t* const xp = reinterpret_cast<const bf16_t*>(p.x) + ((int64_t)b * N + qi[j]) * p.x_cs + p.x_coff;
+#pragma unroll
+            for (int n = 0; n < 8; ++n) {
+                xv[j][n] = bf16x4{};
+                if (qi[j] < N) xv[j][n] = *reinterpret_cast<const bf16x4*>(xp + 32 * (n >> 2) + 8 * (n & 3) + 4 * hl);
+            }
+        }
+#pragma unroll
+        for (int j = 0; j < QB; ++j) {
+            const float l0 = __shfl(lacc[j][0], r & 15), l1 = __shfl(lacc[j][1], r & 15);
+            const float inv = 1.f / ((r >> 4) ? l1 : l0);
+            bf16x8 of[2];
+#pragma unroll
+            for (int kk = 0; kk < 2; ++kk)
+#pragma unroll
+                for (int e = 0; e < 8; ++e) of[kk][e] = (bf16_t)(oacc[j][8 * kk + e] * inv);
+            bf16_t* const yp = reinterpret_cast<bf16_t*>(p.y) + ((int64_t)b * N + qi[j]) * p.y_cs + p.y_coff;
+#pragma unroll
+            for (int mb = 0; mb < 2; ++mb) {
+                f32x16 acc;
+#pragma unroll
+                for (int e = 0; e < 16; ++e) acc[e] = 0.f;
+#pragma unroll
+                for (int kk = 0; kk < 2; ++kk) acc = __builtin_amdgcn_mfma_f32_32x32x16_bf16(wf[mb * 2 + kk], of[kk], acc, 0, 0, 0);
+#pragma unroll
+                for (int g = 0; g < 4; ++g)
+#pragma unroll
+                    for (int i = 0; i < 4; ++i) yv[g][i] = (bf16_t)((acc[4 * g + i] + bias[mb * 4 + g][i]) + (float)xv[j][mb * 4 + g][i]);
+                if (qi[j] < N) {
+#pragma unroll
+                    for (int g = 0; g < 4; ++g) *reinterpret_cast<bf16x4*>(yp + 32 * mb + 8 * g + 4 * hl) = yv[g];
+                }
+            }
+        }
+    } else {
+#pragma unroll
+    for (int j = 0; j < QB; ++j) {
+        const float l0 = __shfl(lacc[j][0], r & 15), l1 = __shfl(lacc[j][1], r & 15);
+        const float inv = 1.f / ((r >> 4) ? l1 : l0);
+        if (qi[j] < N) {
+            bf16_t* op = reinterpret_cast<bf16_t*>(p.o) + ((int64_t)b * N + qi[j]) * p.o_cs + p.o_coff;
+#pragma unroll
+            for (int g = 0; g < 4; ++g) {
+                bf16x4 t = {(bf16_t)(oacc[j][4 * g] * inv), (bf16_t)(oacc[j][4 * g + 1] * inv), (bf16_t)(oacc[j][4 * g + 2] * inv),
+                            (bf16_t)(oacc[j][4 * g + 3] * inv)};
+                *reinterpret_cast<bf16x4*>(op + 8 * g + 4 * h) = t;
+            }
+        }
+    }
+    }
diff --git a/super-resolution-images-for-3d-printing-defect-detection_amd/csrc/common.h b/super-resolution-images-for-3d-printing-defect-detection_amd/csrc/common.h
--- a/super-resolution-images-for-3d-printing-defect-detection_amd/csrc/common.h
+++ b/super-resolution-images-for-3d-printing-defect-detection_amd/csrc/common.h
@@ -83,6 +83,8 @@
     int cu_count();
     int chain_mask = 511;
     int chain_max_wgs = 0;
+    bool stream_map_legacy = false;
+    bool attn_vconv_separate = false;
     int block_stream_bands = 0;
     int64_t alloc_cap = 0;
     bool route_log = false;
@@ -247,6 +249,11 @@
 
 int attention_launch(sr_ctx* ctx, int dtype, const void* qkv, int64_t cs, int qoff, int koff, int voff,
                      int B, int N, void* o, int64_t o_cs, int o_coff, hipStream_t st);
+struct AttnVconvWeights { void* a = nullptr; float* bias = nullptr; };
+int attn_vconv_pack_weights(sr_ctx* ctx, const float* w_hwio, const float* bias, AttnVconvWeights* out);
+static inline void attn_vconv_free_weights(sr_ctx* ctx, AttnVconvWeights* w) { weights_free(ctx, w->a, w->bias); }
+int attention_vconv_launch(sr_ctx* ctx, const void* qkv, int64_t cs, int qoff, int koff, int voff, int B, int N, const AttnVconvWeights& w, TensorView x, TensorView y,
+                           hipStream_t st);
 int attention_fwd_lse_launch(sr_ctx* ctx, const float* q, const float* k, const float* v, int64_t q_rs, int64_t k_rs, int64_t v_rs, int B, int N,
                              float* o, float* lse, hipStream_t st);
 int attention_bwd_launch(sr_ctx* ctx, const float* q, const float* k, const float* v, const float* o, const float* dout, const float* lse,
diff --git a/super-resolution-images-for-3d-printing-defect-detection_amd/csrc/conv_stream.hip b/super-resolution-images-for-3d-printing-defect-detection_amd/csrc/conv_stream.hip
--- a/super-resolution-images-for-3d-printing-defect-detection_amd/csrc/conv_stream.hip
+++ b/super-resolution-images-for-3d-printing-defect-detection_amd/csrc/conv_stream.hip
@@ -4,6 +4,7 @@
 #include <type_traits>
 
 #include "conv_rows_epi.h"
+#include "conv_stream_map.h"
 
 namespace {
 
@@ -31,6 +32,7 @@
     int nct, tilesX, tilesY;
     int tiles_per_wg;
     int ntiles;
+    int ngroups, legacy_map;
 };
 
 __global__ void __launch_bounds__((S_NCOMP + S_NLOAD) * 64, (S_NCOMP + S_NLOAD + 3) / 4) conv64_stream_kernel(StreamParams sp) {
@@ -42,7 +44,8 @@
     const ConvParams& p = sp.c;
     const int tid = threadIdx.x, lane = tid & 63, px = lane & 15, q = lane >> 4;
     const int wave = __builtin_amdgcn_readfirstlane(tid >> 6);
-    const int ct = blockIdx.x % sp.nct, wgs = blockIdx.x / sp.nct;
+    const StreamBlock sb = conv_stream_block(blockIdx.x, sp.ngroups, sp.nct, sp.legacy_map != 0);
+    const int ct = sb.ct, wgs = sb.wgs;
     const int t0 = wgs * sp.tiles_per_wg, t1 = min(sp.ntiles, t0 + sp.tiles_per_wg);
     if (t0 >= t1) return;
     const int nunits = 2 * (t1 - t0);
@@ -186,10 +189,13 @@
     const int64_t ntiles = (int64_t)p0.B * sp.tilesX * sp.tilesY;
     if (ntiles >= (1ll << 30)) return ctx->fail(SR_ERR_INVALID, "conv_stream: too many tiles for one launch");
     sp.ntiles = (int)ntiles;
-    const int ncu = ctx->cu_count();
+    int ncu = ctx->cu_count();
+    if (ctx->chain_max_wgs > 0 && ctx->chain_max_wgs < ncu) ncu = ctx->chain_max_wgs;
     const int groups = (int)std::max<int64_t>(1, std::min<int64_t>(ntiles, ncu / sp.nct > 0 ? ncu / sp.nct : 1));
     sp.tiles_per_wg = (int)((ntiles + groups - 1) / groups);
     const int ngroups = (int)((ntiles + sp.tiles_per_wg - 1) / sp.tiles_per_wg);
+    sp.ngroups = ngroups;
+    sp.legacy_map = ctx->stream_map_legacy ? 1 : 0;
     auto k = conv64_stream_kernel;
     if (int rc = ctx->ensure_dyn_lds(reinterpret_cast<const void*>(k), S_LDS)) return rc;
     hipLaunchKernelGGL(k, dim3(ngroups * sp.nct), dim3((S_NCOMP + S_NLOAD) * 64), S_LDS, st, sp);
diff --git a/super-resolution-images-for-3d-printing-defect-detection_amd/csrc/conv_stream_map.h b/super-resolution-images-for-3d-printing-defect-detection_amd/csrc/conv_stream_map.h
--- /dev/null
+++ b/super-resolution-images-for-3d-printing-defect-detection_amd/csrc/conv_stream_map.h
@@ -0,0 +1,21 @@
+#pragma once
+
+#if defined(__HIPCC__)
+#define SR_STREAM_MAP_HD __host__ __device__
+#else
+#define SR_STREAM_MAP_HD
+#endif
+
+constexpr int SR_STREAM_XCDS = 8;
+
+struct StreamBlock { int ct, wgs; };
+
+SR_STREAM_MAP_HD inline StreamBlock conv_stream_block(int block, int ngroups, int nct, bool legacy) {
+    const int full = legacy || nct == 1 ? 0 : ngroups / SR_STREAM_XCDS * SR_STREAM_XCDS * nct;
+    if (block >= full) {
+        const int rest = block - full;
+        return StreamBlock{rest % nct, full / nct + rest / nct};
+    }
+    const int x = block % SR_STREAM_XCDS, j = block / SR_STREAM_XCDS;
+    return StreamBlock{j % nct, j / nct * SR_STREAM_XCDS + x};
+}
```
